# RaphaelHaddad/Real-Time-Brain-Inspired-Video-Memory

Hardware: NVIDIA B200
Metric: queries_per_sec_top10_384d (higher is better)
Workload: dtype tf32

## Files before the change

real-time-brain-inspired-video-memory_b200/csrc/api.cu:

```cuda
#include "common.cuh"

#include <dlfcn.h>
#include <stdarg.h>
#include <stdlib.h>
#include <string.h>
#include <time.h>
#include <new>
#include <vector>

namespace vm {

static thread_local char g_err[512] = "";
void set_error(const char *fmt, ...)
{
    va_list ap;
    va_start(ap, fmt);
    vsnprintf(g_err, sizeof(g_err), fmt, ap);
    va_end(ap);
}

int k_convert_rows(const void *src, int src_dtype, void *dst, int dst_dtype, int64_t n, int dim, int ld, cudaStream_t st);
int k_row_inv_norms(const void *rows, int dtype, float *inv_norms, int64_t row0, int64_t n, int ld, int *extreme, cudaStream_t st,
                    const double *exact = nullptr);
int k_invalidate_rows(float *inv_norms, const int64_t *rows_dev, int64_t n, int64_t size, cudaStream_t st);
int k_normalize_queries(const void *q, int q_dtype, int nq, int nq_pad, int dim, int ld, float *out_f32, void *out_bf16,
                        int32_t *zero_me, uint32_t *zero_tab, int zero_tab_n, int tf32_round, int split, bool pdl, cudaStream_t st);
int k_synth_fill(void *rows, int dtype, uint64_t seed, int64_t row0, int64_t n, int dim, int ld, uint64_t dup_period,
                 cudaStream_t st);
int k_merge_candidates(const uint64_t *cand, int lists, int nq, int kp, uint64_t *merged, cudaStream_t st);

int k_slab_top(const SelectArgs &sa, int nq, int kp, uint64_t *merged, int *incomplete, cudaStream_t st);
int k_rescore(const RescoreArgs &a, cudaStream_t st, const int *incomplete);
int k_select_rescore(const SelectArgs &sa, const RescoreArgs &a, cudaStream_t st, bool pdl);
bool select_rescore_fits(int lists, int list_len, int kp, int dtype, int dim, int ld);
int k_collect_rescore(const uint64_t *buf, const int *cnt, int cap, const RescoreArgs &a, cudaStream_t st);
int k_exact(const ExactArgs &a, cudaStream_t st, bool pdl);
int k_merge_topk_lists(const void *idx, const void *score, const void *count, size_t stride_bytes, int lists, int nq, int k,
                       int64_t *out_idx, double *out_score, int32_t *out_count, cudaStream_t st);
int k_p2p_publish(void *flag, unsigned long long gen, cudaStream_t st);
int k_merge_topk_p2p(void *const *peers, int nranks, size_t slot_off, size_t flag_off, unsigned long long gen, int nq, int k,
                     int64_t *out_idx, double *out_score, int32_t *out_count, cudaStream_t st);
int k_merge_max_by_id(const int64_t *idx, const double *score, const int32_t *count, int nq, int k, int k2,
                      int64_t *out_idx, double *out_score, int32_t *out_count, cudaStream_t st);
int k_cosine_pairs(const void *a, const void *b, int dtype, int64_t n, int dim, int zero_rule, int sum_mode, double *out,
                   cudaStream_t st);
int k_pairs_above(int device, const void *x, int dtype, int64_t n, int dim, int ld, float threshold, int64_t cap,
                  int64_t *out_i, int64_t *out_j, float *out_score, int64_t *out_count, int part, int nparts, int flags,
                  cudaStream_t st);
int k_pairs_concat(const void *gathered, size_t per_rank_bytes, int64_t slot, const int64_t *counts, int nranks, int64_t cap,
                   int64_t *out_i, int64_t *out_j, float *out_score, int64_t *out_count, cudaStream_t st);

struct Arena;
int arena_create(Arena **out, int device, size_t max_bytes);
int arena_grow(Arena *a, size_t bytes);
void arena_destroy(Arena *a);
void *arena_base(const Arena *a);
size_t arena_mapped(const Arena *a);

static constexpr int MAXQ = 64;
static constexpr int MAXK = 64;
static constexpr int XCTAS = 148;
static constexpr int MAX_DEVICES = 64;
static constexpr int COLLECT_CAP = 4096;
static constexpr int FLAG_INTERNAL_CAPTURE = 1 << 30;

struct ResultBlock {
    int64_t *idx;
    double *score;
    int32_t *count;
    static ResultBlock at(void *base, int nq, int k)
    {
        char *b = (char *)base;
        return {(int64_t *)b, (double *)(b + (size_t)nq * k * 8), (int32_t *)(b + (size_t)nq * k * 16)};
    }
    ResultBlock from(int q0, int k) const { return {idx + (size_t)q0 * k, score + (size_t)q0 * k, count + q0}; }
};
static constexpr size_t result_bytes(int nq, int k) { return (size_t)nq * k * 16 + (size_t)nq * 4; }
static constexpr size_t packed_bytes(int nq, int k) { return (result_bytes(nq, k) + 7) & ~(size_t)7; }

static void unpack_to_host(const void *pack, int nq, int k, const ResultBlock &out)
{
    const ResultBlock p = ResultBlock::at(const_cast<void *>(pack), nq, k);
    memcpy(out.idx, p.idx, (size_t)nq * k * 8);
    memcpy(out.score, p.score, (size_t)nq * k * 8);
    memcpy(out.count, p.count, (size_t)nq * 4);
}

struct DeviceGuard {
    int prev = -1;
    bool ok = true;
    explicit DeviceGuard(int dev)
    {
        if (cudaGetDevice(&prev) != cudaSuccess) { ok = false; return; }
        if (prev != dev && cudaSetDevice(dev) != cudaSuccess) ok = false;
    }
    ~DeviceGuard() { if (prev >= 0) cudaSetDevice(prev); }
};

struct Buf {
    void *p = nullptr;
    size_t bytes = 0;
    int ensure(size_t need)
    {
        if (need <= bytes) return VM_OK;
        if (p) cudaFree(p);
        p = nullptr; bytes = 0;
        cudaError_t e = cudaMalloc(&p, need);
        if (e != cudaSuccess) { set_error("cudaMalloc(%zu) failed: %s", need, cudaGetErrorString(e)); return VM_ERR_OOM; }
        bytes = need;
        return VM_OK;
    }
    void release() { if (p) cudaFree(p); p = nullptr; bytes = 0; }
};

struct Workspace {
    bool ready = false;
    int lists_max = 0;
    Buf q_raw, q_f32, q_bf16, seed, cand, merged, o_idx, flags, col_thr, col_cnt, col_buf, xs, xr, xc, taken, gather_send, gather_recv, misc, ubuf, done, scnt, sel_inc;
    int32_t *h_uncert = nullptr;
    unsigned char *h_pack = nullptr;
    unsigned char *h_q = nullptr;
    void release()
    {
        Buf *all[] = {&q_raw, &q_f32, &q_bf16, &seed, &cand, &merged, &o_idx, &flags, &col_thr, &col_cnt, &col_buf, &xs, &xr, &xc, &taken,
                      &gather_send, &gather_recv, &misc, &ubuf, &done, &scnt, &sel_inc};
        for (Buf *b : all) b->release();
        if (h_uncert) cudaFreeHost(h_uncert);
        if (h_pack) cudaFreeHost(h_pack);
        if (h_q) cudaFreeHost(h_q);
        h_uncert = nullptr; h_pack = nullptr; h_q = nullptr;
        ready = false;
    }
};

}

using namespace vm;

struct vm_store {
    int device = 0, dim = 0, ld = 0, dtype = VM_F32, sm_count = 148;
    int64_t capacity = 0, size = 0;
    void *rows = nullptr;
    float *inv_norms = nullptr;
    double *rows_exact = nullptr;
    bool owns = false;
    Arena *ar_rows = nullptr, *ar_inv = nullptr, *ar_exact = nullptr;
    int64_t max_capacity = 0;
    const void *exact_rows() const { return rows_exact ? (const void *)rows_exact : (const void *)rows; }
    int exact_dtype() const { return rows_exact ? (int)VM_F64 : dtype; }
    int *extreme = nullptr;
    unsigned long long *cum = nullptr;
    int64_t n_batches = 0, n_queries = 0;
    int last_band_ctas = 0, last_band_nq = 0;
    Buf stage, stage_idx;
    Workspace ws;
    static constexpr int EV_RING = 64;
    cudaEvent_t evr[EV_RING][2] = {};
    int ev_next = 0;
    int ev_pending = 0;
    int ev_cur = -1;
    bool timed = false;
    struct GraphEntry {
        cudaGraphExec_t exec = nullptr;
        uint64_t version = 0;
        int nq = 0, k = 0, flags = 0, score_mode = 0, sum_mode = 0, q_dtype = 0;
        double min_score = 0.0;
        int64_t row_offset = 0;
        vm_topk_stats stats{};
    };
    GraphEntry graphs[4];
    int graph_next = 0;
    uint64_t version = 1;
    uint64_t seen_version = 0;
    int stable_calls = 0;
    cudaStream_t gstream = nullptr;
};

static constexpr size_t XCHG_SLOT_BYTES = (result_bytes(MAXQ, MAXK) + 255) & ~(size_t)255;
static constexpr size_t XCHG_FLAG_OFF = 2 * XCHG_SLOT_BYTES;
static constexpr size_t XCHG_BYTES = XCHG_FLAG_OFF + 256;

struct vm_comm {
    void *nccl = nullptr;
    int nranks = 1, rank = 0, device = 0;
    void *peer[16] = {};
    bool p2p = false;
    unsigned long long gen = 0;
    Buf pl_i, pl_j, pl_s, pl_cnt, pg_cnt, pg_send, pg_recv;
    int64_t *h_counts = nullptr;
};

struct Id128 { char b[128]; };
namespace {
struct NcclApi {
    void *h = nullptr;
    int (*GetUniqueId)(void *) = nullptr;
    int (*CommInitRank)(void **, int,  Id128, int) = nullptr;
    int (*AllGather)(const void *, void *, size_t, int, void *, cudaStream_t) = nullptr;
    int (*Broadcast)(const void *, void *, size_t, int, int, void *, cudaStream_t) = nullptr;
    int (*CommDestroy)(void *) = nullptr;
    const char *(*GetErrorString)(int) = nullptr;
};
}
static NcclApi g_nccl;

static int nccl_load()
{
    if (g_nccl.h) return VM_OK;
    void *h = dlopen("libnccl.so.2", RTLD_NOW | RTLD_GLOBAL);
    if (!h) h = dlopen("libnccl.so", RTLD_NOW | RTLD_GLOBAL);
    VM_REQUIRE(h, VM_ERR_NCCL, "cannot load libnccl.so.2: %s", dlerror());
    g_nccl.GetUniqueId = (int (*)(void *))dlsym(h, "ncclGetUniqueId");
    g_nccl.CommInitRank = (int (*)(void **, int, Id128, int))dlsym(h, "ncclCommInitRank");
    g_nccl.AllGather = (int (*)(const void *, void *, size_t, int, void *, cudaStream_t))dlsym(h, "ncclAllGather");
    g_nccl.Broadcast = (int (*)(const void *, void *, size_t, int, int, void *, cudaStream_t))dlsym(h, "ncclBroadcast");
    g_nccl.CommDestroy = (int (*)(void *))dlsym(h, "ncclCommDestroy");
    g_nccl.GetErrorString = (const char *(*)(int))dlsym(h, "ncclGetErrorString");
    VM_REQUIRE(g_nccl.GetUniqueId && g_nccl.CommInitRank && g_nccl.AllGather && g_nccl.Broadcast && g_nccl.CommDestroy, VM_ERR_NCCL,
               "libnccl lacks a required symbol");
    g_nccl.h = h;
    return VM_OK;
}
#define VM_NCCL_CHECK(expr)                                                                            \
    do {                                                                                               \
        int _r = (expr);                                                                               \
        if (_r != 0) {                                                                                 \
            set_error("%s failed: %s", #expr, g_nccl.GetErrorString ? g_nccl.GetErrorString(_r) : "?"); \
            return VM_ERR_NCCL;                                                                        \
        }                                                                                              \
    } while (0)

static int check_arch(int device, int *sm_count)
{
    cudaDeviceProp p;
    VM_CUDA_CHECK(cudaGetDeviceProperties(&p, device));
    VM_REQUIRE(p.major == 10, VM_ERR_UNSUPPORTED, "device %d is sm_%d%d; libvidmem is built for sm_100a only", device,
               p.major, p.minor);
    if (sm_count) *sm_count = p.multiProcessorCount;
    return VM_OK;
}

static int ws_prepare(vm_store *s)
{
    Workspace &w = s->ws;
    if (w.ready) return VM_OK;
    int lists = 2 * s->sm_count;
    w.lists_max = lists;
    int rc;
#define ENS(b, bytes) if ((rc = (b).ensure(bytes)) != VM_OK) return rc
    ENS(w.q_raw, (size_t)MAXQ * s->dim * 8);
    ENS(w.q_f32, (size_t)MAXQ * s->ld * 4);
    ENS(w.q_bf16, (size_t)2 * MAXQ * s->ld * 2);
    ENS(w.cand, (size_t)lists * MAXQ * (MAXK > SCAN_SLAB ? MAXK : SCAN_SLAB) * 8);
    ENS(w.merged, (size_t)MAXQ * MAXK * 8);
    ENS(w.o_idx, result_bytes(MAXQ, MAXK) + 64);
    ENS(w.flags, (size_t)(MAXQ + 2) * 4);
    ENS(w.seed, (size_t)(SEED_TAB_WORDS + 3 * MAXQ) * 4);
    ENS(w.ubuf, (size_t)MAXQ * SCAN_UNION_CAP * 8);
    ENS(w.done, 64);
    ENS(w.scnt, (size_t)256 * MAXQ * 4);
    ENS(w.sel_inc, (size_t)MAXQ * 4);
    VM_CUDA_CHECK(cudaMemset(w.done.p, 0, 64));
    ENS(w.col_thr, (size_t)MAXQ * 4);
    ENS(w.col_cnt, (size_t)MAXQ * 4);
    ENS(w.col_buf, (size_t)MAXQ * COLLECT_CAP * 8);
    ENS(w.xs, (size_t)XCTAS * MAXQ * MAXK * 8);
    ENS(w.xr, (size_t)XCTAS * MAXQ * MAXK * 4);
    ENS(w.xc, (size_t)XCTAS * MAXQ * 4);
    ENS(w.taken, (size_t)MAXQ * XCTAS * MAXK);
#undef ENS
    VM_CUDA_CHECK(cudaMallocHost((void **)&w.h_uncert, 64));
    VM_CUDA_CHECK(cudaMallocHost((void **)&w.h_pack, result_bytes(MAXQ, MAXK) + 64));
    VM_CUDA_CHECK(cudaMallocHost((void **)&w.h_q, (size_t)MAXQ * s->dim * 8));
    w.ready = true;
    return VM_OK;
}

static double scan_eps_stored(int kernel, int store_dtype, int dim, int split);
static double scan_eps(int kernel, int store_dtype, int dim, int split, bool shadow = false)
{
    const double base = scan_eps_stored(kernel, store_dtype, dim, split);
    if (!shadow) return base;
    return base + (store_dtype == VM_F32 ? 1.1920928955078125e-07 : 1.953125e-3 * 1.01);
}
static double scan_eps_stored(int kernel, int store_dtype, int dim, int split)
{
    const double u = 1.1920928955078125e-07;
    const double fp32_acc = (double)(dim + 16) * u;
    if (kernel == 1) return fp32_acc;
    if (store_dtype == VM_F32)
        return 9.765625e-4 + 4.8828125e-4 + 1e-6 + fp32_acc;
    if (!split) return 3.90625e-3 + fp32_acc;
    return 1.52587890625e-5 * 1.01 + (double)(dim + dim / 8 + 32) * u;
}

extern "C" int vm_version(void) { return VM_ABI_VERSION; }
extern "C" const char *vm_last_error(void) { return g_err; }

extern "C" int vm_device_info(int device, int *sm_count, int *cc_major, int *cc_minor, size_t *total_mem)
{
    cudaDeviceProp p;
    VM_CUDA_CHECK(cudaGetDeviceProperties(&p, device));
    if (sm_count) *sm_count = p.multiProcessorCount;
    if (cc_major) *cc_major = p.major;
    if (cc_minor) *cc_minor = p.minor;
    if (total_mem) *total_mem = p.totalGlobalMem;
    return VM_OK;
}

extern "C" int vm_ld(int dim) { return ld_for_dim(dim); }

static int store_new(vm_store **out, int device, int dim, int dtype, int64_t capacity)
{
    VM_REQUIRE(out, VM_ERR_BADARG, "out is NULL");
    VM_REQUIRE(dim >= 1 && dim <= 4096, VM_ERR_BADARG, "dim %d outside [1, 4096]", dim);
    VM_REQUIRE(dtype == VM_F32 || dtype == VM_BF16, VM_ERR_BADARG, "store dtype must be VM_F32 or VM_BF16");
    VM_REQUIRE(capacity >= 1 && capacity < 0xFFFFFFFFLL, VM_ERR_BADARG, "capacity %lld outside [1, 2^32-2]", (long long)capacity);
    int sms = 0;
    int rc = check_arch(device, &sms);
    if (rc != VM_OK) return rc;
    vm_store *s = new (std::nothrow) vm_store();
    VM_REQUIRE(s, VM_ERR_OOM, "host allocation failed");
    s->device = device; s->dim = dim; s->ld = ld_for_dim(dim); s->dtype = dtype; s->capacity = capacity; s->sm_count = sms;
    {
        DeviceGuard g(device);
        if (cudaMalloc((void **)&s->extreme, 4) != cudaSuccess || cudaMemset(s->extreme, 0, 4) != cudaSuccess ||
            cudaMalloc((void **)&s->cum, 64) != cudaSuccess || cudaMemset(s->cum, 0, 64) != cudaSuccess) {
            set_error("store allocation failed");
            vm_store_destroy(s);
            return VM_ERR_OOM;
        }
    }
    *out = s;
    return VM_OK;
}

extern "C" int vm_store_create(vm_store **out, int device, int dim, int dtype, int64_t capacity)
{
    int rc = store_new(out, device, dim, dtype, capacity);
    if (rc != VM_OK) return rc;
    vm_store *s = *out;
    DeviceGuard g(device);
    s->owns = true;
    size_t bytes = (size_t)capacity * s->ld * dtype_size(dtype);
    cudaError_t e = cudaMalloc(&s->rows, bytes);
    if (e == cudaSuccess) e = cudaMalloc((void **)&s->inv_norms, (size_t)capacity * 4);
    if (e != cudaSuccess) {
        set_error("store allocation of %zu bytes failed: %s", bytes, cudaGetErrorString(e));
        vm_store_destroy(s);
        *out = nullptr;
        return VM_ERR_OOM;
    }
    return VM_OK;
}

extern "C" int vm_store_create_exact(vm_store **out, int device, int dim, int shadow_dtype, int64_t capacity)
{
    int rc = vm_store_create(out, device, dim, shadow_dtype, capacity);
    if (rc != VM_OK) return rc;
    vm_store *s = *out;
    DeviceGuard g(device);
    const size_t bytes = (size_t)capacity * s->ld * 8;
    cudaError_t e = cudaMalloc((void **)&s->rows_exact, bytes);
    if (e != cudaSuccess) {
        set_error("store allocation of %zu bytes (binary64 rows) failed: %s", bytes, cudaGetErrorString(e));
        vm_store_destroy(s);
        *out = nullptr;
        return VM_ERR_OOM;
    }
    return VM_OK;
}

static int store_back(vm_store *s, int64_t capacity)
{
    int rc = arena_grow(s->ar_rows, (size_t)capacity * s->ld * dtype_size(s->dtype));
    if (rc == VM_OK) rc = arena_grow(s->ar_inv, (size_t)capacity * 4);
    if (rc == VM_OK && s->ar_exact) rc = arena_grow(s->ar_exact, (size_t)capacity * s->ld * 8);
    return rc;
}

extern "C" int vm_store_create_growable(vm_store **out, int device, int dim, int dtype, int exact, int64_t initial_capacity,
                                        int64_t max_capacity)
{
    VM_REQUIRE(initial_capacity >= 1 && max_capacity >= initial_capacity, VM_ERR_BADARG, "need 1 <= initial_capacity <= max_capacity");
    int rc = store_new(out, device, dim, dtype, max_capacity);
    if (rc != VM_OK) return rc;
    vm_store *s = *out;
    DeviceGuard g(device);
    s->max_capacity = max_capacity;
    s->capacity = initial_capacity;
    rc = arena_create(&s->ar_rows, device, (size_t)max_capacity * s->ld * dtype_size(dtype));
    if (rc == VM_OK) rc = arena_create(&s->ar_inv, device, (size_t)max_capacity * 4);
    if (rc == VM_OK && exact) rc = arena_create(&s->ar_exact, device, (size_t)max_capacity * s->ld * 8);
    if (rc == VM_OK) rc = store_back(s, initial_capacity);
    if (rc != VM_OK) { vm_store_destroy(s); *out = nullptr; return rc; }
    s->rows = arena_base(s->ar_rows);
    s->inv_norms = (float *)arena_base(s->ar_inv);
    if (exact) s->rows_exact = (double *)arena_base(s->ar_exact);
    return VM_OK;
}

extern "C" int vm_store_reserve(vm_store *s, int64_t capacity)
{
    VM_REQUIRE(s, VM_ERR_BADARG, "store is NULL");
    if (capacity <= s->capacity) return VM_OK;
    VM_REQUIRE(s->ar_rows, VM_ERR_STATE, "store is not growable (created over fixed buffers of %lld rows)", (long long)s->capacity);
    VM_REQUIRE(capacity <= s->max_capacity, VM_ERR_OVERFLOW, "capacity %lld exceeds the reserved maximum %lld", (long long)capacity,
               (long long)s->max_capacity);
    DeviceGuard g(s->device);
    int rc = store_back(s, capacity);
    if (rc != VM_OK) return rc;
    s->capacity = capacity;
    return VM_OK;
}

extern "C" int64_t vm_store_max_capacity(const vm_store *s) { return s ? (s->ar_rows ? s->max_capacity : s->capacity) : -1; }
extern "C" void *vm_store_rows_ptr(const vm_store *s) { return s ? s->rows : nullptr; }
extern "C" float *vm_store_inv_norms_ptr(const vm_store *s) { return s ? s->inv_norms : nullptr; }
extern "C" double *vm_store_rows_exact_ptr(const vm_store *s) { return s ? s->rows_exact : nullptr; }
extern "C" size_t vm_store_resident_bytes(const vm_store *s)
{
    if (!s) return 0;
    if (s->ar_rows) return arena_mapped(s->ar_rows) + arena_mapped(s->ar_inv) + (s->ar_exact ? arena_mapped(s->ar_exact) : 0);
    return (size_t)s->capacity * ((size_t)s->ld * (dtype_size(s->dtype) + (s->rows_exact ? 8 : 0)) + 4);
}

extern "C" int vm_store_attach_exact(vm_store **out, int device, int dim, int shadow_dtype, int64_t capacity, void *rows_dev,
                                     float *inv_norms_dev, double *rows_exact_dev)
{
    VM_REQUIRE(rows_exact_dev && ((uintptr_t)rows_exact_dev & 15) == 0, VM_ERR_BADARG, "binary64 rows buffer must be 16-byte aligned");
    int rc = vm_store_attach(out, device, dim, shadow_dtype, capacity, rows_dev, inv_norms_dev);
    if (rc != VM_OK) return rc;
    (*out)->rows_exact = rows_exact_dev;
    return VM_OK;
}

extern "C" int vm_store_attach(vm_store **out, int device, int dim, int dtype, int64_t capacity, void *rows_dev,
                               float *inv_norms_dev)
{
    VM_REQUIRE(rows_dev && inv_norms_dev, VM_ERR_BADARG, "attach needs device buffers");
    VM_REQUIRE(((uintptr_t)rows_dev & 127) == 0, VM_ERR_BADARG, "rows buffer must be 128-byte aligned");
    int rc = store_new(out, device, dim, dtype, capacity);
    if (rc != VM_OK) return rc;
    (*out)->rows = rows_dev;
    (*out)->inv_norms = inv_norms_dev;
    (*out)->owns = false;
    return VM_OK;
}

extern "C" int vm_store_destroy(vm_store *s)
{
    if (!s) return VM_OK;
    DeviceGuard g(s->device);
    cudaDeviceSynchronize();
    if (s->owns) { cudaFree(s->rows); cudaFree(s->inv_norms); if (s->rows_exact) cudaFree(s->rows_exact); }
    arena_destroy(s->ar_rows); arena_destroy(s->ar_inv); arena_destroy(s->ar_exact);
    if (s->extreme) cudaFree(s->extreme);
    if (s->cum) cudaFree(s->cum);
    s->stage.release(); s->stage_idx.release();
    s->ws.release();
    for (auto &pr : s->evr) { if (pr[0]) cudaEventDestroy(pr[0]); if (pr[1]) cudaEventDestroy(pr[1]); }
    for (auto &ge : s->graphs) if (ge.exec) cudaGraphExecDestroy(ge.exec);
    if (s->gstream) cudaStreamDestroy(s->gstream);
    delete s;
    return VM_OK;
}

extern "C" int64_t vm_store_size(const vm_store *s) { return s ? s->size : -1; }
extern "C" int64_t vm_store_capacity(const vm_store *s) { return s ? s->capacity : -1; }
extern "C" int vm_store_dim(const vm_store *s) { return s ? s->dim : -1; }
extern "C" int vm_store_ld(const vm_store *s) { return s ? s->ld : -1; }

static int store_write(vm_store *s, int64_t row0, const void *rows, int src_dtype, int src_mem, int64_t n, cudaStream_t st)
{
    VM_REQUIRE(src_dtype == VM_F32 || src_dtype == VM_BF16 || src_dtype == VM_F64, VM_ERR_BADARG, "bad source dtype");
    if (n == 0) return VM_OK;
    VM_REQUIRE(rows, VM_ERR_BADARG, "rows is NULL");
    DeviceGuard g(s->device);
    const void *src = rows;
    if (src_mem == VM_MEM_HOST) {
        size_t bytes = (size_t)n * s->dim * dtype_size(src_dtype);
        int rc = s->stage.ensure(bytes);
        if (rc != VM_OK) return rc;
        VM_CUDA_CHECK(cudaMemcpyAsync(s->stage.p, rows, bytes, cudaMemcpyHostToDevice, st));
        src = s->stage.p;
    }
    char *dst = (char *)s->rows + (size_t)row0 * s->ld * dtype_size(s->dtype);
    int rc = k_convert_rows(src, src_dtype, dst, s->dtype, n, s->dim, s->ld, st);
    if (rc != VM_OK) return rc;
    if (s->rows_exact) {
        rc = k_convert_rows(src, src_dtype, s->rows_exact + (size_t)row0 * s->ld, VM_F64, n, s->dim, s->ld, st);
        if (rc != VM_OK) return rc;
    }
    return k_row_inv_norms(s->rows, s->dtype, s->inv_norms, row0, row0 + n, s->ld, s->extreme, st, s->rows_exact);
}

extern "C" int vm_store_append(vm_store *s, const void *rows, int src_dtype, int src_mem, int64_t n, int64_t *first_row,
                               void *stream)
{
    VM_REQUIRE(s, VM_ERR_BADARG, "store is NULL");
    VM_REQUIRE(n >= 0, VM_ERR_BADARG, "n < 0");
    if (s->ar_rows && s->size + n > s->capacity) {
        const int64_t row_bytes = (int64_t)s->ld * (int64_t)(dtype_size(s->dtype) + (s->rows_exact ? 8 : 0)) + 4;
        const int64_t slack_rows = ((int64_t)256 << 20) / row_bytes + 1;
        int64_t want = s->size + n + slack_rows;
        if (want > s->max_capacity) want = s->max_capacity;
        if (want >= s->size + n) {
            int rc = vm_store_reserve(s, want);
            if (rc != VM_OK && want > s->size + n) rc = vm_store_reserve(s, s->size + n);
            if (rc != VM_OK) return rc;
        }
    }
    VM_REQUIRE(s->size + n <= s->capacity, VM_ERR_OVERFLOW, "append of %lld rows exceeds capacity %lld (size %lld)",
               (long long)n, (long long)s->capacity, (long long)s->size);
    int rc = store_write(s, s->size, rows, src_dtype, src_mem, n, (cudaStream_t)stream);
    if (rc != VM_OK) return rc;
    if (first_row) *first_row = s->size;
    s->size += n;
    ++s->version;
    return VM_OK;
}

extern "C" int vm_store_update(vm_store *s, int64_t row0, const void *rows, int src_dtype, int src_mem, int64_t n, void *stream)
{
    VM_REQUIRE(s, VM_ERR_BADARG, "store is NULL");
    VM_REQUIRE(row0 >= 0 && n >= 0 && row0 + n <= s->size, VM_ERR_BADARG, "update range [%lld, %lld) outside [0, %lld)",
               (long long)row0, (long long)(row0 + n), (long long)s->size);
    ++s->version;
    return store_write(s, row0, rows, src_dtype, src_mem, n, (cudaStream_t)stream);
}

extern "C" int vm_store_invalidate(vm_store *s, const int64_t *rows_host, int64_t n, void *stream)
{
    VM_REQUIRE(s, VM_ERR_BADARG, "store is NULL");
    if (n <= 0) return VM_OK;
    VM_REQUIRE(rows_host, VM_ERR_BADARG, "rows is NULL");
    DeviceGuard g(s->device);
    int rc = s->stage_idx.ensure((size_t)n * 8);
    if (rc != VM_OK) return rc;
    VM_CUDA_CHECK(cudaMemcpyAsync(s->stage_idx.p, rows_host, (size_t)n * 8, cudaMemcpyHostToDevice, (cudaStream_t)stream));
    ++s->version;
    return k_invalidate_rows(s->inv_norms, (const int64_t *)s->stage_idx.p, n, s->size, (cudaStream_t)stream);
}

extern "C" int vm_store_set_size(vm_store *s, int64_t n, int64_t recompute_from_row, void *stream)
{
    VM_REQUIRE(s, VM_ERR_BADARG, "store is NULL");
    VM_REQUIRE(n >= 0 && n <= s->capacity, VM_ERR_BADARG, "size %lld outside [0, capacity]", (long long)n);
    DeviceGuard g(s->device);
    s->size = n;
    ++s->version;
    if (recompute_from_row >= 0 && recompute_from_row < n) {
        if (s->rows_exact) {
            const int64_t r0 = recompute_from_row;
            int rc = k_convert_rows((const char *)s->rows + (size_t)r0 * s->ld * dtype_size(s->dtype), s->dtype,
                                    s->rows_exact + (size_t)r0 * s->ld, VM_F64, n - r0, s->ld, s->ld, (cudaStream_t)stream);
            if (rc != VM_OK) return rc;
        }
        return k_row_inv_norms(s->rows, s->dtype, s->inv_norms, recompute_from_row, n, s->ld, s->extreme, (cudaStream_t)stream, s->rows_exact);
    }
    return VM_OK;
}

extern "C" int vm_store_last_scan_ms(vm_store *s, float *ms)
{
    VM_REQUIRE(s && ms, VM_ERR_BADARG, "NULL argument");
    VM_REQUIRE(s->timed, VM_ERR_STATE, "no vm_topk call with VM_FLAG_TIMING has run the scan kernel yet");
    DeviceGuard g(s->device);
    VM_CUDA_CHECK(cudaEventSynchronize(s->evr[s->ev_cur][1]));
    VM_CUDA_CHECK(cudaEventElapsedTime(ms, s->evr[s->ev_cur][0], s->evr[s->ev_cur][1]));
    return VM_OK;
}

extern "C" int vm_store_avg_scan_ms(vm_store *s, float *ms, int *calls)
{
    VM_REQUIRE(s && ms, VM_ERR_BADARG, "NULL argument");
    VM_REQUIRE(s->timed && s->ev_pending > 0, VM_ERR_STATE, "no vm_topk call with VM_FLAG_TIMING since the last read");
    DeviceGuard g(s->device);
    VM_CUDA_CHECK(cudaEventSynchronize(s->evr[s->ev_cur][1]));
    double sum = 0.0;
    const int n = s->ev_pending;
    for (int i = 0; i < n; ++i) {
        const int slot = (s->ev_cur - i + 2 * vm_store::EV_RING) % vm_store::EV_RING;
        float t = 0.0f;
        VM_CUDA_CHECK(cudaEventElapsedTime(&t, s->evr[slot][0], s->evr[slot][1]));
        sum += t;
    }
    *ms = (float)(sum / n);
    if (calls) *calls = n;
    s->ev_pending = 0;
    return VM_OK;
}

extern "C" int vm_store_band_keys(vm_store *s, int nq_cap, int64_t *kept_per_query, int64_t *spilled_per_query, int *nq_out)
{
    VM_REQUIRE(s && kept_per_query && spilled_per_query, VM_ERR_BADARG, "NULL argument");
    VM_REQUIRE(s->ws.ready && s->last_band_ctas > 0, VM_ERR_STATE, "the last top-k call of this store was not a band-keeping tcgen05 scan");
    const int ctas = s->last_band_ctas, nq = s->last_band_nq;
    VM_REQUIRE(nq_cap >= nq, VM_ERR_BADARG, "room for %d queries needed", nq);
    DeviceGuard g(s->device);
    VM_CUDA_CHECK(cudaDeviceSynchronize());
    std::vector<int> sc((size_t)ctas * nq), uc(nq);
    VM_CUDA_CHECK(cudaMemcpy(sc.data(), s->ws.scnt.p, sc.size() * 4, cudaMemcpyDeviceToHost));
    VM_CUDA_CHECK(cudaMemcpy(uc.data(), (int *)s->ws.seed.p + SEED_TAB_WORDS + 2 * MAXQ, (size_t)nq * 4, cudaMemcpyDeviceToHost));
    for (int q = 0; q < nq; ++q) {
        int64_t k = 0;
        for (int c = 0; c < ctas; ++c) k += sc[(size_t)c * nq + q];
        kept_per_query[q] = k;
        spilled_per_query[q] = uc[q];
    }
    if (nq_out) *nq_out = nq;
    return VM_OK;
}

extern "C" int vm_store_read_counters(vm_store *s, vm_store_counters *out, int reset)
{
    VM_REQUIRE(s && out, VM_ERR_BADARG, "NULL argument");
    DeviceGuard g(s->device);
    unsigned long long h[8] = {0, 0, 0, 0, 0, 0, 0, 0};
    VM_CUDA_CHECK(cudaMemcpy(h, s->cum, sizeof(h), cudaMemcpyDeviceToHost));
    out->batches = s->n_batches; out->queries = s->n_queries;
    out->uncertified = (int64_t)h[0]; out->band_settled = (int64_t)h[1]; out->collect_settled = (int64_t)h[2];
    out->full_rescans = (int64_t)h[3];
    out->bound_violations = (int64_t)h[4];
    if (reset) {
        VM_CUDA_CHECK(cudaMemset(s->cum, 0, sizeof(h)));
        s->n_batches = 0; s->n_queries = 0;
    }
    return VM_OK;
}

extern "C" int vm_store_clear(vm_store *s)
{
    VM_REQUIRE(s, VM_ERR_BADARG, "store is NULL");
    DeviceGuard g(s->device);
    VM_CUDA_CHECK(cudaMemset(s->extreme, 0, 4));
    s->size = 0;
    ++s->version;
    return VM_OK;
}

extern "C" size_t vm_topk_packed_bytes(int nq, int k) { return nq > 0 && k > 0 ? packed_bytes(nq, k) : 0; }

namespace {
struct TopkCall {
    vm_store *s;
    const void *queries;
    int q_dtype, q_mem, nq, k;
    double min_score;
    int score_mode, sum_mode, flags;
    int64_t row_offset;
    ResultBlock d;
    cudaStream_t st;
    vm_topk_stats *stats;
    ResultBlock h = {};
};
}

static cudaError_t wait_stream(cudaStream_t st, const vm_store *s = nullptr)
{
    static const bool block = [] { const char *e = getenv("VIDMEM_SYNC"); return e && !strcmp(e, "block"); }();
    if (block) return cudaStreamSynchronize(st);
    if (s) {
        const double est_us = (double)s->size * s->ld * (double)dtype_size(s->dtype) / 6.5e6;
        if (est_us > 400.0) {
            struct timespec ts;
            const long ns = (long)(est_us * 750.0);
            ts.tv_sec = ns / 1000000000L; ts.tv_nsec = ns % 1000000000L;
            nanosleep(&ts, nullptr);
        }
    }
    for (;;) {
        const cudaError_t e = cudaStreamQuery(st);
        if (e != cudaErrorNotReady) return e;
#if defined(__x86_64__) || defined(__i386__)
        __builtin_ia32_pause();
#endif
    }
}

static int pack_out_enqueue(const TopkCall &c)
{
    VM_CUDA_CHECK(cudaMemcpyAsync(c.s->ws.h_pack, c.d.idx, result_bytes(c.nq, c.k), cudaMemcpyDeviceToHost, c.st));
    return VM_OK;
}

static int tc_list_len(int k) { return k <= 16 ? 32 : (k <= 48 ? 64 : 0); }

static int queries_per_pass(const vm_store *s, int k, int flags)
{
    const int kp = tc_list_len(k);
    if (!(flags & (VM_FLAG_FORCE_EXACT | VM_FLAG_FORCE_SIMT)) && kp)
        for (int nq = 64; nq >= 16; nq -= 16)
            if (scan_tc_supported(s->dtype, s->dim, nq, kp)) return nq;
    return MAXQ;
}

static int topk_batch(const TopkCall &c)
{
    vm_store *s = c.s;
    Workspace &w = s->ws;
    cudaStream_t st = c.st;
    const void *q_dev = c.queries;
    if (c.q_mem == VM_MEM_HOST) {
        const size_t qbytes = (size_t)c.nq * s->dim * dtype_size(c.q_dtype);
        memcpy(w.h_q, c.queries, qbytes);
        VM_CUDA_CHECK(cudaMemcpyAsync(w.q_raw.p, w.h_q, qbytes, cudaMemcpyHostToDevice, st));
        q_dev = w.q_raw.p;
    }
    FinalizeArgs fin{c.k, c.min_score, c.score_mode, c.row_offset, c.d.idx, c.d.score, c.d.count};
    ExactArgs ex{s->exact_rows(), s->inv_norms, s->exact_dtype(), s->ld, s->dim, s->size, q_dev, c.q_dtype, c.nq, c.k, c.sum_mode,
                 nullptr, (double *)w.xs.p, (uint32_t *)w.xr.p, (int32_t *)w.xc.p, (uint8_t *)w.taken.p, XCTAS, fin, s->cum,
                 (int *)w.done.p};
    if (!(c.flags & FLAG_INTERNAL_CAPTURE)) { ++s->n_batches; s->n_queries += c.nq; }
    int launches = 0;
    if (c.stats) { c.stats->uncertified = 0; c.stats->candidates = 0; c.stats->scan_ctas = 0; }

    int kernel = 0, kp = 0;
    if (!(c.flags & VM_FLAG_FORCE_EXACT) && s->size > 0) {
        int kp_tc = tc_list_len(c.k);
        int kp_simt = c.k <= 24 ? (c.k + 8 > 16 ? ((c.k + 8 + 7) & ~7) : 16) : 0;
        bool tc_ok = kp_tc > 0 && scan_tc_supported(s->dtype, s->dim, c.nq, kp_tc);
        bool want_tc = !(c.flags & VM_FLAG_FORCE_SIMT);
        if (want_tc && tc_ok) { kernel = 2; kp = kp_tc; }
        else if (kp_simt > 0) { kernel = 1; kp = kp_simt; }
        else if (tc_ok) { kernel = 2; kp = kp_tc; }
    }
    if (kernel == 0) {
        int rc = k_exact(ex, st, false);
        if (rc != VM_OK) return rc;
        launches += 2;
        if (c.h.idx) {
            if ((rc = pack_out_enqueue(c)) != VM_OK) return rc;
            VM_CUDA_CHECK(wait_stream(st, s));
            unpack_to_host(w.h_pack, c.nq, c.k, c.h);
        }
        if (c.stats) { c.stats->scan_kernel = 0; c.stats->scan_launches += launches; }
        return VM_OK;
    }

    int nq_pad = kernel == 2 ? ((c.nq + 15) & ~15) : c.nq;
    const int split = (kernel == 2 && s->dtype == VM_BF16 && !(c.flags & VM_FLAG_NO_SPLIT) &&
                       (c.nq <= 48 || (c.flags & VM_FLAG_SPLIT)) && scan_tc_supported(s->dtype, s->dim, c.nq, kp, 1)) ? 1 : 0;
#ifdef VIDMEM_NO_GRAPH_PDL
    const bool pdl = !(c.flags & (VM_FLAG_TIMING | FLAG_INTERNAL_CAPTURE));
#else
    const bool pdl = !(c.flags & VM_FLAG_TIMING);
#endif
    int rc = k_normalize_queries(q_dev, c.q_dtype, c.nq, nq_pad, s->dim, s->ld, (float *)w.q_f32.p,
                                 (kernel == 2 && s->dtype == VM_BF16) ? w.q_bf16.p : nullptr,
                                 (int32_t *)w.flags.p + c.nq, kernel == 2 ? (uint32_t *)w.seed.p : nullptr,
                                 kernel == 2 ? (int)(w.seed.bytes / 4) : 0, kernel == 2 && s->dtype == VM_F32, split, pdl, st);
    if (rc != VM_OK) return rc;
    ++launches;
    const double eps = scan_eps(kernel, s->dtype, s->dim, split, s->rows_exact != nullptr);

    ScanArgs a;
    ScanInfo sinfo;
    a.rows = s->rows; a.inv_norms = s->inv_norms; a.dtype = s->dtype; a.n = s->size; a.dim = s->dim; a.ld = s->ld;
    a.queries = (const float *)w.q_f32.p; a.nq = c.nq; a.kp = kp; a.cand = (uint64_t *)w.cand.p; a.stream = st;
    a.slab = (uint64_t *)w.cand.p; a.scnt = (int *)w.scnt.p;
    a.ubuf = (uint64_t *)w.ubuf.p; a.ucnt = (int *)w.seed.p + SEED_TAB_WORDS + 2 * MAXQ; a.ucap = SCAN_UNION_CAP;
    a.band = nextafterf((float)(2.0 * eps), INFINITY); a.ksel = c.k; a.split = split; a.pdl = pdl;
    const bool timing = (c.flags & VM_FLAG_TIMING) != 0;
    if (timing) {
        s->ev_cur = s->ev_next;
        s->ev_next = (s->ev_next + 1) % vm_store::EV_RING;
        if (s->ev_pending < vm_store::EV_RING) ++s->ev_pending;
        if (!s->evr[s->ev_cur][0]) { VM_CUDA_CHECK(cudaEventCreate(&s->evr[s->ev_cur][0])); VM_CUDA_CHECK(cudaEventCreate(&s->evr[s->ev_cur][1])); }
        VM_CUDA_CHECK(cudaEventRecord(s->evr[s->ev_cur][0], st));
    }
    if (kernel == 1) {
        int64_t need = (s->size + 31) / 32;
        a.ctas = (int)imin64(need, 2 * s->sm_count);
        rc = launch_scan_simt(a);
        launches += (c.nq + 7) / 8;
    } else {
        int64_t tiles = (s->size + 127) / 128;
        a.ctas = (int)imin64(tiles, s->sm_count);

        a.dump = tiles <= s->sm_count && tiles * SCAN_DUMP_TILE <= SCAN_DUMP_MAX_KEYS &&
                 (size_t)tiles * c.nq * SCAN_DUMP_TILE * 8 <= w.cand.bytes &&
                 select_rescore_fits((int)tiles, SCAN_DUMP_TILE, kp, s->exact_dtype(), s->dim, s->ld);
        s->last_band_ctas = a.dump ? 0 : a.ctas; s->last_band_nq = c.nq;
        rc = launch_scan_tc(a, s->dtype == VM_BF16 ? w.q_bf16.p : w.q_f32.p, (uint32_t *)w.seed.p, (int *)w.flags.p + c.nq + 1, nullptr, &sinfo);
        launches += 1;
    }
    if (rc != VM_OK) return rc;
    if (timing) { VM_CUDA_CHECK(cudaEventRecord(s->evr[s->ev_cur][1], st)); s->timed = true; }

    int32_t *flags = (int32_t *)w.flags.p;
    int32_t *uncert = flags + c.nq;
    RescoreArgs rs{(const uint64_t *)w.merged.p, kp, s->exact_rows(), s->inv_norms, s->exact_dtype(), s->ld, s->dim, s->size, q_dev,
                   c.q_dtype, c.nq, eps, c.sum_mode, fin, flags, uncert, s->extreme,
                   kernel == 2 ? (float *)w.col_thr.p : nullptr, s->cum};
    SelectArgs sel;
    const bool union_src = kernel == 2 && !a.dump;
    if (union_src) {
        sel.slab = a.slab; sel.scnt = a.scnt; sel.ctas = a.ctas; sel.ubuf = a.ubuf; sel.ucnt = a.ucnt; sel.ucap = a.ucap;
        sel.seed_tab = a.ctas <= 256 ? (const uint32_t *)w.seed.p : nullptr; sel.nq_pad = nq_pad; sel.ksel = c.k; sel.band = a.band;
    } else { sel.cand = a.cand; sel.lists = a.ctas; sel.list_len = a.dump ? SCAN_DUMP_TILE : kp; sel.complete = a.dump ? 1 : 0; }
    rc = k_select_rescore(sel, rs, st, pdl);
    if (rc == VM_ERR_UNSUPPORTED && !a.dump) {
        if (union_src) rc = k_slab_top(sel, c.nq, kp, (uint64_t *)w.merged.p, (int *)w.sel_inc.p, st);
        else rc = k_merge_candidates(a.cand, a.ctas, c.nq, kp, (uint64_t *)w.merged.p, st);
        if (rc != VM_OK) return rc;
        rc = k_rescore(rs, st, union_src ? (const int *)w.sel_inc.p : nullptr);
        ++launches;
    }
    if (rc != VM_OK) return rc;
    launches += 1;

    ex.flags = flags;
    int n_uncert = 0, n_full = -1;
    auto run_collect = [&]() -> int {
        VM_CUDA_CHECK(cudaMemsetAsync(w.col_cnt.p, 0, (size_t)c.nq * 4, st));
        ScanCollect sc{(const float *)w.col_thr.p, (uint64_t *)w.col_buf.p, (int *)w.col_cnt.p, COLLECT_CAP, uncert};
        int r = launch_scan_tc(a, s->dtype == VM_BF16 ? w.q_bf16.p : w.q_f32.p, nullptr, nullptr, &sc);
        if (r != VM_OK) return r;
        return k_collect_rescore((const uint64_t *)w.col_buf.p, (const int *)w.col_cnt.p, COLLECT_CAP, rs, st);
    };
    if (c.flags & VM_FLAG_ASYNC) {
        if (c.flags & FLAG_INTERNAL_CAPTURE) {
            VM_CUDA_CHECK(cudaMemcpyAsync(w.h_uncert, uncert, 4, cudaMemcpyDeviceToHost, st));
        } else {
            rc = k_exact(ex, st, pdl);
            if (rc != VM_OK) return rc;
            launches += 1;
        }
        n_uncert = -1;
    } else {
        VM_CUDA_CHECK(cudaMemcpyAsync(w.h_uncert, uncert, 4, cudaMemcpyDeviceToHost, st));
        if (c.h.idx && (rc = pack_out_enqueue(c)) != VM_OK) return rc;
        VM_CUDA_CHECK(wait_stream(st, s));
        n_uncert = *w.h_uncert;
        n_full = 0;
        if (n_uncert > 0) {
            int left = n_uncert;
            if (kernel == 2) {
                if ((rc = run_collect()) != VM_OK) return rc;
                launches += 2;
                VM_CUDA_CHECK(cudaMemcpyAsync(w.h_uncert, uncert, 4, cudaMemcpyDeviceToHost, st));
                VM_CUDA_CHECK(wait_stream(st, s));
                left = *w.h_uncert;
            }
            n_full = left;
            if (left > 0) {
                rc = k_exact(ex, st, false);
                if (rc != VM_OK) return rc;
                launches += 1;
            }
            if (c.h.idx) {
                if ((rc = pack_out_enqueue(c)) != VM_OK) return rc;
                VM_CUDA_CHECK(wait_stream(st, s));
            }
        }
        if (c.h.idx) unpack_to_host(w.h_pack, c.nq, c.k, c.h);
    }
    if (c.stats) {
        c.stats->scan_kernel = kernel;
        c.stats->scan_launches += launches;
        c.stats->uncertified += n_uncert > 0 ? n_uncert : 0;
        c.stats->full_rescans = n_full;
        c.stats->candidates = kp;
        c.stats->scan_ctas = a.ctas;
        c.stats->scan_stages = kernel == 2 ? sinfo.stages : 0;
        c.stats->scan_variant = kernel == 2 ? sinfo.variant : 0;
    }
    return VM_OK;
}

static constexpr int GRAPH_SKIPPED = 1;

static int graph_capture(const TopkCall &c, vm_store::GraphEntry *ge)
{
    vm_store *s = c.s;
    Workspace &w = s->ws;
    vm_topk_stats cs{};
    TopkCall cc = c;
    cc.queries = w.q_raw.p; cc.q_mem = VM_MEM_DEVICE; cc.flags |= VM_FLAG_ASYNC | FLAG_INTERNAL_CAPTURE;
    cc.d = ResultBlock::at(w.o_idx.p, c.nq, c.k); cc.st = s->gstream; cc.stats = &cs;
    const size_t qbytes = (size_t)c.nq * s->dim * dtype_size(c.q_dtype);
    cudaGraph_t graph = nullptr;
    VM_CUDA_CHECK(cudaStreamBeginCapture(s->gstream, cudaStreamCaptureModeRelaxed));
    int rc = VM_OK;
    if (cudaMemcpyAsync(w.q_raw.p, w.h_q, qbytes, cudaMemcpyHostToDevice, s->gstream) != cudaSuccess) rc = VM_ERR_CUDA;
    if (rc == VM_OK) rc = topk_batch(cc);
    if (rc == VM_OK && cudaMemcpyAsync(w.h_pack, cc.d.idx, result_bytes(c.nq, c.k), cudaMemcpyDeviceToHost, s->gstream) != cudaSuccess)
        rc = VM_ERR_CUDA;
    cudaError_t ce = cudaStreamEndCapture(s->gstream, &graph);
    if (rc != VM_OK || ce != cudaSuccess || !graph) {
        if (graph) cudaGraphDestroy(graph);
        if (rc == VM_OK) { set_error("graph capture failed: %s", cudaGetErrorString(ce)); rc = VM_ERR_CUDA; }
        cudaGetLastError();
        return rc;
    }
    ce = cudaGraphInstantiate(&ge->exec, graph, 0);
    cudaGraphDestroy(graph);
    if (ce != cudaSuccess) { ge->exec = nullptr; set_error("cudaGraphInstantiate failed: %s", cudaGetErrorString(ce)); return VM_ERR_CUDA; }
    ge->version = s->version; ge->nq = c.nq; ge->k = c.k; ge->flags = c.flags; ge->score_mode = c.score_mode;
    ge->sum_mode = c.sum_mode; ge->q_dtype = c.q_dtype; ge->min_score = c.min_score; ge->row_offset = c.row_offset; ge->stats = cs;
    return VM_OK;
}

static int topk_graph(const TopkCall &c, int out_mem, bool sharded, const ResultBlock &out)
{
    vm_store *s = c.s;
    Workspace &w = s->ws;
    static const bool no_graph = getenv("VIDMEM_NO_GRAPH") != nullptr;
    if (s->seen_version == s->version) { if (s->stable_calls < 1 << 20) ++s->stable_calls; }
    else { s->seen_version = s->version; s->stable_calls = 0; }
    if (no_graph || s->stable_calls < 16 || sharded || c.st != nullptr || c.q_mem != VM_MEM_HOST || out_mem != VM_MEM_HOST ||
        (c.flags & (VM_FLAG_ASYNC | VM_FLAG_TIMING | VM_FLAG_FORCE_EXACT)) || s->size == 0 ||
        c.nq > queries_per_pass(s, c.k, c.flags))
        return GRAPH_SKIPPED;
    if (!s->gstream) VM_CUDA_CHECK(cudaStreamCreate(&s->gstream));
    vm_store::GraphEntry *ge = nullptr;
    for (auto &e : s->graphs)
        if (e.exec && e.version == s->version && e.nq == c.nq && e.k == c.k && e.flags == c.flags && e.score_mode == c.score_mode &&
            e.sum_mode == c.sum_mode && e.q_dtype == c.q_dtype && e.row_offset == c.row_offset &&
            memcmp(&e.min_score, &c.min_score, sizeof(double)) == 0) { ge = &e; break; }
    if (!ge) {
        ge = &s->graphs[s->graph_next];
        s->graph_next = (s->graph_next + 1) & 3;
        if (ge->exec) { cudaGraphExecDestroy(ge->exec); ge->exec = nullptr; }
        const int rc = graph_capture(c, ge);
        if (rc != VM_OK) return rc;
    }
    memcpy(w.h_q, c.queries, (size_t)c.nq * s->dim * dtype_size(c.q_dtype));
    ++s->n_batches; s->n_queries += c.nq;
    VM_CUDA_CHECK(cudaGraphLaunch(ge->exec, s->gstream));
    VM_CUDA_CHECK(wait_stream(s->gstream, s));
    const int uncertified = ge->stats.scan_kernel != 0 ? *w.h_uncert : 0;
    if (uncertified > 0) {
        TopkCall rerun = c;
        rerun.d = ResultBlock::at(w.o_idx.p, c.nq, c.k); rerun.st = s->gstream; rerun.h = out;
        return topk_batch(rerun);
    }
    unpack_to_host(w.h_pack, c.nq, c.k, out);
    if (c.stats) { *c.stats = ge->stats; c.stats->uncertified = uncertified; }
    return VM_OK;
}

static size_t xchg_slot_off(unsigned long long gen) { return (size_t)(gen & 1) * XCHG_SLOT_BYTES; }

static ResultBlock batch_dest(vm_store *s, const vm_comm *comm, bool sharded, int out_mem, const ResultBlock &out, int nb, int k)
{
    if (sharded && comm->p2p) return ResultBlock::at((char *)comm->peer[comm->rank] + xchg_slot_off(comm->gen), nb, k);
    if (sharded) return ResultBlock::at(s->ws.gather_send.p, nb, k);
    return out_mem == VM_MEM_DEVICE ? out : ResultBlock::at(s->ws.o_idx.p, nb, k);
}

static int exchange_merge(vm_store *s, vm_comm *comm, int nb, int k, const ResultBlock &m, cudaStream_t st)
{
    if (comm->p2p) {
        const int rc = k_p2p_publish((char *)comm->peer[comm->rank] + XCHG_FLAG_OFF, comm->gen, st);
        if (rc != VM_OK) return rc;
        return k_merge_topk_p2p(comm->peer, comm->nranks, xchg_slot_off(comm->gen), XCHG_FLAG_OFF, comm->gen, nb, k, m.idx, m.score,
                                m.count, st);
    }
    const Workspace &w = s->ws;
    VM_NCCL_CHECK(g_nccl.AllGather(w.gather_send.p, w.gather_recv.p, packed_bytes(nb, k),  0, comm->nccl, st));
    const ResultBlock r = ResultBlock::at(w.gather_recv.p, nb, k);
    return k_merge_topk_lists(r.idx, r.score, r.count, packed_bytes(nb, k), comm->nranks, nb, k, m.idx, m.score, m.count, st);
}

static int topk_common(vm_store *s, vm_comm *comm, int64_t row_offset, const void *queries, int q_dtype, int q_mem, int nq,
                       int k, double min_score, int score_mode, int sum_mode, int flags, int64_t *out_idx,
                       double *out_score, int32_t *out_count, int out_mem, vm_topk_stats *stats, void *stream)
{
    VM_REQUIRE(s, VM_ERR_BADARG, "store is NULL");
    VM_REQUIRE(nq >= 0, VM_ERR_BADARG, "nq < 0");
    VM_REQUIRE(k >= 1 && k <= MAXK, VM_ERR_BADARG, "k %d outside [1, %d]", k, MAXK);
    VM_REQUIRE(q_dtype == VM_F32 || q_dtype == VM_BF16 || q_dtype == VM_F64, VM_ERR_BADARG, "bad query dtype");
    VM_REQUIRE(score_mode == VM_SCORE_RAW || score_mode == VM_SCORE_NEO4J, VM_ERR_BADARG, "bad score_mode");
    VM_REQUIRE(sum_mode == VM_SUM_NAIVE || sum_mode == VM_SUM_NEUMAIER, VM_ERR_BADARG, "bad sum_mode");
    VM_REQUIRE(!(flags & VM_FLAG_ASYNC) || (out_mem == VM_MEM_DEVICE && q_mem == VM_MEM_DEVICE), VM_ERR_BADARG,
               "VM_FLAG_ASYNC needs device queries and device outputs");
    if (stats) memset(stats, 0, sizeof(*stats));
    if (nq == 0) return VM_OK;
    VM_REQUIRE(queries && out_idx && out_score && out_count, VM_ERR_BADARG, "NULL buffer");
    DeviceGuard g(s->device);
    VM_REQUIRE(g.ok, VM_ERR_CUDA, "cannot select device %d", s->device);
    int rc = ws_prepare(s);
    if (rc != VM_OK) return rc;
    const bool sharded = comm && comm->nranks > 1;
    const ResultBlock out{out_idx, out_score, out_count};
    const TopkCall call{s, queries, q_dtype, q_mem, nq, k, min_score, score_mode, sum_mode, flags, row_offset, {}, (cudaStream_t)stream,
                        stats};
    if ((rc = topk_graph(call, out_mem, sharded, out)) != GRAPH_SKIPPED) return rc;

    Workspace &w = s->ws;
    const int bq = queries_per_pass(s, k, flags);
    for (int q0 = 0; q0 < nq; q0 += bq) {
        const int nb = nq - q0 < bq ? nq - q0 : bq;
        const ResultBlock out_b = out.from(q0, k);
        if (sharded && comm->p2p) {
            ++comm->gen;
        } else if (sharded) {
            if ((rc = w.gather_send.ensure(packed_bytes(nb, k))) != VM_OK) return rc;
            if ((rc = w.gather_recv.ensure(packed_bytes(nb, k) * comm->nranks)) != VM_OK) return rc;
        }
        TopkCall c = call;
        c.queries = (const char *)queries + (size_t)q0 * s->dim * dtype_size(q_dtype);
        c.nq = nb;
        c.d = batch_dest(s, comm, sharded, out_mem, out_b, nb, k);
        if (out_mem == VM_MEM_HOST) {
            if (sharded) c.flags |= VM_FLAG_ASYNC;
            else c.h = out_b;
        }
        if ((rc = topk_batch(c)) != VM_OK) return rc;
        if (!sharded) continue;
        const ResultBlock ws = ResultBlock::at(w.o_idx.p, nb, k);
        if ((rc = exchange_merge(s, comm, nb, k, out_mem == VM_MEM_DEVICE ? out_b : ws, c.st)) != VM_OK) return rc;
        if (stats) stats->scan_launches += 2;
        if (out_mem == VM_MEM_HOST) {
            VM_CUDA_CHECK(cudaMemcpyAsync(w.h_pack, ws.idx, result_bytes(nb, k), cudaMemcpyDeviceToHost, c.st));
            VM_CUDA_CHECK(wait_stream(c.st, s));
            unpack_to_host(w.h_pack, nb, k, out_b);
        }
    }
    return VM_OK;
}

extern "C" int vm_topk(vm_store *s, const void *queries, int q_dtype, int q_mem, int nq, int k, double min_score,
                       int score_mode, int sum_mode, int flags, int64_t *out_idx, double *out_score, int32_t *out_count,
                       int out_mem, vm_topk_stats *stats, void *stream)
{
    return topk_common(s, nullptr, 0, queries, q_dtype, q_mem, nq, k, min_score, score_mode, sum_mode, flags, out_idx,
                       out_score, out_count, out_mem, stats, stream);
}

extern "C" int vm_topk_sharded(vm_store *s, vm_comm *comm, int64_t row_offset, const void *queries, int q_dtype, int q_mem,
                               int nq, int k, double min_score, int score_mode, int sum_mode, int flags, int64_t *out_idx,
                               double *out_score, int32_t *out_count, int out_mem, vm_topk_stats *stats, void *stream)
{
    VM_REQUIRE(comm, VM_ERR_BADARG, "comm is NULL");
    return topk_common(s, comm, row_offset, queries, q_dtype, q_mem, nq, k, min_score, score_mode, sum_mode, flags, out_idx,
                       out_score, out_count, out_mem, stats, stream);
}

extern "C" int vm_merge_topk_lists(int device, const int64_t *idx_dev, const double *score_dev, const int32_t *count_dev,
                                   int nlists, int nq, int k, int64_t *out_idx_dev, double *out_score_dev,
                                   int32_t *out_count_dev, void *stream)
{
    VM_REQUIRE(idx_dev && score_dev && count_dev && out_idx_dev && out_score_dev && out_count_dev, VM_ERR_BADARG, "NULL buffer");
    VM_REQUIRE(nlists >= 1 && nq >= 1 && k >= 1, VM_ERR_BADARG, "bad shape");
    DeviceGuard g(device);
    size_t stride = (size_t)nq * k * 8;
    VM_REQUIRE(device >= 0 && device < MAX_DEVICES, VM_ERR_BADARG, "device index %d outside [0, %d)", device, MAX_DEVICES);
    static thread_local Buf cnt_wide_dev[MAX_DEVICES];
    Buf &cnt_wide = cnt_wide_dev[device];
    int rc = cnt_wide.ensure(stride * nlists);
    if (rc != VM_OK) return rc;
    VM_CUDA_CHECK(cudaMemcpy2DAsync(cnt_wide.p, stride, count_dev, (size_t)nq * 4, (size_t)nq * 4, nlists,
                                    cudaMemcpyDeviceToDevice, (cudaStream_t)stream));
    return k_merge_topk_lists(idx_dev, score_dev, cnt_wide.p, stride, nlists, nq, k, out_idx_dev, out_score_dev,
                              out_count_dev, (cudaStream_t)stream);
}

extern "C" int vm_merge_topk_packed(int device, const void *packed_dev, int nlists, int nq, int k, int64_t *out_idx_dev,
                                    double *out_score_dev, int32_t *out_count_dev, void *stream)
{
    VM_REQUIRE(packed_dev && out_idx_dev && out_score_dev && out_count_dev, VM_ERR_BADARG, "NULL buffer");
    VM_REQUIRE(nlists >= 1 && nq >= 1 && k >= 1, VM_ERR_BADARG, "bad shape");
// ... 196 lines not shown
```

real-time-brain-inspired-video-memory_b200/csrc/common.cuh:

```cuda
#pragma once
#include <cuda_runtime.h>
#include <cuda_bf16.h>
#include <stdint.h>
#include <stdio.h>
#include <math.h>
#include <utility>
#include "../../include/vidmem.h"

namespace vm {

void set_error(const char *fmt, ...);
#define VM_CUDA_CHECK(expr)                                                                      \
    do {                                                                                         \
        cudaError_t _e = (expr);                                                                 \
        if (_e != cudaSuccess) {                                                                 \
            vm::set_error("%s failed: %s (%s:%d)", #expr, cudaGetErrorString(_e), __FILE__, __LINE__); \
            return VM_ERR_CUDA;                                                                  \
        }                                                                                        \
    } while (0)
#define VM_REQUIRE(cond, code, ...)          \
    do {                                     \
        if (!(cond)) {                       \
            vm::set_error(__VA_ARGS__);      \
            return (code);                   \
        }                                    \
    } while (0)

__device__ __forceinline__ void pdl_wait() { asm volatile("griddepcontrol.wait;" ::: "memory"); }
__device__ __forceinline__ void pdl_launch_dependents() { asm volatile("griddepcontrol.launch_dependents;" ::: "memory"); }

template <typename... KArgs, typename... Args>
static inline cudaError_t launch_pdl(void (*kernel)(KArgs...), dim3 grid, dim3 block, size_t smem, cudaStream_t st, bool pdl,
                                     Args &&...args)
{
    cudaLaunchConfig_t cfg = {};
    cfg.gridDim = grid; cfg.blockDim = block; cfg.dynamicSmemBytes = smem; cfg.stream = st;
    cudaLaunchAttribute at[1];
    at[0].id = cudaLaunchAttributeProgrammaticStreamSerialization;
    at[0].val.programmaticStreamSerializationAllowed = 1;
    cfg.attrs = at;
    cfg.numAttrs = pdl ? 1 : 0;
    return cudaLaunchKernelEx(&cfg, kernel, std::forward<Args>(args)...);
}

template <auto Kernel>
static inline cudaError_t max_smem_once(int bytes)
{
    static bool set[64] = {};
    int dev = 0;
    cudaError_t e = cudaGetDevice(&dev);
    if (e != cudaSuccess || set[dev & 63]) return e;
    e = cudaFuncSetAttribute(Kernel, cudaFuncAttributeMaxDynamicSharedMemorySize, bytes);
    if (e == cudaSuccess) set[dev & 63] = true;
    return e;
}

__host__ __device__ __forceinline__ uint32_t f32_ordered(float f)
{
#ifdef __CUDA_ARCH__
    uint32_t b = __float_as_uint(f);
#else
    uint32_t b;
    memcpy(&b, &f, 4);
#endif
    return (b & 0x80000000u) ? ~b : (b | 0x80000000u);
}
__host__ __device__ __forceinline__ float f32_from_ordered(uint32_t o)
{
    uint32_t b = (o & 0x80000000u) ? (o & 0x7FFFFFFFu) : ~o;
#ifdef __CUDA_ARCH__
    return __uint_as_float(b);
#else
    float f;
    memcpy(&f, &b, 4);
    return f;
#endif
}
__host__ __device__ __forceinline__ uint64_t make_key(float score, uint32_t row)
{
    return ((uint64_t)f32_ordered(score) << 32) | (uint64_t)(0xFFFFFFFFu - row);
}
__host__ __device__ __forceinline__ uint32_t key_row(uint64_t k) { return 0xFFFFFFFFu - (uint32_t)(k & 0xFFFFFFFFu); }
__host__ __device__ __forceinline__ float key_score(uint64_t k) { return f32_from_ordered((uint32_t)(k >> 32)); }

static constexpr int SEED_TAB_WORDS = 256 * 64;
#ifdef __CUDACC__
__device__ __forceinline__ float seed_select(const uint32_t *seed_tab, int G, int nq_pad, int q, int k, int lane)
{
    uint32_t vals[8];
#pragma unroll
    for (int t = 0; t < 8; ++t) {
        const int i = lane + 32 * t;
        vals[t] = i < G ? __ldcg(seed_tab + (size_t)i * nq_pad + q) : 0u;
    }
    uint32_t prefix = 0;
    int need = k;
    for (int bit = 31; bit >= 16; --bit) {
        const uint32_t hi = bit == 31 ? 0u : (0xFFFFFFFFu << (bit + 1));
        int cnt = 0;
#pragma unroll
        for (int t = 0; t < 8; ++t) cnt += ((vals[t] & hi) == prefix && ((vals[t] >> bit) & 1u)) ? 1 : 0;
        const int tot = __reduce_add_sync(0xffffffffu, cnt);
        if (tot >= need) prefix |= 1u << bit;
        else need -= tot;
    }
    float sd = f32_from_ordered(prefix);
    if (!(sd > -INFINITY) || G < k) sd = -INFINITY;
    return sd;
}

__device__ __forceinline__ float band_floor(float L, float band)
{
    if (!(L > -INFINITY)) return -INFINITY;
    const float t = __fsub_rd(L, band);
    return nextafterf(t, -INFINITY);
}

#endif

struct RefSum {
    double s, c;
    __device__ __forceinline__ void init() { s = 0.0; c = 0.0; }
    template <bool NEUMAIER>
    __device__ __forceinline__ void add(double x)
    {
        double t = __dadd_rn(s, x);
        if (NEUMAIER) {
            const bool big = fabs(s) >= fabs(x);
            const double hi = big ? s : x, lo = big ? x : s;
            c = __dadd_rn(c, __dadd_rn(__dadd_rn(hi, -t), lo));
        }
        s = t;
    }
    template <bool NEUMAIER>
    __device__ __forceinline__ void add_block(const double (&x)[8])
    {
        double t[8];
        t[0] = __dadd_rn(s, x[0]);
#pragma unroll
        for (int u = 1; u < 8; ++u) t[u] = __dadd_rn(t[u - 1], x[u]);
        if (NEUMAIER) {
#pragma unroll
            for (int u = 0; u < 8; ++u) {
                const double prev = u ? t[u - 1] : s;
                const bool big = fabs(prev) >= fabs(x[u]);
                const double hi = big ? prev : x[u], lo = big ? x[u] : prev;
                c = __dadd_rn(c, __dadd_rn(__dadd_rn(hi, -t[u]), lo));
            }
        }
        s = t[7];
    }
    template <bool NEUMAIER>
    __device__ __forceinline__ double result() const
    {
        double r = s;
        if (NEUMAIER && c != 0.0 && isfinite(c)) r = __dadd_rn(r, c);
        return r;
    }
};

template <bool NEUMAIER, typename F>
__device__ __forceinline__ void ref_sum_range(RefSum &acc, int lo, int hi, F prod)
{
    int i = lo;
    for (; i + 8 <= hi; i += 8) {
        double x[8];
#pragma unroll
        for (int u = 0; u < 8; ++u) x[u] = prod(i + u);
        acc.add_block<NEUMAIER>(x);
    }
    for (; i < hi; ++i) acc.add<NEUMAIER>(prod(i));
}

__device__ __forceinline__ float load_as_float(const float *p, int64_t i) { return p[i]; }
__device__ __forceinline__ float load_as_float(const __nv_bfloat16 *p, int64_t i) { return __bfloat162float(p[i]); }
__device__ __forceinline__ double load_elem(const float *p, int64_t i) { return (double)p[i]; }
__device__ __forceinline__ double load_elem(const __nv_bfloat16 *p, int64_t i) { return (double)__bfloat162float(p[i]); }
__device__ __forceinline__ double load_elem(const double *p, int64_t i) { return p[i]; }
__device__ __forceinline__ double load_as_double(const void *p, int dtype, int64_t i)
{
    if (dtype == VM_F32) return (double)((const float *)p)[i];
    if (dtype == VM_BF16) return (double)__bfloat162float(((const __nv_bfloat16 *)p)[i]);
    return ((const double *)p)[i];
}

static inline int64_t imin64(int64_t a, int64_t b) { return a < b ? a : b; }
static inline int ld_for_dim(int dim) { return (dim + 7) & ~7; }
static inline size_t dtype_size(int dt) { return dt == VM_F32 ? 4 : dt == VM_BF16 ? 2 : 8; }

struct ScanArgs {
    const void *rows;
    const float *inv_norms;
    int dtype;
    int64_t n;
    int dim, ld;
    const float *queries;
    int nq;
    int kp;
    uint64_t *cand;
    int ctas;
    cudaStream_t stream;
    int dump = 0;
    uint64_t *slab = nullptr;
    int *scnt = nullptr;
    uint64_t *ubuf = nullptr;
    int *ucnt = nullptr;
    int ucap = 0;
    float band = 0.0f;
    int ksel = 0;
    int split = 0;
    bool pdl = false;
};
static constexpr int SCAN_UNION_CAP = 16384;
static constexpr int SCAN_SLAB = 128;
static constexpr int SELECT_KEY_CAP = 4096;
static constexpr int SCAN_DUMP_TILE = 128;
static constexpr int SCAN_DUMP_MAX_KEYS = 9472;
int launch_scan_simt(const ScanArgs &a);
int scan_simt_max_queries();
struct ScanCollect {
    const float *thr;
    uint64_t *buf;
    int *cnt;
    int cap;
    const int *pending;
};
struct ScanInfo { int stages = 0, variant = 0; };
int launch_scan_tc(const ScanArgs &a, const void *queries_store_dtype, uint32_t *seed_tab, int *seed_ctr,
                   const ScanCollect *sc = nullptr, ScanInfo *info = nullptr);
bool scan_tc_supported(int dtype, int dim, int nq, int kp, int split = 0);


struct FinalizeArgs {
    int k;
    double min_score;
    int score_mode;
    int64_t row_offset;
    int64_t *out_idx;
    double *out_score;
    int32_t *out_count;
};
struct RescoreArgs {
    const uint64_t *merged;
    int kp;
    const void *rows;
    const float *inv_norms;
    int dtype, ld, dim;
    int64_t n_rows;
    const void *queries;
    int q_dtype, nq;
    double eps;
    int sum_mode;
    FinalizeArgs fin;
    int32_t *flags, *uncertified_count;
    const int *extreme;
    float *collect_thr;
    unsigned long long *cum = nullptr;
};
struct SelectArgs {
    const uint64_t *cand = nullptr;
    int lists = 0, list_len = 0;
    int complete = 0;
    const uint64_t *slab = nullptr;
    const int *scnt = nullptr;
    int ctas = 0;
    const uint64_t *ubuf = nullptr;
    const int *ucnt = nullptr;
    int ucap = 0;
    const uint32_t *seed_tab = nullptr;
    int nq_pad = 0, ksel = 0;
    float band = 0.0f;
};
struct ExactArgs {
    const void *rows;
    const float *inv_norms;
    int dtype, ld, dim;
    int64_t n;
    const void *queries;
    int q_dtype, nq, k, sum_mode;
    int32_t *flags;
    double *xlist_score;
    uint32_t *xlist_row;
    int32_t *xlist_cnt;
    uint8_t *taken;
    int ctas;
    FinalizeArgs fin;
    unsigned long long *cum = nullptr;
    int *done_ctr = nullptr;
};

}
```

real-time-brain-inspired-video-memory_b200/csrc/scan_tc.cu:

```cuda
#include "tc_common.cuh"

namespace vm {
using namespace tc;

static constexpr int TC_BLOCK_M = 128;
static constexpr int TC_STAGE_BYTES = TC_BLOCK_M * 128;
static constexpr int TC_ACC = 8;
static constexpr int TC_THREADS_SVC = 288;
static constexpr int TC_THREADS = 192;
static constexpr int TC_TMEM_COLS = 512;
static constexpr int TC_MAX_STAGES = 8;

struct CollectArgs {
    const float *thr;
    uint64_t *buf;
    int *cnt;
    int cap;
    const int *pending;
};

struct BandArgs {
    uint64_t *slab;
    int *scnt;
    uint64_t *ubuf;
    int *ucnt;
    int ucap;
    float band;
    int ksel;
    int use_seed;
};

struct TcLayout {
    int nq_pad, KB, stages, split;
    uint32_t off_b, off_a, off_tauf, off_lcnt, off_cmax, off_wmax, off_flags, off_bars, off_tmem, total;
};

static TcLayout make_layout(int dtype, int ld, int nq, int split = 0)
{
    TcLayout L{};
    const int es = dtype == VM_F32 ? 4 : 2;
    L.nq_pad = (nq + 15) & ~15;
    L.KB = (ld * es + 127) / 128;
    L.split = (split && dtype == VM_BF16) ? 1 : 0;
    uint32_t o = 0;
    L.off_b = o; o += (uint32_t)L.KB * L.nq_pad * 128 * (L.split ? 2 : 1);
    const uint32_t epi = (uint32_t)L.nq_pad * (4 + 4 + 4 + 16) + 64 + 8 * (2 * TC_MAX_STAGES + 1 + 2 * TC_ACC) + 16;
    int64_t room = 227 * 1024 - 2048 - (int64_t)o - epi;
    L.stages = (int)(room / TC_STAGE_BYTES);
    if (L.stages > TC_MAX_STAGES) L.stages = TC_MAX_STAGES;
    if (L.stages < 0) L.stages = 0;
    L.off_a = o; o += (uint32_t)L.stages * TC_STAGE_BYTES;
    L.off_tauf = o; o += (uint32_t)L.nq_pad * 4;
    L.off_lcnt = o; o += (uint32_t)L.nq_pad * 4;
    L.off_cmax = o; o += (uint32_t)L.nq_pad * 4;
    L.off_wmax = o; o += (uint32_t)L.nq_pad * 16;
    L.off_flags = o; o += 64;
    L.off_bars = o; o += 8 * (2 * TC_MAX_STAGES + 1 + 2 * TC_ACC);
    L.off_tmem = o; o += 16;
    L.total = o + 1024;
#ifdef VIDMEM_AB_SMEMPAD
    if (L.total < 220 * 1024) L.total = 220 * 1024;
#endif
    return L;
}

__device__ __forceinline__ uint32_t own_kth_score(const uint64_t *slab, int n, int k, int lane)
{
    constexpr int PER = SCAN_SLAB / 32;
    uint32_t vals[PER];
#pragma unroll
    for (int t = 0; t < PER; ++t) {
        const int i = lane + 32 * t;
        vals[t] = i < n ? (uint32_t)(__ldcg(slab + i) >> 32) : 0u;
    }
    uint32_t prefix = 0;
    int need = k;
    for (int bit = 31; bit >= 12; --bit) {
        const uint32_t hi = bit == 31 ? 0u : (0xFFFFFFFFu << (bit + 1));
        int cnt = 0;
#pragma unroll
        for (int t = 0; t < PER; ++t) cnt += ((vals[t] & hi) == prefix && ((vals[t] >> bit) & 1u)) ? 1 : 0;
        const int tot = __reduce_add_sync(0xffffffffu, cnt);
        if (tot >= need) prefix |= 1u << bit;
        else need -= tot;
    }
    int ge = 0;
#pragma unroll
    for (int t = 0; t < PER; ++t) ge += (vals[t] != 0u && vals[t] >= prefix) ? 1 : 0;
    ge = __reduce_add_sync(0xffffffffu, ge);
    return (ge >= k && prefix != 0u) ? prefix : 0u;
}

template <bool TF32, bool DUMP, bool SPLIT>
__global__ void __launch_bounds__(DUMP ? TC_THREADS : TC_THREADS_SVC, 1)
scan_tc_kernel(const __grid_constant__ CUtensorMap tmA, const __grid_constant__ CUtensorMap tmB,
               const float *__restrict__ inv_norms, int64_t n, int num_tiles, int nq, TcLayout L, uint64_t *__restrict__ dump_keys,
               uint32_t *__restrict__ seed_tab, int *__restrict__ seed_ctr, CollectArgs col, BandArgs ub, int svc_sleep)
{
    const bool collect = !DUMP && col.thr != nullptr;
#ifndef VIDMEM_AB_NOPDL
    pdl_launch_dependents();
#endif
    if (collect) {
        pdl_wait();
        if (*col.pending == 0) return;
    }

    extern __shared__ __align__(16) uint8_t smem_raw[];
    uint8_t *base = smem_raw + ((1024u - (smem_u32(smem_raw) & 1023u)) & 1023u);
    uint8_t *sB = base + L.off_b;
    uint8_t *sA = base + L.off_a;
    float *tauf = (float *)(base + L.off_tauf);
    int *lcnt = (int *)(base + L.off_lcnt);
    uint32_t *cmax = (uint32_t *)(base + L.off_cmax);
    uint32_t *wmax = (uint32_t *)(base + L.off_wmax);
    volatile int *s_done = (volatile int *)(base + L.off_flags);
    uint64_t *bars = (uint64_t *)(base + L.off_bars);
    uint64_t *full = bars, *empty = bars + TC_MAX_STAGES, *qfull = bars + 2 * TC_MAX_STAGES;
    uint64_t *tfull = qfull + 1, *tempty = tfull + TC_ACC;
    uint32_t *tmem_slot = (uint32_t *)(base + L.off_tmem);

    const int warp = __shfl_sync(0xffffffffu, threadIdx.x >> 5, 0);
    const int lane = threadIdx.x & 31;
    const int nq_pad = L.nq_pad, KB = L.KB, stages = L.stages;
    constexpr int ELEMS = TF32 ? 32 : 64;

    if (warp == 0 && lane == 0) {
        tma_prefetch_desc(&tmA);
        tma_prefetch_desc(&tmB);
        for (int s = 0; s < stages; ++s) { mbar_init(&full[s], 1); mbar_init(&empty[s], 1); }
        mbar_init(qfull, 1);
        for (int a = 0; a < TC_ACC; ++a) { mbar_init(&tfull[a], 1); mbar_init(&tempty[a], 4); }
        fence_barrier_init();
    }
    if (warp == 1) tmem_alloc(tmem_slot, TC_TMEM_COLS);
#ifndef VIDMEM_AB_NOPDL
    if (!collect) pdl_wait();
#endif
    if (warp >= 2 && warp < 6) {
        const int e = threadIdx.x - 64;
        if (e < nq_pad) {
            lcnt[e] = 0;
            cmax[e] = 0u;
            tauf[e] = collect ? (e < nq ? col.thr[e] : INFINITY) : (e < nq ? -INFINITY : INFINITY);
        }
        if (e < 2) s_done[e] = 0;
    }
    tc_fence_before();
    __syncthreads();
    tc_fence_after();
    const uint32_t tmem_base = *tmem_slot;
    uint32_t *gbound = seed_tab ? seed_tab + SEED_TAB_WORDS : nullptr;

    if (warp == 0) {
        if (elect_one()) {
            constexpr int QPARTS = SPLIT ? 2 : 1;
            mbar_arrive_expect_tx(qfull, (uint32_t)(KB * QPARTS) * nq_pad * 128);
            for (int part = 0; part < QPARTS; ++part)
                for (int kb = 0; kb < KB; ++kb)
                    tma_load_2d(&tmB, qfull, sB + (size_t)(part * KB + kb) * nq_pad * 128, kb * ELEMS, part * nq_pad, L2_EVICT_LAST);
        }
        __syncwarp();
        int stage = 0;
        uint32_t phase = 0;
        for (int tile = blockIdx.x; tile < num_tiles; tile += gridDim.x) {
            for (int kb = 0; kb < KB; ++kb) {
                mbar_wait(&empty[stage], phase ^ 1);
                if (elect_one()) {
                    mbar_arrive_expect_tx(&full[stage], TC_STAGE_BYTES);
                    tma_load_2d(&tmA, &full[stage], sA + (size_t)stage * TC_STAGE_BYTES, kb * ELEMS, tile * TC_BLOCK_M, L2_EVICT_FIRST);
                }
                __syncwarp();
                if (++stage == stages) { stage = 0; phase ^= 1; }
            }
        }
    } else if (warp == 1) {
        const uint32_t idesc = make_idesc(TF32 ? 2u : 1u, TC_BLOCK_M, (uint32_t)nq_pad);
        mbar_wait(qfull, 0);
        tc_fence_after();
        int stage = 0, acc = 0;
        uint32_t phase = 0, acc_phase = 0;
        const uint64_t da0 = make_smem_desc_sw128(smem_u32(sA)), db0 = make_smem_desc_sw128(smem_u32(sB));
        const uint32_t kb_step = (uint32_t)(nq_pad * 128) >> 4, lo_step = (uint32_t)(KB * nq_pad * 128) >> 4;
        for (int tile = blockIdx.x; tile < num_tiles; tile += gridDim.x) {
            mbar_wait(&tempty[acc], acc_phase ^ 1);
            tc_fence_after();
            const uint32_t d_tmem = tmem_base + (uint32_t)(acc * nq_pad);
            for (int kb = 0; kb < KB; ++kb) {
                mbar_wait(&full[stage], phase);
                tc_fence_after();
                if (elect_one()) {
                    const uint64_t da = da0 + (uint64_t)((uint32_t)stage * (TC_STAGE_BYTES >> 4));
                    const uint64_t db = db0 + (uint64_t)((uint32_t)kb * kb_step);
#pragma unroll
                    for (int j = 0; j < 4; ++j) {
                        umma<TF32>(d_tmem, da + 2 * j, db + 2 * j, idesc, (uint32_t)((kb | j) != 0));
                        if constexpr (SPLIT) umma<TF32>(d_tmem, da + 2 * j, db + lo_step + 2 * j, idesc, 1u);
                    }
                    umma_commit(&empty[stage]);
                    if (kb == KB - 1) umma_commit(&tfull[acc]);
                }
                __syncwarp();
                if (++stage == stages) { stage = 0; phase ^= 1; }
            }
            if (++acc == TC_ACC) { acc = 0; acc_phase ^= 1; }
        }
    } else if (warp < 6) {
        const int e = threadIdx.x - 64;
        const int quad = warp & 3;
        const int row_in_tile = quad * 32 + lane;
        int acc = 0;
        uint32_t acc_phase = 0;
        if constexpr (DUMP) {
            for (int tile = blockIdx.x; tile < num_tiles; tile += gridDim.x) {
                const int64_t r = (int64_t)tile * TC_BLOCK_M + row_in_tile;
                const float iv = r < n ? __ldg(inv_norms + r) : -1.0f;
                mbar_wait(&tfull[acc], acc_phase);
                tc_fence_after();
                const uint32_t taddr = tmem_base + ((uint32_t)(quad * 32) << 16) + (uint32_t)(acc * nq_pad);
                uint64_t *out = dump_keys + (int64_t)tile * nq * TC_BLOCK_M + row_in_tile;
                for (int c = 0; c < nq_pad; c += 16) {
                    uint32_t v[16];
                    tmem_ld16(taddr + c, v);
                    tmem_ld_wait();
#pragma unroll
                    for (int j = 0; j < 16; ++j)
                        if (c + j < nq)
                            out[(int64_t)(c + j) * TC_BLOCK_M] = iv >= 0.0f ? make_key(__uint_as_float(v[j]) * iv, (uint32_t)r) : 0ull;
                }
                tc_fence_before();
                __syncwarp();
                if (lane == 0) mbar_arrive(&tempty[acc]);
                if (++acc == TC_ACC) { acc = 0; acc_phase ^= 1; }
            }
        } else {
        if (ub.use_seed && !collect) {
            const int64_t row0 = (int64_t)blockIdx.x * TC_BLOCK_M + row_in_tile;
            const float inv0 = row0 < n ? __ldg(inv_norms + row0) : -1.0f;
            mbar_wait(&tfull[0], 0);
            tc_fence_after();
            const uint32_t taddr0 = tmem_base + ((uint32_t)(quad * 32) << 16);
            for (int c = 0; c < nq_pad; c += 16) {
                uint32_t v[16];
                tmem_ld16(taddr0 + c, v);
                tmem_ld_wait();
#pragma unroll
                for (int j = 0; j < 16; ++j) {
                    const float sc = inv0 >= 0.0f ? __uint_as_float(v[j]) * inv0 : -INFINITY;
                    const uint32_t mx = __reduce_max_sync(0xffffffffu, f32_ordered(sc));
                    if (lane == 0) wmax[(warp - 2) * nq_pad + c + j] = mx;
                }
            }
            named_bar_sync(1, 128);
            if (e < nq_pad) {
                uint32_t m = wmax[e];
#pragma unroll
                for (int w = 1; w < 4; ++w) m = max(m, wmax[w * nq_pad + e]);
                seed_tab[(size_t)blockIdx.x * nq_pad + e] = m;
                cmax[e] = m;
            }
            __threadfence();
            named_bar_sync(1, 128);
            if (e == 0) {
                atomicAdd(seed_ctr, 1);
                const long long t0 = clock64();
                while (*(volatile int *)seed_ctr < (int)gridDim.x)
                    if (clock64() - t0 > 400000) break;
                __threadfence();
            }
            named_bar_sync(1, 128);
            const int G = (int)gridDim.x;
            int *pub_ctr = reinterpret_cast<int *>(gbound + 64);
            if (warp == 2) {
                for (int q = blockIdx.x; q < nq; q += G) {
                    const float sd = seed_select(seed_tab, G, nq_pad, q, ub.ksel, lane);
                    if (lane == 0) {
                        if (sd > -INFINITY) atomicMax(gbound + q, f32_ordered(sd));
                        __threadfence();
                        atomicAdd(pub_ctr, 1);
                    }
                }
                if (lane == 0) {
                    const long long t0 = clock64();
                    while (*(volatile int *)pub_ctr < nq)
                        if (clock64() - t0 > 200000) break;
                    __threadfence();
                }
            }
            named_bar_sync(1, 128);
            if (e < nq) {
                const uint32_t o = __ldcg(gbound + e);
                if (o != 0u) tauf[e] = band_floor(f32_from_ordered(o), ub.band);
            }
            named_bar_sync(1, 128);
        }
        if (!collect && e == 0) s_done[1] = 1;
        uint64_t *my_slab = collect ? nullptr : ub.slab + (size_t)blockIdx.x * nq * SCAN_SLAB;
        int64_t row = (int64_t)blockIdx.x * TC_BLOCK_M + row_in_tile;
        float inv = row < n ? __ldg(inv_norms + row) : -1.0f;
        for (int tile = blockIdx.x; tile < num_tiles; tile += gridDim.x) {
            const int64_t row_next = row + (int64_t)gridDim.x * TC_BLOCK_M;
            const float inv_next = (tile + (int)gridDim.x < num_tiles && row_next < n) ? __ldg(inv_norms + row_next) : -1.0f;
            const bool valid = inv >= 0.0f;
            mbar_wait(&tfull[acc], acc_phase);
            tc_fence_after();
            const uint32_t taddr = tmem_base + ((uint32_t)(quad * 32) << 16) + (uint32_t)(acc * nq_pad);
            auto process = [&](const uint32_t (&v)[16], int c) {
                float tf[16];
#pragma unroll
                for (int j4 = 0; j4 < 4; ++j4) {
                    const float4 t4 = *reinterpret_cast<const float4 *>(tauf + c + 4 * j4);
                    tf[4 * j4] = t4.x; tf[4 * j4 + 1] = t4.y; tf[4 * j4 + 2] = t4.z; tf[4 * j4 + 3] = t4.w;
                }
                if (valid) {
                    uint32_t hits = 0;
#pragma unroll
                    for (int j = 0; j < 16; ++j) hits |= (__uint_as_float(v[j]) * inv >= tf[j]) ? (1u << j) : 0u;
                    hits &= nq - c >= 16 ? 0xFFFFu : ((1u << (nq - c > 0 ? nq - c : 0)) - 1u);
                    while (hits) {
                        const int j = __ffs(hits) - 1;
                        hits &= hits - 1;
                        const int q = c + j;
                        float s = 0.0f;
#pragma unroll
                        for (int jj = 0; jj < 16; ++jj) s = (jj == j) ? __uint_as_float(v[jj]) * inv : s;
                        const uint64_t key = make_key(s, (uint32_t)row);
                        if (collect) {
                            const int pos = atomicAdd(col.cnt + q, 1);
                            if (pos < col.cap) col.buf[(size_t)q * col.cap + pos] = key;
                        } else {
#ifdef VIDMEM_AB_NORARE
                            if (key == 1) tauf[q] = 0.0f;
                            continue;
#endif
                            const int pos = atomicAdd(&lcnt[q], 1);
                            atomicMax(&cmax[q], (uint32_t)(key >> 32));
                            if (pos < SCAN_SLAB) __stcg(my_slab + (size_t)q * SCAN_SLAB + pos, key);
                            else {
                                const int p = atomicAdd(ub.ucnt + q, 1);
                                if (p < ub.ucap) __stcg(ub.ubuf + (size_t)q * ub.ucap + p, key);
                                else tauf[q] = INFINITY;
                            }
                        }
                    }
                }
            };
            uint32_t va[16], vb[16];
#ifdef VIDMEM_AB_NOEPI
            if (tile < 0)
#endif
            tmem_ld16(taddr, va);
#ifdef VIDMEM_AB_NOEPI
            if (tile < 0)
#endif
            for (int c = 0; c < nq_pad; c += 32) {
                tmem_ld_wait();
                if (c + 16 < nq_pad) tmem_ld16(taddr + c + 16, vb);
                process(va, c);
                if (c + 16 < nq_pad) {
                    tmem_ld_wait();
                    if (c + 32 < nq_pad) tmem_ld16(taddr + c + 32, va);
                    process(vb, c + 16);
                }
            }
#ifdef VIDMEM_AB_TILEBAR
            named_bar_sync(1, 128);
#endif
            tc_fence_before();
            __syncwarp();
            if (lane == 0) mbar_arrive(&tempty[acc]);
            if (++acc == TC_ACC) { acc = 0; acc_phase ^= 1; }
            row = row_next;
            inv = inv_next;
        }
        if (!collect) {
            named_bar_sync(1, 128);
            if (e < nq) {
                ub.scnt[(size_t)blockIdx.x * nq + e] = lcnt[e];
                if (seed_tab != nullptr) __stcg(seed_tab + (size_t)blockIdx.x * nq_pad + e, cmax[e]);
            }
        }
        }
        __syncwarp();
        if (lane == 0) atomicAdd((int *)s_done, 1);
    } else {
#ifdef VIDMEM_AB_NOSVC
        if (false) {
#else
        if (!DUMP && warp == 8 && seed_tab != nullptr && !collect) {
#endif
            const int G = (int)gridDim.x;
            while (s_done[1] == 0 && s_done[0] < 4) __nanosleep(100);
            uint32_t pub0 = 0xFFFFFFFFu, pub1 = 0xFFFFFFFFu;
            uint32_t kth_done = 0;
            const uint64_t *my_slab = ub.slab + (size_t)blockIdx.x * nq * SCAN_SLAB;
            while (!__any_sync(0xffffffffu, s_done[0] >= 4)) {
#pragma unroll
                for (int h = 0; h < 2; ++h) {
                    const int q = lane + 32 * h;
                    if (q < nq) {
                        const uint32_t c = *(volatile uint32_t *)(cmax + q);
                        uint32_t &pub = h ? pub1 : pub0;
                        if (c != pub && c != 0u) { __stcg(seed_tab + (size_t)blockIdx.x * nq_pad + q, c); pub = c; }
                    }
                }
                __syncwarp();
                if (G >= ub.ksel)
                    for (int q = blockIdx.x; q < nq; q += G) {
                        const float sd = seed_select(seed_tab, G, nq_pad, q, ub.ksel, lane);
                        if (lane == 0 && sd > -INFINITY) atomicMax(gbound + q, f32_ordered(sd));
                    }
                __syncwarp();
#ifndef VIDMEM_AB_KTH_LEVELS
#define VIDMEM_AB_KTH_LEVELS 2
#endif
#ifndef VIDMEM_AB_KTH_PER_ROUND
#define VIDMEM_AB_KTH_PER_ROUND 1
#endif
                {
                    constexpr int LV = VIDMEM_AB_KTH_LEVELS;
                    int served = 0;
#pragma unroll
                    for (int h = 0; h < 2; ++h) {
                        const int q = lane + 32 * h;
                        int level = 0;
                        if (q < nq) {
                            const int have = *(volatile int *)(lcnt + q);
#pragma unroll
                            for (int l = 1; l <= LV; ++l) level = have >= (SCAN_SLAB >> (LV - l)) ? l : level;
                        }
                        const int done = (int)((kth_done >> (4 * h)) & 15u);
                        unsigned todo = __ballot_sync(0xffffffffu, level > done && (SCAN_SLAB >> (LV - level)) >= ub.ksel);
                        while (todo && (VIDMEM_AB_KTH_PER_ROUND == 0 || served < VIDMEM_AB_KTH_PER_ROUND)) {
                            const int src = __ffs(todo) - 1;
                            todo &= todo - 1;
                            ++served;
                            const int lv = __shfl_sync(0xffffffffu, level, src);
                            const int qq = src + 32 * h;
                            const uint32_t ok = own_kth_score(my_slab + (size_t)qq * SCAN_SLAB, SCAN_SLAB >> (LV - lv), ub.ksel, lane);
                            if (lane == src && ok != 0u) {
                                atomicMax(gbound + qq, ok);
                                kth_done = (kth_done & ~(15u << (4 * h))) | ((uint32_t)lv << (4 * h));
                            }
                        }
                    }
                }
                __syncwarp();
#pragma unroll
                for (int h = 0; h < 2; ++h) {
                    const int q = lane + 32 * h;
                    if (q < nq) {
                        const uint32_t o = __ldcg(gbound + q);
                        if (o != 0u) {
                            const float f = band_floor(f32_from_ordered(o), ub.band);
                            if (f > tauf[q]) *(volatile float *)(tauf + q) = f;
                        }
                    }
                }
                __nanosleep(svc_sleep);
            }
        }
    }

    tc_fence_before();
    __syncthreads();
    if (warp == 1) {
        tc_fence_after();
        tmem_dealloc(tmem_base, TC_TMEM_COLS);
    }
}

bool scan_tc_supported(int dtype, int dim, int nq, int kp, int split)
{
    (void)kp;
    if (dtype != VM_F32 && dtype != VM_BF16) return false;
    if (nq < 1 || nq > 64) return false;
    TcLayout L = make_layout(dtype, ld_for_dim(dim), nq, split);
    return L.stages >= 3;
}

int launch_scan_tc(const ScanArgs &a, const void *queries_store_dtype, uint32_t *seed_tab, int *seed_ctr, const ScanCollect *sc,
                   ScanInfo *info)
{
    VM_REQUIRE(a.n >= 1 && a.n < 0x7FFFFF00LL, VM_ERR_UNSUPPORTED, "tcgen05 scan: shard rows %lld outside [1, 2^31)", (long long)a.n);
    TcLayout L = make_layout(a.dtype, a.ld, a.nq, a.split);
    VM_REQUIRE(L.stages >= 3, VM_ERR_UNSUPPORTED, "tcgen05 scan: dim %d x %d queries does not fit shared memory", a.dim, a.nq);
    CUtensorMap tmA, tmB;
    int rc = make_tmap_2d_cached(&tmA, a.rows, a.dtype, (uint64_t)a.n, (uint64_t)a.ld, (uint64_t)a.ld, TC_BLOCK_M);
    if (rc != VM_OK) return rc;
    rc = make_tmap_2d_cached(&tmB, queries_store_dtype, a.dtype, (uint64_t)L.nq_pad * (L.split ? 2 : 1), (uint64_t)a.ld, (uint64_t)a.ld,
                             (uint32_t)L.nq_pad);
    if (rc != VM_OK) return rc;
    const int num_tiles = (int)((a.n + TC_BLOCK_M - 1) / TC_BLOCK_M);
    const bool dump = a.dump && !sc;
    if (sc || dump || a.ctas > 256) { seed_tab = nullptr; seed_ctr = nullptr; }
    CollectArgs col{};
    if (sc) { col.thr = sc->thr; col.buf = sc->buf; col.cnt = sc->cnt; col.cap = sc->cap; col.pending = sc->pending; }
    BandArgs ub{a.slab, a.scnt, a.ubuf, a.ucnt, a.ucap, a.band, a.ksel, 0};
    ub.use_seed = (seed_tab && seed_ctr && a.ksel >= 1 && a.ctas >= a.ksel) ? 1 : 0;
    if (!sc && !dump)
        VM_REQUIRE(ub.slab && ub.scnt && ub.ubuf && ub.ucnt && ub.ucap > 0 && ub.ksel >= 1, VM_ERR_BADARG, "tcgen05 scan: slab / spill buffers missing");
    if (dump) VM_REQUIRE(TC_BLOCK_M == SCAN_DUMP_TILE && (int64_t)num_tiles * TC_BLOCK_M <= SCAN_DUMP_MAX_KEYS && a.ctas == num_tiles,
                         VM_ERR_UNSUPPORTED, "tcgen05 scan: dump mode needs one CTA per tile and at most %d rows", SCAN_DUMP_MAX_KEYS);
#ifdef VIDMEM_AB_SVCSLEEP
    const int svc_sleep = VIDMEM_AB_SVCSLEEP;
#else
    const int svc_sleep = a.dtype == VM_F32 ? 500 : 200;
#endif
    if (info && !sc) { info->stages = L.stages; info->variant = dump ? 1 : 2; }
    const bool pdl = a.pdl && !sc;
#ifdef VIDMEM_AB_CLASSIC_LAUNCH
#define LAUNCH_IMPL(TF, DU, SP) scan_tc_kernel<TF, DU, SP><<<a.ctas, DU ? TC_THREADS : TC_THREADS_SVC, L.total, a.stream>>>(tmA, tmB, a.inv_norms, a.n, num_tiles, a.nq, L, a.cand, seed_tab, seed_ctr, col, ub, svc_sleep)
#else
#define LAUNCH_IMPL(TF, DU, SP) VM_CUDA_CHECK(launch_pdl(scan_tc_kernel<TF, DU, SP>, dim3(a.ctas), dim3(DU ? TC_THREADS : TC_THREADS_SVC), L.total, a.stream, pdl, \
                                 tmA, tmB, a.inv_norms, a.n, num_tiles, a.nq, L, a.cand, seed_tab, seed_ctr, col, ub, svc_sleep))
#endif
#define LAUNCH_TC(TF, DU, SP)                                                                                                \
    do {                                                                                                                   \
        VM_CUDA_CHECK((max_smem_once<scan_tc_kernel<TF, DU, SP>>(227 * 1024)));                                              \
        LAUNCH_IMPL(TF, DU, SP);                                                                                           \
    } while (0)
    if (a.dtype == VM_F32) { if (dump) LAUNCH_TC(true, true, false); else LAUNCH_TC(true, false, false); }
    else if (L.split) { if (dump) LAUNCH_TC(false, true, true); else LAUNCH_TC(false, false, true); }
    else { if (dump) LAUNCH_TC(false, true, false); else LAUNCH_TC(false, false, false); }
#undef LAUNCH_TC
#undef LAUNCH_IMPL
    VM_CUDA_CHECK(cudaGetLastError());
    return VM_OK;
}

}
```

real-time-brain-inspired-video-memory_b200/csrc/select.cu:

```cuda
#include "common.cuh"

#include <type_traits>

namespace vm {

static constexpr int MERGE_THREADS = 512;
static constexpr int MERGE_SURV = 1024;

__device__ uint64_t radix_select_kth(const uint64_t *skeys, int total, int kp, int *hist, int *s_bin, int *s_need)
{
    const int tid = threadIdx.x, lane = tid & 31;
    uint64_t prefix = 0;
    int need = kp;
    for (int pass = 0; pass < 8; ++pass) {
        const int shift = 56 - 8 * pass;
        const uint64_t hmask = pass == 0 ? 0ull : (~0ull << (shift + 8));
        if (tid < 256) hist[tid] = 0;
        __syncthreads();
        for (int e = tid; e < total; e += MERGE_THREADS) {
            const uint64_t k = skeys[e];
            const bool act = k != 0 && (k & hmask) == prefix;
            const int bin = act ? (int)((k >> shift) & 0xFF) : -1;
            const unsigned peers = __match_any_sync(__activemask(), bin);
            if (act && (__ffs(peers) - 1) == lane) atomicAdd(&hist[bin], __popc(peers));
// ... 155 lines not shown
}

__device__ __forceinline__ bool better(double sa, uint32_t ra, double sb, uint32_t rb)
{
    return sa > sb || (sa == sb && ra < rb);
}

static constexpr int RS_THREADS = 256;
static constexpr int RS_SMEM_ROW_BYTES = 96 * 1024;

__device__ __forceinline__ void load_vec16(const float *p, float *o)
{
    const float4 t = *reinterpret_cast<const float4 *>(p);
    o[0] = t.x; o[1] = t.y; o[2] = t.z; o[3] = t.w;
}
__device__ __forceinline__ void load_vec16(const __nv_bfloat16 *p, float *o)
{
    const uint4 u = *reinterpret_cast<const uint4 *>(p);
    o[0] = __uint_as_float(u.x << 16); o[1] = __uint_as_float(u.x & 0xffff0000u);
    o[2] = __uint_as_float(u.y << 16); o[3] = __uint_as_float(u.y & 0xffff0000u);
    o[4] = __uint_as_float(u.z << 16); o[5] = __uint_as_float(u.z & 0xffff0000u);
    o[6] = __uint_as_float(u.w << 16); o[7] = __uint_as_float(u.w & 0xffff0000u);
}

__device__ __forceinline__ void load_vec16(const double *p, double *o)
{
    const double2 t = *reinterpret_cast<const double2 *>(p);
    o[0] = t.x; o[1] = t.y;
}
template <typename T> struct StageOf { using type = float; };
template <> struct StageOf<double> { using type = double; };

template <bool NEUMAIER, typename T>
__global__ void __launch_bounds__(RS_THREADS, 1) rescore_kernel(const uint64_t *__restrict__ merged, int kp, const T *__restrict__ rows,
                                                            const float *__restrict__ inv_norms, int ld, int dim, int64_t n_rows,
                                                            const void *__restrict__ queries, int q_dtype, double eps,
                                                            FinalizeArgs f, int32_t *__restrict__ flags,
                                                            int32_t *__restrict__ uncertified_count, int chunk,
                                                            const int *__restrict__ extreme, float *__restrict__ collect_thr,
                                                            unsigned long long *__restrict__ cum, const int *__restrict__ incomplete)
{
    constexpr int VEC = 16 / (int)sizeof(T);
    extern __shared__ double rs_smem[];
    double *sq = rs_smem;
    using S = typename StageOf<T>::type;
    S *srow = reinterpret_cast<S *>(rs_smem + chunk);
    const int pitch = chunk + 1;
    __shared__ double s_dot[64], s_rr[64], s_qq;
    __shared__ double s_score[64];
    __shared__ uint32_t s_row[64];
    __shared__ int s_valid[64];
    __shared__ int s_cnt;
    const int q = blockIdx.x, j = threadIdx.x;
    if (j == 0) s_cnt = 0;
    if (j < 64) {
        uint64_t key = j < kp ? merged[(int64_t)q * kp + j] : 0;
        s_valid[j] = key != 0;
        s_row[j] = key != 0 ? key_row(key) : 0;
    }
    __syncthreads();
    const int kind = j < kp ? 0 : (j < 2 * kp ? 1 : (j == 2 * kp ? 2 : 3));
    const int cand = kind == 0 ? j : (kind == 1 ? j - kp : 0);
    const bool active = kind == 2 || (kind < 2 && s_valid[cand]);
    RefSum acc;
    acc.init();
    for (int c0 = 0; c0 < dim; c0 += chunk) {
        const int len = min(chunk, dim - c0);
        const int vlen = (min(chunk, ld - c0) + VEC - 1) / VEC;
        for (int i = j; i < len; i += RS_THREADS) sq[i] = load_as_double(queries, q_dtype, (int64_t)q * dim + c0 + i);
        const int groups = kp * vlen;
        for (int g0 = j; g0 < groups; g0 += 4 * RS_THREADS) {
            S buf[4][VEC];
            int rr_[4], cc_[4];
#pragma unroll
            for (int u = 0; u < 4; ++u) {
                const int g = g0 + u * RS_THREADS;
                rr_[u] = g < groups ? g / vlen : -1;
                cc_[u] = g < groups ? (g - rr_[u] * vlen) * VEC : 0;
                if (rr_[u] >= 0 && s_valid[rr_[u]]) load_vec16(rows + (int64_t)s_row[rr_[u]] * ld + c0 + cc_[u], buf[u]);
                else
#pragma unroll
                    for (int x = 0; x < VEC; ++x) buf[u][x] = (S)0;
            }
#pragma unroll
            for (int u = 0; u < 4; ++u)
                if (rr_[u] >= 0)
#pragma unroll
                    for (int x = 0; x < VEC; ++x)
                        if (cc_[u] + x < chunk) srow[rr_[u] * pitch + cc_[u] + x] = buf[u][x];
        }
        __syncthreads();
        if (active) {
            const S *mine = srow + cand * pitch;
            if (kind == 0)
                ref_sum_range<NEUMAIER>(acc, 0, len, [&](int i) { return __dmul_rn(sq[i], (double)mine[i]); });
            else if (kind == 1)
                ref_sum_range<NEUMAIER>(acc, 0, len, [&](int i) { const double y = (double)mine[i]; return __dmul_rn(y, y); });
            else
                ref_sum_range<NEUMAIER>(acc, 0, len, [&](int i) { const double x = sq[i]; return __dmul_rn(x, x); });
        }
        __syncthreads();
    }
    if (active) {
        const double r = acc.result<NEUMAIER>();
        if (kind == 0) s_dot[cand] = r;
        else if (kind == 1) s_rr[cand] = r;
        else s_qq = r;
    }
    __syncthreads();
    const bool valid = j < 64 && s_valid[j];
    double sc = 0.0;
    const uint32_t row = j < 64 ? s_row[j] : 0;
    if (valid) {
        const double n1 = __dsqrt_rn(s_qq);
        const double n2 = __dsqrt_rn(s_rr[j]);
        sc = (n1 == 0.0 || n2 == 0.0) ? 0.0 : __ddiv_rn(s_dot[j], __dmul_rn(n1, n2));
    }
    if (j < 64) s_score[j] = sc;
    __syncthreads();
    int ncand = 0;
    for (int i = 0; i < 64; ++i) ncand += s_valid[i];
    int rank = 0;
    if (valid)
        for (int i = 0; i < 64; ++i)
            if (s_valid[i] && i != j && better(s_score[i], s_row[i], sc, row)) ++rank;
    double outv = convert_score(sc, f.score_mode);
    bool emit = valid && rank < f.k && outv > f.min_score;
    if (emit) {
        f.out_idx[(int64_t)q * f.k + rank] = (int64_t)row + f.row_offset;
        f.out_score[(int64_t)q * f.k + rank] = outv;
        atomicAdd(&s_cnt, 1);
    }
    __syncthreads();
    if (valid && rank == min(f.k, ncand) - 1) {
        bool cert = true;
        if (ncand >= kp && (int64_t)ncand < n_rows) {
            float worst = key_score(merged[(int64_t)q * kp + kp - 1]);
            cert = ((double)worst + eps) < sc;
        }
        if (incomplete && incomplete[q]) cert = false;
        const bool bound_ok = !(extreme && *extreme != 0);
        if (!bound_ok && (int64_t)ncand < n_rows) cert = false;
        flags[q] = cert ? 0 : (bound_ok ? 1 : 2);
        if (collect_thr) {
            float t = (float)(sc - 2.0 * eps);
            t = nextafterf(nextafterf(t, -INFINITY), -INFINITY);
            collect_thr[q] = (!cert && bound_ok) ? t : INFINITY;
        }
        if (!cert) { atomicAdd(uncertified_count, 1); if (cum) atomicAdd(cum, 1ull); }
    }
    if (ncand == 0 && j == 0) { flags[q] = 0; if (collect_thr) collect_thr[q] = INFINITY; }
    if (j == 0) f.out_count[q] = s_cnt;
    int cnt = s_cnt;
    for (int t = cnt + j; t < f.k; t += RS_THREADS) {
        f.out_idx[(int64_t)q * f.k + t] = -1;
        f.out_score[(int64_t)q * f.k + t] = 0.0;
    }
}

__device__ __forceinline__ void cp_async16(void *smem_dst, const void *gsrc)
{
    asm volatile("cp.async.cg.shared.global [%0], [%1], 16;" ::"r"((uint32_t)__cvta_generic_to_shared(smem_dst)), "l"(gsrc) : "memory");
}
__device__ __forceinline__ void cp_async_commit() { asm volatile("cp.async.commit_group;" ::: "memory"); }
template <int N> __device__ __forceinline__ void cp_async_wait() { asm volatile("cp.async.wait_group %0;" ::"n"(N) : "memory"); }

static constexpr int SR_THREADS = 512;
static constexpr int BAND_CAP_MIN = 1024, BAND_CAP_MAX = 2048;

template <bool NEUMAIER, typename T, int THREADS>
__device__ void band_score_global(const T *__restrict__ rows, int ld, int dim, const double *sq, double n1, int m, double *s_sc, double *s_rr,
                                  const uint32_t *s_row)
{
    const int tid = threadIdx.x;
    const int lines = (ld * (int)sizeof(T) + 127) / 128;
    for (int e = tid; e < m * lines; e += THREADS) {
        const int r = e / lines, l = e - r * lines;
        asm volatile("prefetch.global.L2 [%0];" ::"l"(reinterpret_cast<const char *>(rows + (int64_t)s_row[r] * ld) + (size_t)l * 128));
    }
    for (int t = tid; t < 2 * m; t += THREADS) {
        const int e = t >> 1;
        const T *row = rows + (int64_t)s_row[e] * ld;
        RefSum acc;
        acc.init();
        if (t & 1) {
            ref_sum_range<NEUMAIER>(acc, 0, dim, [&](int i) { const double y = load_elem(row, i); return __dmul_rn(y, y); });
            s_rr[e] = acc.result<NEUMAIER>();
        } else {
            ref_sum_range<NEUMAIER>(acc, 0, dim, [&](int i) { return __dmul_rn(sq[i], load_elem(row, i)); });
            s_sc[e] = acc.result<NEUMAIER>();
        }
    }
    __syncthreads();
    for (int e = tid; e < m; e += THREADS) {
        const double n2 = __dsqrt_rn(s_rr[e]);
        s_sc[e] = (n1 == 0.0 || n2 == 0.0) ? 0.0 : __ddiv_rn(s_sc[e], __dmul_rn(n1, n2));
    }
    __syncthreads();
}

template <int THREADS>
__device__ int band_emit(int m, const double *s_sc, const uint32_t *s_row, int *s_out, const FinalizeArgs &f, int q)
{
    const int tid = threadIdx.x;
    if (tid == 0) *s_out = 0;
    __syncthreads();
    for (int e = tid; e < m; e += THREADS) {
        const double sc = s_sc[e];
        const uint32_t row = s_row[e];
        int rank = 0;
        for (int i = 0; i < m && rank < f.k; ++i) rank += better(s_sc[i], s_row[i], sc, row) ? 1 : 0;
        if (rank < f.k) {
            const double outv = convert_score(sc, f.score_mode);
            if (outv > f.min_score) {
                f.out_idx[(int64_t)q * f.k + rank] = (int64_t)row + f.row_offset;
                f.out_score[(int64_t)q * f.k + rank] = outv;
                atomicMax(s_out, rank + 1);
            }
        }
    }
    __syncthreads();
    const int cntv = *s_out;
    if (tid == 0) f.out_count[q] = cntv;
    for (int t = cntv + tid; t < f.k; t += THREADS) {
        f.out_idx[(int64_t)q * f.k + t] = -1;
        f.out_score[(int64_t)q * f.k + t] = 0.0;
    }
    return cntv;
}

static constexpr uint32_t NO_ROW = 0xFFFFFFFFu;

template <bool NEUMAIER, typename T, int THREADS>
__device__ __forceinline__ void stage_and_chain(const T *__restrict__ rows, int ld, int dim, int kp, const uint32_t *s_rid,
                                                unsigned char *srow, int pitch, const double *sq, double *s_dot, double *s_rr, double *s_qq)
{
    const int tid = threadIdx.x, j = tid;
    const int gpr = ld * (int)sizeof(T) / 16;
    const int c1 = gpr / 3, c2 = 2 * gpr / 3;
#pragma unroll
    for (int c = 0; c < 3; ++c) {
        const int g_lo = c == 0 ? 0 : (c == 1 ? c1 : c2), g_hi = c == 0 ? c1 : (c == 1 ? c2 : gpr);
        const int w = g_hi - g_lo;
        for (int e = tid; e < kp * w; e += THREADS) {
            const int r = e / w, g = g_lo + (e - r * w);
            const uint32_t rid = s_rid[r];
            if (rid != NO_ROW)
                cp_async16(srow + (size_t)r * pitch + (size_t)g * 16,
                           reinterpret_cast<const unsigned char *>(rows + (int64_t)rid * ld) + (size_t)g * 16);
        }
        cp_async_commit();
    }
    const int kind = j < kp ? 0 : (j < 2 * kp ? 1 : ((j == 2 * kp && s_qq != nullptr) ? 2 : 3));
    const int cidx = kind == 0 ? j : (kind == 1 ? j - kp : 0);
    const bool active = kind == 2 || (kind < 2 && s_rid[cidx] != NO_ROW);
    const T *mine = reinterpret_cast<const T *>(srow + (size_t)cidx * pitch);
    constexpr int EPG = 16 / (int)sizeof(T);
    RefSum acc;
    acc.init();
#pragma unroll
    for (int c = 0; c < 3; ++c) {
        if (c == 0) cp_async_wait<2>();
        else if (c == 1) cp_async_wait<1>();
        else cp_async_wait<0>();
        __syncthreads();
        const int g_lo = c == 0 ? 0 : (c == 1 ? c1 : c2), g_hi = c == 0 ? c1 : (c == 1 ? c2 : gpr);
        const int i_lo = g_lo * EPG, i_hi = min(g_hi * EPG, dim);
        if (active) {
            if (kind == 0)
                ref_sum_range<NEUMAIER>(acc, i_lo, i_hi, [&](int i) { return __dmul_rn(sq[i], load_elem(mine, i)); });
            else if (kind == 1)
                ref_sum_range<NEUMAIER>(acc, i_lo, i_hi, [&](int i) { const double y = load_elem(mine, i); return __dmul_rn(y, y); });
            else
                ref_sum_range<NEUMAIER>(acc, i_lo, i_hi, [&](int i) { const double x = sq[i]; return __dmul_rn(x, x); });
        }
    }
    if (active) {
        const double r = acc.result<NEUMAIER>();
        if (kind == 0) s_dot[cidx] = r;
        else if (kind == 1) s_rr[cidx] = r;
        else *s_qq = r;
    }
    __syncthreads();
}

struct SelectSrc {
    const uint64_t *cand;
    int lists, list_len;
    int complete;
    const uint64_t *slab;
    const int *scnt;
    int ctas;
    const uint64_t *ubuf;
    const int *ucnt;
    int ucap;
    const uint32_t *seed_tab;
    int nq_pad, ksel;
    float band;
    int key_cap;
    int band_cap;
};

template <int THREADS>
__device__ int load_slab_keys(const SelectSrc &src, int q, int nq, uint64_t *skeys, int *s_cnts, int *s_total, float *s_bf, bool *incomplete)
{
    const int tid = threadIdx.x, lane = tid & 31, warp = tid >> 5;
    if (warp == 0) {
        float Lb = -INFINITY;
        if (src.seed_tab != nullptr) {
            if (src.ctas >= src.ksel) Lb = seed_select(src.seed_tab, src.ctas, src.nq_pad, q, src.ksel, lane);
            const uint32_t o = __ldcg(src.seed_tab + SEED_TAB_WORDS + q);
            if (o != 0u) Lb = fmaxf(Lb, f32_from_ordered(o));
        }
        if (lane == 0) { *s_bf = band_floor(Lb, src.band); *s_total = 0; }
    }
    for (int c = tid; c < src.ctas; c += THREADS) s_cnts[c] = min(src.scnt[(size_t)c * nq + q], SCAN_SLAB);
    __syncthreads();
    const float bf = *s_bf;
    constexpr int WARPS = THREADS / 32, PER = SCAN_SLAB / 32, BATCH = 4;
    for (int c0 = warp; c0 < src.ctas; c0 += WARPS * BATCH) {
        uint64_t kk[BATCH][PER];
#pragma unroll
        for (int b = 0; b < BATCH; ++b) {
            const int c = c0 + b * WARPS;
            const int cnt = c < src.ctas ? s_cnts[c] : 0;
#pragma unroll
            for (int t = 0; t < PER; ++t)
                kk[b][t] = (lane + 32 * t < cnt) ? __ldcg(src.slab + ((size_t)c * nq + q) * SCAN_SLAB + lane + 32 * t) : 0ull;
        }
#pragma unroll
        for (int b = 0; b < BATCH; ++b)
#pragma unroll
            for (int t = 0; t < PER; ++t) {
                const uint64_t k = kk[b][t];
                if (k != 0 && key_score(k) >= bf) {
                    const int p = atomicAdd(s_total, 1);
                    if (p < src.key_cap) skeys[p] = k;
                }
            }
    }
    const int spilled = src.ucnt[q];
    const int ns = min(spilled, src.ucap);
    for (int e = tid; e < ns; e += THREADS) {
        const uint64_t k = __ldcg(src.ubuf + (size_t)q * src.ucap + e);
        if (k != 0 && key_score(k) >= bf) {
            const int p = atomicAdd(s_total, 1);
            if (p < src.key_cap) skeys[p] = k;
        }
    }
    __syncthreads();
    const int got = *s_total;
    *incomplete = spilled > src.ucap || got > src.key_cap;
    return min(got, src.key_cap);
}

__global__ void __launch_bounds__(SR_THREADS) slab_top_kernel(SelectSrc src, int nq, int kp, uint64_t *__restrict__ merged,
                                                             int *__restrict__ incomplete)
{
    extern __shared__ __align__(16) unsigned char st_smem[];
    uint64_t *skeys = reinterpret_cast<uint64_t *>(st_smem);
    __shared__ int s_cnts[256];
    __shared__ int s_total, s_bin, s_need, s_m;
    __shared__ int hist[256];
    __shared__ float s_bf;
    const int q = blockIdx.x, tid = threadIdx.x;
    bool inc = false;
    const int total = load_slab_keys<SR_THREADS>(src, q, nq, skeys, s_cnts, &s_total, &s_bf, &inc);
    for (int e = tid; e < kp; e += SR_THREADS) merged[(int64_t)q * kp + e] = 0;
    if (tid == 0) { incomplete[q] = inc ? 1 : 0; s_m = 0; }
    __syncthreads();
    if (total <= MERGE_SURV) {
        for (int e = tid; e < total; e += SR_THREADS) {
            const uint64_t k = skeys[e];
            int rank = 0;
            for (int i = 0; i < total; ++i) rank += skeys[i] > k ? 1 : 0;
            if (rank < kp) merged[(int64_t)q * kp + rank] = k;
        }
        return;
    }
    const uint64_t Tk = radix_select_kth(skeys, total, kp, hist, &s_bin, &s_need);
    for (int e = tid; e < total; e += SR_THREADS) {
        const uint64_t k = skeys[e];
        if (k > Tk) merged[(int64_t)q * kp + atomicAdd(&s_m, 1)] = k;
        else if (k == Tk) merged[(int64_t)q * kp + kp - 1] = k;
    }
}

template <bool NEUMAIER, typename T>
__global__ void __launch_bounds__(SR_THREADS, 1) select_rescore_kernel(SelectSrc src, int nq, int kp,
                                                                   const T *__restrict__ rows, int ld, int dim, int64_t n_rows,
                                                                   const void *__restrict__ queries, int q_dtype, double eps,
                                                                   FinalizeArgs f, int32_t *__restrict__ flags,
                                                                   int32_t *__restrict__ uncertified_count,
                                                                   const int *__restrict__ extreme, float *__restrict__ collect_thr,
                                                                   unsigned long long *__restrict__ cum, const float *__restrict__ inv_norms)
{
    extern __shared__ __align__(16) unsigned char sr_smem[];
    uint64_t *skeys = reinterpret_cast<uint64_t *>(sr_smem);
    uint32_t *lmax = reinterpret_cast<uint32_t *>(skeys + src.key_cap);
    double *sq = reinterpret_cast<double *>(lmax + ((src.lists + 3) & ~3));
    const int pitch = ld * (int)sizeof(T) + 16;
    unsigned char *srow = reinterpret_cast<unsigned char *>(sq + ((dim + 1) & ~1));
    double *b_sc = reinterpret_cast<double *>(srow + (((size_t)kp * pitch + 15) & ~(size_t)15));
    uint32_t *b_row = reinterpret_cast<uint32_t *>(b_sc + src.band_cap);
    __shared__ uint64_t s_top[64];
    __shared__ uint32_t s_rid[64];
    __shared__ uint64_t surv[MERGE_SURV];
    __shared__ int hist[256];
    __shared__ int s_bin, s_need, s_m, s_nz, s_cnt, s_band, s_viol, s_out, s_total;
    __shared__ int s_cnts[256];
    __shared__ uint32_t s_L;
    __shared__ float s_thr, s_bf;
    __shared__ double s_dot[64], s_rr[64], s_qq, s_score[64];
    const int q = blockIdx.x, tid = threadIdx.x, lane = tid & 31, warp = tid >> 5;

    pdl_launch_dependents();
    if (tid == 0) { s_m = 0; s_nz = 0; s_cnt = 0; s_band = 0; s_viol = 0; s_thr = -INFINITY; }
    if (tid < 64) s_top[tid] = 0;
    pdl_wait();
    __syncthreads();

    const bool union_mode = src.slab != nullptr;
    int total, lists = src.lists, list_len = src.list_len;
    bool overflow = false;
    int nz = 0;
    if (union_mode) {
        total = load_slab_keys<SR_THREADS>(src, q, nq, skeys, s_cnts, &s_total, &s_bf, &overflow);
        lists = 0;
        if (tid == 0) nz = total;
    } else {
        total = lists * list_len;
#pragma unroll 10
        for (int e = tid; e < total; e += SR_THREADS) {
            const int l = e / list_len, j = e - l * list_len;
            const uint64_t k = src.cand[((int64_t)l * nq + q) * list_len + j];
            skeys[e] = k;
            nz += k != 0;
        }
    }
    for (int i = tid; i < dim; i += SR_THREADS) sq[i] = load_as_double(queries, q_dtype, (int64_t)q * dim + i);
    if (nz) atomicAdd(&s_nz, nz);
    __syncthreads();
    const int nonzero = s_nz;
    bool done = false;
    if (total <= MERGE_SURV) {
        for (int e = tid; e < total; e += SR_THREADS) {
            const uint64_t k = skeys[e];
            if (k == 0) continue;
            int rank = 0;
            for (int i = 0; i < total; ++i) rank += skeys[i] > k ? 1 : 0;
            if (rank < kp) s_top[rank] = k;
        }
        done = true;
    } else if (nonzero >= kp && lists >= kp && lists <= 256) {
        for (int l = warp; l < lists; l += SR_THREADS / 32) {
            uint32_t m = 0;
            for (int j = lane; j < list_len; j += 32) m = max(m, (uint32_t)(skeys[l * list_len + j] >> 32));
            m = __reduce_max_sync(0xffffffffu, m);
            if (lane == 0) lmax[l] = m;
        }
        __syncthreads();
        if (warp == 0) {
            uint32_t vals[8];
#pragma unroll
            for (int t = 0; t < 8; ++t) vals[t] = (lane + 32 * t) < lists ? lmax[lane + 32 * t] : 0u;
            uint32_t prefix = 0;
            int need = kp;
            for (int bit = 31; bit >= 12; --bit) {
                const uint32_t hi = bit == 31 ? 0u : (0xFFFFFFFFu << (bit + 1));
                int cnt = 0;
#pragma unroll
                for (int t = 0; t < 8; ++t) cnt += ((vals[t] & hi) == prefix && ((vals[t] >> bit) & 1u)) ? 1 : 0;
                const int tot = __reduce_add_sync(0xffffffffu, cnt);
                if (tot >= need) prefix |= 1u << bit;
                else need -= tot;
            }
            if (lane == 0) s_L = prefix;
        }
        __syncthreads();
        const uint32_t Lb = s_L;
        if (Lb != 0) {
            for (int e = tid; e < total; e += SR_THREADS) {
                const uint64_t k = skeys[e];
                if ((uint32_t)(k >> 32) >= Lb && k != 0) {
                    const int p = atomicAdd(&s_m, 1);
                    if (p < MERGE_SURV) surv[p] = k;
                }
            }
            __syncthreads();
            const int m = s_m;
            if (m >= kp && m <= MERGE_SURV) {
                for (int e = tid; e < m; e += SR_THREADS) {
                    const uint64_t k = surv[e];
                    int rank = 0;
                    for (int i = 0; i < m; ++i) rank += surv[i] > k ? 1 : 0;
                    if (rank < kp) s_top[rank] = k;
                }
                done = true;
            }
        }
    }
    if (!done) {
        __syncthreads();
        uint64_t Tk = 1;
        if (nonzero >= kp) Tk = radix_select_kth(skeys, total, kp, hist, &s_bin, &s_need);
        if (tid == 0) s_m = 0;
        __syncthreads();
        for (int e = tid; e < total; e += SR_THREADS) {
            const uint64_t k = skeys[e];
            if (k >= Tk && k != 0) {
                if (nonzero >= kp && k == Tk) s_top[kp - 1] = k;
                else s_top[atomicAdd(&s_m, 1)] = k;
            }
        }
    }
    __syncthreads();

    const int j = tid;
    const uint64_t mykey = j < 64 ? s_top[j] : 0;
    const bool cand_valid = j < kp && mykey != 0;
    if (j < 64) s_rid[j] = cand_valid ? key_row(mykey) : NO_ROW;
    __syncthreads();
    stage_and_chain<NEUMAIER, T, SR_THREADS>(rows, ld, dim, kp, s_rid, srow, pitch, sq, s_dot, s_rr, &s_qq);

    double sc = 0.0;
    const uint32_t row = cand_valid ? key_row(mykey) : 0;
    const double n1 = __dsqrt_rn(s_qq);
    if (n1 == 0.0) {
        if (tid == 0) {
            int c = 0;
            const double outv = convert_score(0.0, f.score_mode);
            if (outv > f.min_score)
                for (int64_t r = 0; r < n_rows && c < f.k; ++r)
                    if (__ldg(inv_norms + r) >= 0.0f) {
                        f.out_idx[(int64_t)q * f.k + c] = r + f.row_offset;
                        f.out_score[(int64_t)q * f.k + c] = outv;
                        ++c;
                    }
            for (int t = c; t < f.k; ++t) { f.out_idx[(int64_t)q * f.k + t] = -1; f.out_score[(int64_t)q * f.k + t] = 0.0; }
            f.out_count[q] = c;
            flags[q] = 0;
            if (collect_thr) collect_thr[q] = INFINITY;
        }
        return;
    }
    if (cand_valid) {
        const double n2 = __dsqrt_rn(s_rr[j]);
        sc = (n1 == 0.0 || n2 == 0.0) ? 0.0 : __ddiv_rn(s_dot[j], __dmul_rn(n1, n2));
        if (fabs((double)key_score(mykey) - sc) > eps) atomicAdd(&s_viol, 1);
    }
    if (j < 64) s_score[j] = sc;
    __syncthreads();
    int ncand = 0;
    for (int i = 0; i < kp; ++i) ncand += s_top[i] != 0;
    int rank = 0;
    if (cand_valid)
        for (int i = 0; i < kp; ++i)
            if (s_top[i] != 0 && i != j && better(s_score[i], key_row(s_top[i]), sc, row)) ++rank;
    const double outv = convert_score(sc, f.score_mode);
    const bool emit = cand_valid && rank < f.k && outv > f.min_score;
    if (emit) {
        f.out_idx[(int64_t)q * f.k + rank] = (int64_t)row + f.row_offset;
        f.out_score[(int64_t)q * f.k + rank] = outv;
        atomicAdd(&s_cnt, 1);
    }
    if (cand_valid && ncand >= f.k && rank == f.k - 1) {
        float t = (float)(sc - eps);
        t = nextafterf(nextafterf(t, -INFINITY), -INFINITY);
        s_thr = t;
    }
    __syncthreads();
    const float thr = s_thr;
    {
        int inb = 0;
        for (int e = tid; e < total; e += SR_THREADS) {
            const uint64_t k = skeys[e];
            inb += (k != 0 && key_score(k) >= thr) ? 1 : 0;
        }
        if (inb) atomicAdd(&s_band, inb);
    }
    __syncthreads();
    const int band = s_band;
    const bool bound_ok = !(extreme && *extreme != 0) && s_viol == 0;
    const bool src_complete = union_mode ? !overflow : (src.complete != 0);
    bool cert;
    if (src_complete) cert = band <= ncand;
    else if (union_mode) cert = false;
    else cert = ncand < kp || band < kp;
    if (!bound_ok && (int64_t)ncand < n_rows) cert = false;
    if (ncand == 0) cert = true;
    if (cert) {
        if (tid == 0) {
            flags[q] = 0;
            if (collect_thr) collect_thr[q] = INFINITY;
            f.out_count[q] = s_cnt;
        }
        const int cnt = s_cnt;
        for (int t = cnt + tid; t < f.k; t += SR_THREADS) {
            f.out_idx[(int64_t)q * f.k + t] = -1;
            f.out_score[(int64_t)q * f.k + t] = 0.0;
        }
        return;
    }
    if (tid == 0 && cum) { atomicAdd(cum, 1ull); if (s_viol) atomicAdd(cum + 4, 1ull); }
    if (bound_ok && src_complete && band <= src.band_cap) {
        if (tid == 0) s_m = 0;
        __syncthreads();
        for (int e = tid; e < total; e += SR_THREADS) {
            const uint64_t k = skeys[e];
            if (k != 0 && key_score(k) >= thr) b_row[atomicAdd(&s_m, 1)] = key_row(k);
        }
        __syncthreads();
        for (int b0 = 0; b0 < band; b0 += kp) {
            const int cnt = min(kp, band - b0);
            if (tid < 64) s_rid[tid] = tid < cnt ? b_row[b0 + tid] : NO_ROW;
            __syncthreads();
            stage_and_chain<NEUMAIER, T, SR_THREADS>(rows, ld, dim, kp, s_rid, srow, pitch, sq, s_dot, s_rr, nullptr);
            if (tid < cnt) {
                const double n2 = __dsqrt_rn(s_rr[tid]);
                b_sc[b0 + tid] = (n1 == 0.0 || n2 == 0.0) ? 0.0 : __ddiv_rn(s_dot[tid], __dmul_rn(n1, n2));
            }
            __syncthreads();
        }
        band_emit<SR_THREADS>(band, b_sc, b_row, &s_out, f, q);
        if (tid == 0) {
            flags[q] = 0;
            if (collect_thr) collect_thr[q] = INFINITY;
            if (cum) atomicAdd(cum + 1, 1ull);
        }
        return;
    }
    if (tid == 0) {
        flags[q] = bound_ok ? 1 : 2;
        if (collect_thr) {
            float t = thr > -INFINITY ? (float)((double)thr - eps) : -INFINITY;
            t = nextafterf(t, -INFINITY);
            collect_thr[q] = bound_ok ? t : INFINITY;
        }
        atomicAdd(uncertified_count, 1);
        f.out_count[q] = s_cnt;
    }
    const int cnt = s_cnt;
    for (int t = cnt + tid; t < f.k; t += SR_THREADS) {
        f.out_idx[(int64_t)q * f.k + t] = -1;
        f.out_score[(int64_t)q * f.k + t] = 0.0;
    }
}

static constexpr int CR_THREADS = 512;
template <bool NEUMAIER, typename T>
__global__ void __launch_bounds__(CR_THREADS, 1) collect_rescore_kernel(const uint64_t *__restrict__ buf, const int *__restrict__ cnt, int cap,
                                                                       const T *__restrict__ rows, int ld, int dim,
                                                                       const void *__restrict__ queries, int q_dtype, FinalizeArgs f,
                                                                       int32_t *__restrict__ flags, int32_t *__restrict__ uncertified_count,
                                                                       int nq, unsigned long long *__restrict__ cum, int stage_rows)
{
    extern __shared__ __align__(16) unsigned char cr_smem[];
    double *sq = reinterpret_cast<double *>(cr_smem);
    double *s_sc = sq + ((dim + 1) & ~1);
    double *s_rr = s_sc + cap;
    uint32_t *s_row = reinterpret_cast<uint32_t *>(s_sc + (stage_rows > 0 ? cap : 2 * cap));
    const int pitch = ld * (int)sizeof(T) + 16;
    unsigned char *srow = reinterpret_cast<unsigned char *>(s_row + ((cap + 3) & ~3));
    __shared__ double s_n1;
    __shared__ int s_out;
    __shared__ uint32_t s_rid[64];
    __shared__ double s_dot[64], s_r2[64];
    const int q = blockIdx.x, tid = threadIdx.x;
    if (flags[nq] == 0 || flags[q] != 1) return;
    const int m = cnt[q];
    if (m > cap) {
        if (tid == 0) flags[q] = 2;
        return;
    }
    for (int i = tid; i < dim; i += CR_THREADS) sq[i] = load_as_double(queries, q_dtype, (int64_t)q * dim + i);
    for (int e = tid; e < m; e += CR_THREADS) s_row[e] = key_row(buf[(size_t)q * cap + e]);
    __syncthreads();
    if (tid == 0) {
        RefSum qq; qq.init();
        ref_sum_range<NEUMAIER>(qq, 0, dim, [&](int i) { return __dmul_rn(sq[i], sq[i]); });
        s_n1 = __dsqrt_rn(qq.result<NEUMAIER>());
    }
    __syncthreads();
    if (stage_rows > 0) {
        const double n1 = s_n1;
        for (int b0 = 0; b0 < m; b0 += stage_rows) {
            const int c = min(stage_rows, m - b0);
            if (tid < 64) s_rid[tid] = tid < c ? s_row[b0 + tid] : NO_ROW;
            __syncthreads();
            stage_and_chain<NEUMAIER, T, CR_THREADS>(rows, ld, dim, stage_rows, s_rid, srow, pitch, sq, s_dot, s_r2, nullptr);
            if (tid < c) {
                const double n2 = __dsqrt_rn(s_r2[tid]);
                s_sc[b0 + tid] = (n1 == 0.0 || n2 == 0.0) ? 0.0 : __ddiv_rn(s_dot[tid], __dmul_rn(n1, n2));
            }
            __syncthreads();
        }
    } else {
        band_score_global<NEUMAIER, T, CR_THREADS>(rows, ld, dim, sq, s_n1, m, s_sc, s_rr, s_row);
    }
    band_emit<CR_THREADS>(m, s_sc, s_row, &s_out, f, q);
    if (tid == 0) {
        flags[q] = 0;
        atomicSub(uncertified_count, 1);
        if (cum) atomicAdd(cum + 2, 1ull);
    }
}

#define XK 64

template <int THREADS>
__device__ void exact_merge_query(const double *__restrict__ xlist_score, const uint32_t *__restrict__ xlist_row,
                                  const int32_t *__restrict__ xlist_cnt, int lists, int nq, int k, int q, const FinalizeArgs &f,
                                  uint8_t *__restrict__ taken, double *w_s, uint32_t *w_r, int *w_p, int *s_out)
{
    const int tid = threadIdx.x, lane = tid & 31, warp = tid >> 5;
    const int total = lists * k;
    uint8_t *tk = taken + (int64_t)q * total;
    for (int e = tid; e < total; e += THREADS) tk[e] = 0;
    if (tid == 0) *s_out = 0;
    __syncthreads();
    auto scan_local = [&](double &bs, uint32_t &br, int &bp) {
        bp = -1; bs = 0.0; br = 0;
        for (int e = tid; e < total; e += THREADS) {
            int l = e / k, j = e - l * k;
            if (tk[e] || j >= xlist_cnt[(int64_t)l * nq + q]) continue;
            int64_t g = ((int64_t)l * nq + q) * k + j;
            double s = xlist_score[g];
            uint32_t r = xlist_row[g];
            if (bp < 0 || better(s, r, bs, br)) { bs = s; br = r; bp = e; }
        }
    };
    double bs; uint32_t br; int bp;
    scan_local(bs, br, bp);
    for (int r = 0; r < f.k; ++r) {
        double ms = bs; uint32_t mr = br; int mp = bp;
        for (int o = 16; o > 0; o >>= 1) {
            double ts = __shfl_xor_sync(0xffffffffu, ms, o);
            uint32_t tr = __shfl_xor_sync(0xffffffffu, mr, o);
            int tp = __shfl_xor_sync(0xffffffffu, mp, o);
            if (tp >= 0 && (mp < 0 || better(ts, tr, ms, mr))) { ms = ts; mr = tr; mp = tp; }
        }
        if (lane == 0) { w_s[warp] = ms; w_r[warp] = mr; w_p[warp] = mp; }
        __syncthreads();
        ms = w_s[0]; mr = w_r[0]; mp = w_p[0];
        for (int w = 1; w < THREADS / 32; ++w)
            if (w_p[w] >= 0 && (mp < 0 || better(w_s[w], w_r[w], ms, mr))) { ms = w_s[w]; mr = w_r[w]; mp = w_p[w]; }
        if (mp < 0) break;
        double outv = convert_score(ms, f.score_mode);
        if (tid == 0 && outv > f.min_score) {
            f.out_idx[(int64_t)q * f.k + r] = (int64_t)mr + f.row_offset;
            f.out_score[(int64_t)q * f.k + r] = outv;
            *s_out = r + 1;
        }
        if (mp == bp) {
            tk[bp] = 1;
            scan_local(bs, br, bp);
        }
        __syncthreads();
    }
    __syncthreads();
    int cnt = *s_out;
    if (tid == 0) f.out_count[q] = cnt;
    for (int t = cnt + tid; t < f.k; t += THREADS) {
        f.out_idx[(int64_t)q * f.k + t] = -1;
        f.out_score[(int64_t)q * f.k + t] = 0.0;
    }
    __syncthreads();
}

static constexpr int XS_THREADS = 256;
static constexpr int XS_CG = 24;
static constexpr int XS_PITCH = XS_CG * 16 + 16;

template <bool NEUMAIER, typename T>
__global__ void __launch_bounds__(XS_THREADS) exact_scan_kernel(const T *__restrict__ rows, const float *__restrict__ inv_norms,
                                                               int64_t n, int ld, int dim, const void *__restrict__ queries,
                                                               int q_dtype, int nq, int32_t *__restrict__ flags, int k,
                                                               double *__restrict__ xlist_score, uint32_t *__restrict__ xlist_row,
                                                               int32_t *__restrict__ xlist_cnt, unsigned long long *__restrict__ cum,
                                                               int *__restrict__ done_ctr, FinalizeArgs f, uint8_t *__restrict__ taken)
{
    pdl_launch_dependents();
    pdl_wait();
    if (flags && flags[nq] == 0) return;
    if (flags && cum && blockIdx.x == 0 && threadIdx.x == 0) atomicAdd(cum + 3, (unsigned long long)flags[nq]);
    extern __shared__ __align__(16) unsigned char xs_smem[];
    double *sq = reinterpret_cast<double *>(xs_smem);
    unsigned char *buf0 = reinterpret_cast<unsigned char *>(sq + ((dim + 1) & ~1));
    __shared__ double l_score[XK], n_score[XK];
    __shared__ uint32_t l_row[XK], n_row[XK];
    __shared__ double c_score[128];
    __shared__ uint32_t c_row[128];
    __shared__ double s_dotv[128], s_rrv[128];
    __shared__ int l_cnt, c_cnt;
    __shared__ double s_n1;
    const int tid = threadIdx.x, rt = tid & 127;
    const bool is_rr = tid >= 128;
    const int gpr = ld * (int)sizeof(T) / 16;
    const int nchunks = (gpr + XS_CG - 1) / XS_CG;
    constexpr int EPG = 16 / (int)sizeof(T);
    for (int q = 0; q < nq; ++q) {
        if (flags && flags[q] == 0) continue;
        __syncthreads();
        for (int i = tid; i < dim; i += XS_THREADS) sq[i] = load_as_double(queries, q_dtype, (int64_t)q * dim + i);
        if (tid == 0) { l_cnt = 0; c_cnt = 0; }
        __syncthreads();
        if (tid == 0) {
            RefSum qq; qq.init();
            ref_sum_range<NEUMAIER>(qq, 0, dim, [&](int i) { return __dmul_rn(sq[i], sq[i]); });
            s_n1 = __dsqrt_rn(qq.result<NEUMAIER>());
        }
        __syncthreads();
        const double n1 = s_n1;
        const int64_t ntiles = (n + 127) / 128;
        const int my_tiles = (int)((ntiles - blockIdx.x + gridDim.x - 1) / gridDim.x);
        const int total_steps = my_tiles > 0 ? my_tiles * nchunks : 0;
        auto issue = [&](int st) {
            if (st < total_steps) {
                const int64_t tile = blockIdx.x + (int64_t)(st / nchunks) * gridDim.x;
                const int c = st % nchunks;
                unsigned char *buf = buf0 + (size_t)(st % 3) * 128 * XS_PITCH;
                const int g0 = c * XS_CG, gw = min(XS_CG, gpr - g0);
                for (int e = tid; e < 128 * gw; e += XS_THREADS) {
                    const int rr_ = e / gw, g = e - rr_ * gw;
                    const int64_t row = tile * 128 + rr_;
                    if (row < n)
                        cp_async16(buf + (size_t)rr_ * XS_PITCH + (size_t)g * 16,
                                   reinterpret_cast<const unsigned char *>(rows + row * (int64_t)ld) + (size_t)(g0 + g) * 16);
                }
            }
            cp_async_commit();
        };
        issue(0);
        issue(1);
        RefSum acc;
        acc.init();
        for (int st = 0; st < total_steps; ++st) {
            const int64_t tile = blockIdx.x + (int64_t)(st / nchunks) * gridDim.x;
            const int c = st % nchunks;
            const int64_t r = tile * 128 + rt;
            const bool live = r < n && inv_norms[r] >= 0.0f;
            issue(st + 2);
            cp_async_wait<2>();
            __syncthreads();
            const unsigned char *cur = buf0 + (size_t)(st % 3) * 128 * XS_PITCH;
            const int i_lo = c * XS_CG * EPG, i_hi = min((c + 1) * XS_CG * EPG, dim);
            if (live && i_lo < i_hi) {
                const T *mine = reinterpret_cast<const T *>(cur + (size_t)rt * XS_PITCH);
                if (!is_rr)
                    ref_sum_range<NEUMAIER>(acc, i_lo, i_hi, [&](int i) { return __dmul_rn(sq[i], load_elem(mine, i - i_lo)); });
                else
                    ref_sum_range<NEUMAIER>(acc, i_lo, i_hi, [&](int i) { const double y = load_elem(mine, i - i_lo); return __dmul_rn(y, y); });
            }
            if (c + 1 < nchunks) {
                __syncthreads();
                continue;
            }
            if (live) { if (is_rr) s_rrv[rt] = acc.result<NEUMAIER>(); else s_dotv[rt] = acc.result<NEUMAIER>(); }
            acc.init();
            __syncthreads();
            double sc = 0.0;
            bool hit = false;
            if (live && !is_rr) {
                const double n2 = __dsqrt_rn(s_rrv[rt]);
                sc = (n1 == 0.0 || n2 == 0.0) ? 0.0 : __ddiv_rn(s_dotv[rt], __dmul_rn(n1, n2));
                const int lc = l_cnt;
                hit = lc < k || better(sc, (uint32_t)r, l_score[lc - 1], l_row[lc - 1]);
            }
            if (hit) {
                const int p = atomicAdd(&c_cnt, 1);
                c_score[p] = sc;
                c_row[p] = (uint32_t)r;
            }
            const int cc = __syncthreads_count(hit ? 1 : 0);
            const int lc = l_cnt;
            if (cc > 0) {
                for (int e = tid; e < lc + cc; e += XS_THREADS) {
                    const double se = e < lc ? l_score[e] : c_score[e - lc];
                    const uint32_t re = e < lc ? l_row[e] : c_row[e - lc];
                    int rank = 0;
                    for (int i = 0; i < lc; ++i) rank += better(l_score[i], l_row[i], se, re) ? 1 : 0;
                    for (int i = 0; i < cc; ++i) rank += better(c_score[i], c_row[i], se, re) ? 1 : 0;
                    if (rank < k) { n_score[rank] = se; n_row[rank] = re; }
                }
                __syncthreads();
                const int nl = min(k, lc + cc);
                for (int e = tid; e < nl; e += XS_THREADS) { l_score[e] = n_score[e]; l_row[e] = n_row[e]; }
                if (tid == 0) { l_cnt = nl; c_cnt = 0; }
                __syncthreads();
            }
        }
        cp_async_wait<0>();
        __syncthreads();
        const int lc = l_cnt;
        const int64_t base = ((int64_t)blockIdx.x * nq + q) * k;
        for (int e = tid; e < lc; e += XS_THREADS) { xlist_score[base + e] = l_score[e]; xlist_row[base + e] = l_row[e]; }
        if (tid == 0) xlist_cnt[(int64_t)blockIdx.x * nq + q] = lc;
    }
    if (done_ctr == nullptr) return;
    __shared__ int s_last, s_out;
    __shared__ double w_s[XS_THREADS / 32];
    __shared__ uint32_t w_r[XS_THREADS / 32];
    __shared__ int w_p[XS_THREADS / 32];
    __threadfence();
    __syncthreads();
    if (tid == 0) s_last = atomicAdd(done_ctr, 1) == (int)gridDim.x - 1;
    __syncthreads();
    if (!s_last) return;
    __threadfence();
    for (int q = 0; q < nq; ++q) {
        if (flags[q] == 0) continue;
        exact_merge_query<XS_THREADS>(xlist_score, xlist_row, xlist_cnt, (int)gridDim.x, nq, k, q, f, taken, w_s, w_r, w_p, &s_out);
        if (tid == 0) flags[q] = 0;
    }
    if (tid == 0) { *done_ctr = 0; flags[nq] = 0; }
}

__global__ void __launch_bounds__(256) exact_merge_kernel(const double *__restrict__ xlist_score, const uint32_t *__restrict__ xlist_row,
                                                         const int32_t *__restrict__ xlist_cnt, int lists, int nq, int k,
                                                         const int32_t *__restrict__ flags, FinalizeArgs f, uint8_t *__restrict__ taken)
{
    __shared__ double w_s[8];
    __shared__ uint32_t w_r[8];
    __shared__ int w_p[8];
    __shared__ int s_out;
    const int q = blockIdx.x;
    if (flags && (flags[nq] == 0 || flags[q] == 0)) return;
    exact_merge_query<256>(xlist_score, xlist_row, xlist_cnt, lists, nq, k, q, f, taken, w_s, w_r, w_p, &s_out);
}

__global__ void __launch_bounds__(256) merge_topk_lists_kernel(const char *__restrict__ idx_b, const char *__restrict__ score_b,
                                                              const char *__restrict__ count_b, size_t stride, int lists, int nq, int k,
                                                              int64_t *__restrict__ out_idx, double *__restrict__ out_score,
                                                              int32_t *__restrict__ out_count)
{
    extern __shared__ unsigned char smem_raw[];
    const int q = blockIdx.x, tid = threadIdx.x;
    const int total = lists * k;
    double *s_s = (double *)smem_raw;
    int64_t *s_i = (int64_t *)(s_s + total);
    int *s_v = (int *)(s_i + total);
    for (int e = tid; e < total; e += 256) {
        int l = e / k, j = e - l * k;
        const int64_t *idx = (const int64_t *)(idx_b + (size_t)l * stride);
        const double *score = (const double *)(score_b + (size_t)l * stride);
        const int32_t *count = (const int32_t *)(count_b + (size_t)l * stride);
        int64_t g = (int64_t)q * k + j;
        bool v = j < count[q];
        s_s[e] = v ? score[g] : 0.0;
        s_i[e] = v ? idx[g] : -1;
        s_v[e] = v ? 1 : 0;
    }
    __syncthreads();
    int nvalid = 0;
    for (int e = 0; e < total; ++e) nvalid += s_v[e];
    for (int e = tid; e < total; e += 256) {
        if (!s_v[e]) continue;
        int rank = 0;
        for (int i = 0; i < total; ++i)
            if (s_v[i] && (s_s[i] > s_s[e] || (s_s[i] == s_s[e] && s_i[i] < s_i[e]))) ++rank;
        if (rank < k) { out_idx[(int64_t)q * k + rank] = s_i[e]; out_score[(int64_t)q * k + rank] = s_s[e]; }
    }
    int cnt = min(nvalid, k);
    if (tid == 0) out_count[q] = cnt;
    for (int t = cnt + tid; t < k; t += 256) { out_idx[(int64_t)q * k + t] = -1; out_score[(int64_t)q * k + t] = 0.0; }
}

struct PeerPtrs { const unsigned char *p[16]; };

__global__ void p2p_publish_kernel(unsigned long long *flag, unsigned long long gen)
{
    __threadfence_system();
    asm volatile("st.release.sys.global.u64 [%0], %1;" ::"l"(flag), "l"(gen) : "memory");
}

__global__ void __launch_bounds__(256) merge_topk_p2p_kernel(PeerPtrs peers, int nranks, size_t slot_off, size_t flag_off,
                                                            unsigned long long gen, int nq, int k,
                                                            int64_t *__restrict__ out_idx, double *__restrict__ out_score,
                                                            int32_t *__restrict__ out_count)
{
    extern __shared__ unsigned char smem_raw[];
    const int q = blockIdx.x, tid = threadIdx.x;
    const int total = nranks * k;
    double *s_s = (double *)smem_raw;
    int64_t *s_i = (int64_t *)(s_s + total);
    int *s_v = (int *)(s_i + total);
    if (tid < nranks) {
        const unsigned long long *f = reinterpret_cast<const unsigned long long *>(peers.p[tid] + flag_off);
        unsigned long long v;
        const long long t0 = clock64();
        for (;;) {
            asm volatile("ld.acquire.sys.global.u64 %0, [%1];" : "=l"(v) : "l"(f) : "memory");
            if (v >= gen) break;
            if (clock64() - t0 > 4000000000LL) { printf("vidmem: peer %d never published batch %llu\n", tid, gen); __trap(); }
        }
    }
    __syncthreads();
    for (int e = tid; e < total; e += 256) {
        const int l = e / k, j = e - l * k;
        const unsigned char *b = peers.p[l] + slot_off;
        const int64_t *idx = reinterpret_cast<const int64_t *>(b);
        const double *score = reinterpret_cast<const double *>(b + (size_t)nq * k * 8);
        const int32_t *count = reinterpret_cast<const int32_t *>(b + (size_t)nq * k * 16);
        const bool v = j < __ldcv(count + q);
        s_s[e] = v ? __ldcv(score + (size_t)q * k + j) : 0.0;
        s_i[e] = v ? __ldcv(idx + (size_t)q * k + j) : -1;
        s_v[e] = v ? 1 : 0;
    }
    __syncthreads();
    int nvalid = 0;
    for (int e = 0; e < total; ++e) nvalid += s_v[e];
    for (int e = tid; e < total; e += 256) {
        if (!s_v[e]) continue;
        int rank = 0;
        for (int i = 0; i < total; ++i)
            if (s_v[i] && (s_s[i] > s_s[e] || (s_s[i] == s_s[e] && s_i[i] < s_i[e]))) ++rank;
        if (rank < k) { out_idx[(int64_t)q * k + rank] = s_i[e]; out_score[(int64_t)q * k + rank] = s_s[e]; }
    }
    const int cnt = min(nvalid, k);
    if (tid == 0) out_count[q] = cnt;
    for (int t = cnt + tid; t < k; t += 256) { out_idx[(int64_t)q * k + t] = -1; out_score[(int64_t)q * k + t] = 0.0; }
}

__global__ void __launch_bounds__(256) merge_max_by_id_kernel(const int64_t *__restrict__ idx, const double *__restrict__ score,
                                                             const int32_t *__restrict__ count, int nq, int k, int k2,
                                                             int64_t *__restrict__ out_idx, double *__restrict__ out_score,
                                                             int32_t *__restrict__ out_count)
{
    extern __shared__ unsigned char smem_raw[];
    const int tid = threadIdx.x, total = nq * k;
    double *s_s = (double *)smem_raw;
    int64_t *s_i = (int64_t *)(s_s + total);
    int *s_rep = (int *)(s_i + total);
    __shared__ int s_n;
    if (tid == 0) s_n = 0;
    for (int e = tid; e < total; e += 256) {
        int qi = e / k, j = e - qi * k;
        bool v = j < count[qi];
        s_i[e] = v ? idx[e] : -1;
        s_s[e] = v ? score[e] : 0.0;
        s_rep[e] = 0;
    }
    __syncthreads();
    for (int e = tid; e < total; e += 256) {
        if (s_i[e] < 0) continue;
        bool first = true;
        for (int i = 0; i < e; ++i)
            if (s_i[i] == s_i[e]) { first = false; break; }
        if (!first) continue;
        double m = s_s[e];
        for (int i = e + 1; i < total; ++i)
            if (s_i[i] == s_i[e] && score[i] > m) m = score[i];
        s_rep[e] = 1;
        s_s[e] = m;
        atomicAdd(&s_n, 1);
    }
    __syncthreads();
    for (int e = tid; e < total; e += 256) {
        if (!s_rep[e]) continue;
        int rank = 0;
        for (int i = 0; i < total; ++i)
            if (s_rep[i] && (s_s[i] > s_s[e] || (s_s[i] == s_s[e] && i < e))) ++rank;
        if (rank < k2) { out_idx[rank] = s_i[e]; out_score[rank] = s_s[e]; }
    }
    if (tid == 0) *out_count = min(s_n, k2);
}

template <bool NEUMAIER>
__global__ void cosine_pairs_kernel(const void *__restrict__ a, const void *__restrict__ b, int dtype, int64_t n, int dim,
                                    int zero_rule, double *__restrict__ out)
{
    int64_t i = blockIdx.x * (int64_t)blockDim.x + threadIdx.x;
    if (i >= n) return;
    RefSum dot, aa, bb;
    dot.init(); aa.init(); bb.init();
    for (int c = 0; c < dim; ++c) {
        double x = load_as_double(a, dtype, i * dim + c), y = load_as_double(b, dtype, i * dim + c);
        dot.add<NEUMAIER>(__dmul_rn(x, y));
        aa.add<NEUMAIER>(__dmul_rn(x, x));
        bb.add<NEUMAIER>(__dmul_rn(y, y));
    }
    double n1, n2;
    if (zero_rule == 2) { n1 = pow(aa.result<NEUMAIER>(), 0.5); n2 = pow(bb.result<NEUMAIER>(), 0.5); }
    else { n1 = __dsqrt_rn(aa.result<NEUMAIER>()); n2 = __dsqrt_rn(bb.result<NEUMAIER>()); }
    double den = __dmul_rn(n1, n2);
    bool zero = zero_rule == 1 ? (den == 0.0) : (n1 == 0.0 || n2 == 0.0);
    out[i] = zero ? 0.0 : __ddiv_rn(dot.result<NEUMAIER>(), den);
}

int k_merge_candidates(const uint64_t *cand, int lists, int nq, int kp, uint64_t *merged, cudaStream_t st)
{
    size_t smem = (size_t)lists * kp * sizeof(uint64_t) + (size_t)lists * sizeof(uint32_t) + 16;
    VM_CUDA_CHECK((max_smem_once<merge_candidates_kernel>(200 * 1024)));
    VM_REQUIRE(smem <= 200 * 1024, VM_ERR_UNSUPPORTED, "candidate merge: %d lists x %d exceeds shared memory", lists, kp);
    merge_candidates_kernel<<<nq, MERGE_THREADS, smem, st>>>(cand, lists, nq, kp, merged);
    VM_CUDA_CHECK(cudaGetLastError());
    return VM_OK;
}


template <typename F>
static int with_sum_mode(int sum_mode, F &&f)
{
    return sum_mode == VM_SUM_NEUMAIER ? f(std::true_type{}) : f(std::false_type{});
}

template <typename F>
static int with_row_type(int dtype, int sum_mode, F &&f)
{
    auto by_sum = [&](auto *tag) { return with_sum_mode(sum_mode, [&](auto neu) { return f(neu, tag); }); };
    if (dtype == VM_F32) return by_sum((float *)nullptr);
    if (dtype == VM_F64) return by_sum((double *)nullptr);
    return by_sum((__nv_bfloat16 *)nullptr);
}

int k_rescore(const RescoreArgs &a, cudaStream_t st, const int *incomplete)
{
    const int ssz = a.dtype == VM_F64 ? 8 : 4;
    int chunk = RS_SMEM_ROW_BYTES / (ssz * a.kp) - 1;
    chunk &= ~7;
    if (chunk > a.ld) chunk = a.ld;
    const size_t smem = (size_t)chunk * sizeof(double) + (size_t)a.kp * (chunk + 1) * ssz + 16;
    return with_row_type(a.dtype, a.sum_mode, [&](auto neu, auto *tag) -> int {
        using T = std::remove_pointer_t<decltype(tag)>;
        constexpr bool NEU = decltype(neu)::value;
        VM_CUDA_CHECK((max_smem_once<rescore_kernel<NEU, T>>(160 * 1024)));
        rescore_kernel<NEU, T><<<a.nq, RS_THREADS, smem, st>>>(a.merged, a.kp, (const T *)a.rows, a.inv_norms, a.ld, a.dim,
                                                               a.n_rows, a.queries, a.q_dtype, a.eps, a.fin, a.flags,
                                                               a.uncertified_count, chunk, a.extreme, a.collect_thr, a.cum, incomplete);
        VM_CUDA_CHECK(cudaGetLastError());
        return VM_OK;
    });
}


static constexpr size_t SR_SMEM_LIMIT = 180 * 1024;
static size_t select_rescore_base_smem(int key_cap, int lists, int kp, int dtype, int dim, int ld)
{
    const int es = (int)dtype_size(dtype);
    const size_t rows_area = (((size_t)kp * ((size_t)ld * es + 16) + 15) & ~(size_t)15) + 16;
    return (size_t)key_cap * 8 + (size_t)((lists + 3) & ~3) * 4 + (size_t)((dim + 1) & ~1) * 8 + rows_area + 32;
}
static int select_band_cap(int key_cap, int lists, int kp, int dtype, int dim, int ld)
{
    const size_t base = select_rescore_base_smem(key_cap, lists, kp, dtype, dim, ld);
    if (base + (size_t)BAND_CAP_MIN * 12 > SR_SMEM_LIMIT) return 0;
    size_t cap = (SR_SMEM_LIMIT - base) / 12;
    cap &= ~(size_t)63;
    if (cap > (size_t)BAND_CAP_MAX) cap = BAND_CAP_MAX;
    return (int)cap;
}
bool select_rescore_fits(int lists, int list_len, int kp, int dtype, int dim, int ld)
{
    const int key_cap = lists > 0 ? lists * list_len : SELECT_KEY_CAP;
    return select_band_cap(key_cap, lists, kp, dtype, dim, ld) >= BAND_CAP_MIN && kp <= 64 && 2 * kp + 1 <= SR_THREADS;
}

static SelectSrc make_src(const SelectArgs &sa)
{
    const bool slab_mode = sa.slab != nullptr;
    const int lists = slab_mode ? 0 : sa.lists;
    return SelectSrc{sa.cand, lists, sa.list_len, sa.complete, sa.slab, sa.scnt, sa.ctas, sa.ubuf, sa.ucnt, sa.ucap, sa.seed_tab,
                     sa.nq_pad, sa.ksel, sa.band, slab_mode ? SELECT_KEY_CAP : lists * sa.list_len, 0};
}

int k_select_rescore(const SelectArgs &sa, const RescoreArgs &a, cudaStream_t st, bool pdl)
{
    SelectSrc src = make_src(sa);
    VM_REQUIRE(src.slab == nullptr || src.ctas <= 256, VM_ERR_UNSUPPORTED, "select: %d scan CTAs exceed 256", src.ctas);
    if (!select_rescore_fits(src.lists, src.list_len, a.kp, a.dtype, a.dim, a.ld)) return VM_ERR_UNSUPPORTED;
    src.band_cap = select_band_cap(src.key_cap, src.lists, a.kp, a.dtype, a.dim, a.ld);
    const size_t smem = select_rescore_base_smem(src.key_cap, src.lists, a.kp, a.dtype, a.dim, a.ld) + (size_t)src.band_cap * 12;
    return with_row_type(a.dtype, a.sum_mode, [&](auto neu, auto *tag) -> int {
        using T = std::remove_pointer_t<decltype(tag)>;
        constexpr bool NEU = decltype(neu)::value;
        VM_CUDA_CHECK((max_smem_once<select_rescore_kernel<NEU, T>>(180 * 1024)));
        VM_CUDA_CHECK(launch_pdl(select_rescore_kernel<NEU, T>, dim3(a.nq), dim3(SR_THREADS), smem, st, pdl, src, a.nq, a.kp,
                                 (const T *)a.rows, a.ld, a.dim, a.n_rows, a.queries, a.q_dtype, a.eps, a.fin, a.flags,
                                 a.uncertified_count, a.extreme, a.collect_thr, a.cum, a.inv_norms));
        VM_CUDA_CHECK(cudaGetLastError());
        return VM_OK;
    });
}

int k_slab_top(const SelectArgs &sa, int nq, int kp, uint64_t *merged, int *incomplete, cudaStream_t st)
{
    const SelectSrc src = make_src(sa);
    VM_REQUIRE(src.slab != nullptr && src.ctas <= 256, VM_ERR_UNSUPPORTED, "slab selection: bad source");
    slab_top_kernel<<<nq, SR_THREADS, (size_t)src.key_cap * 8, st>>>(src, nq, kp, merged, incomplete);
    VM_CUDA_CHECK(cudaGetLastError());
    return VM_OK;
}

int k_collect_rescore(const uint64_t *buf, const int *cnt, int cap, const RescoreArgs &a, cudaStream_t st)
{
    const size_t head = (size_t)((a.dim + 1) & ~1) * 8;
    const size_t staged = head + (size_t)cap * 8 + (size_t)((cap + 3) & ~3) * 4 + (size_t)32 * ((size_t)a.ld * dtype_size(a.dtype) + 16) + 64;
    const int stage_rows = staged <= 200 * 1024 ? 32 : 0;
    const size_t smem = stage_rows ? staged : head + (size_t)cap * (8 + 8 + 4) + 32;
    VM_REQUIRE(smem <= 200 * 1024, VM_ERR_UNSUPPORTED, "collect pass: buffer of %d rows exceeds shared memory", cap);
    return with_row_type(a.dtype, a.sum_mode, [&](auto neu, auto *tag) -> int {
        using T = std::remove_pointer_t<decltype(tag)>;
        constexpr bool NEU = decltype(neu)::value;
        VM_CUDA_CHECK((max_smem_once<collect_rescore_kernel<NEU, T>>(200 * 1024)));
        collect_rescore_kernel<NEU, T><<<a.nq, CR_THREADS, smem, st>>>(buf, cnt, cap, (const T *)a.rows, a.ld, a.dim, a.queries,
                                                                       a.q_dtype, a.fin, a.flags, a.uncertified_count, a.nq, a.cum, stage_rows);
        VM_CUDA_CHECK(cudaGetLastError());
        return VM_OK;
    });
}

int k_exact(const ExactArgs &a, cudaStream_t st, bool pdl)
{
    VM_REQUIRE((size_t)a.dim * sizeof(double) <= 40 * 1024, VM_ERR_UNSUPPORTED, "exact scan: dim %d too large", a.dim);
    const size_t smem = (size_t)((a.dim + 1) & ~1) * sizeof(double) + (size_t)3 * 128 * XS_PITCH + 16;
    const bool conditional = a.flags != nullptr && a.done_ctr != nullptr;
    const int rc = with_row_type(a.dtype, a.sum_mode, [&](auto neu, auto *tag) -> int {
        using T = std::remove_pointer_t<decltype(tag)>;
        constexpr bool NEU = decltype(neu)::value;
        VM_CUDA_CHECK((max_smem_once<exact_scan_kernel<NEU, T>>(200 * 1024)));
        VM_CUDA_CHECK(launch_pdl(exact_scan_kernel<NEU, T>, dim3(a.ctas), dim3(XS_THREADS), smem, st, pdl && conditional, (const T *)a.rows,
                                 a.inv_norms, a.n, a.ld, a.dim, a.queries, a.q_dtype, a.nq, a.flags, a.k, a.xlist_score, a.xlist_row,
                                 a.xlist_cnt, a.cum, conditional ? a.done_ctr : (int *)nullptr, a.fin, a.taken));
        VM_CUDA_CHECK(cudaGetLastError());
        return VM_OK;
    });
    if (rc != VM_OK || conditional) return rc;
    exact_merge_kernel<<<a.nq, 256, 0, st>>>(a.xlist_score, a.xlist_row, a.xlist_cnt, a.ctas, a.nq, a.k, a.flags, a.fin, a.taken);
    VM_CUDA_CHECK(cudaGetLastError());
    return VM_OK;
}

int k_merge_topk_lists(const void *idx, const void *score, const void *count, size_t stride_bytes, int lists, int nq, int k,
                       int64_t *out_idx, double *out_score, int32_t *out_count, cudaStream_t st)
{
    int total = lists * k;
    VM_REQUIRE(total <= 4096, VM_ERR_UNSUPPORTED, "merge_topk_lists: lists*k = %d > 4096", total);
    size_t smem = (size_t)total * (8 + 8 + 4);
    VM_CUDA_CHECK((max_smem_once<merge_topk_lists_kernel>(100 * 1024)));
    merge_topk_lists_kernel<<<nq, 256, smem, st>>>((const char *)idx, (const char *)score, (const char *)count, stride_bytes, lists, nq, k,
                                                  out_idx, out_score, out_count);
    VM_CUDA_CHECK(cudaGetLastError());
    return VM_OK;
}

int k_p2p_publish(void *flag, unsigned long long gen, cudaStream_t st)
{
    p2p_publish_kernel<<<1, 1, 0, st>>>((unsigned long long *)flag, gen);
    VM_CUDA_CHECK(cudaGetLastError());
    return VM_OK;
}

int k_merge_topk_p2p(void *const *peers, int nranks, size_t slot_off, size_t flag_off, unsigned long long gen, int nq, int k,
                     int64_t *out_idx, double *out_score, int32_t *out_count, cudaStream_t st)
{
    VM_REQUIRE(nranks >= 1 && nranks <= 16, VM_ERR_UNSUPPORTED, "peer exchange supports up to 16 ranks");
    const int total = nranks * k;
    VM_REQUIRE(total <= 4096, VM_ERR_UNSUPPORTED, "merge: nranks*k = %d > 4096", total);
    PeerPtrs pp{};
    for (int r = 0; r < nranks; ++r) pp.p[r] = (const unsigned char *)peers[r];
    const size_t smem = (size_t)total * (8 + 8 + 4);
    VM_CUDA_CHECK((max_smem_once<merge_topk_p2p_kernel>(100 * 1024)));
    merge_topk_p2p_kernel<<<nq, 256, smem, st>>>(pp, nranks, slot_off, flag_off, gen, nq, k, out_idx, out_score, out_count);
    VM_CUDA_CHECK(cudaGetLastError());
    return VM_OK;
}

int k_merge_max_by_id(const int64_t *idx, const double *score, const int32_t *count, int nq, int k, int k2,
                      int64_t *out_idx, double *out_score, int32_t *out_count, cudaStream_t st)
{
    int total = nq * k;
    VM_REQUIRE(total <= 4096, VM_ERR_UNSUPPORTED, "merge_max_by_id: nq*k = %d > 4096", total);
    size_t smem = (size_t)total * (8 + 8 + 4);
    VM_CUDA_CHECK((max_smem_once<merge_max_by_id_kernel>(100 * 1024)));
    merge_max_by_id_kernel<<<1, 256, smem, st>>>(idx, score, count, nq, k, k2, out_idx, out_score, out_count);
    VM_CUDA_CHECK(cudaGetLastError());
    return VM_OK;
}

int k_cosine_pairs(const void *a, const void *b, int dtype, int64_t n, int dim, int zero_rule, int sum_mode, double *out,
                   cudaStream_t st)
{
    if (n <= 0) return VM_OK;
    int grid = (int)((n + 127) / 128);
    return with_sum_mode(sum_mode, [&](auto neu) -> int {
        cosine_pairs_kernel<decltype(neu)::value><<<grid, 128, 0, st>>>(a, b, dtype, n, dim, zero_rule, out);
        VM_CUDA_CHECK(cudaGetLastError());
        return VM_OK;
    });
}

}
```

real-time-brain-inspired-video-memory_b200/csrc/store.cu:

```cuda
#include "common.cuh"
#include "synth.cuh"

namespace vm {

template <typename DST>
__global__ void convert_rows_kernel(const void *__restrict__ src, int src_dtype, DST *__restrict__ dst, int64_t n,
                                    int dim, int ld)
{
    int64_t total = n * (int64_t)ld;
    for (int64_t e = blockIdx.x * (int64_t)blockDim.x + threadIdx.x; e < total; e += (int64_t)gridDim.x * blockDim.x) {
        int64_t r = e / ld;
        int c = (int)(e - r * ld);
        double dv = 0.0;
        if (c < dim) dv = load_as_double(src, src_dtype, r * dim + c);
        if constexpr (sizeof(DST) == 8) dst[e] = dv;
        else {
            const float v = (float)dv;
            if constexpr (sizeof(DST) == 4) dst[e] = v;
            else dst[e] = __float2bfloat16_rn(v);
        }
    }
}

template <typename T>
__global__ void row_inv_norms_kernel(const T *__restrict__ rows, float *__restrict__ inv_norms, int64_t row0,
                                     int64_t n, int ld, int *__restrict__ extreme, const double *__restrict__ exact)
{
    int lane = threadIdx.x & 31;
    int64_t warp = (blockIdx.x * (int64_t)blockDim.x + threadIdx.x) >> 5;
    int64_t nwarps = ((int64_t)gridDim.x * blockDim.x) >> 5;
    for (int64_t r = row0 + warp; r < n; r += nwarps) {
        const T *p = rows + r * (int64_t)ld;
        double ss = 0.0;
        for (int c = lane; c < ld; c += 32) {
            double v = (double)load_as_float(p, c);
            ss += v * v;
        }
        for (int o = 16; o > 0; o >>= 1) ss += __shfl_xor_sync(0xffffffffu, ss, o);
        double se = 0.0;
        if (exact != nullptr) {
            for (int c = lane; c < ld; c += 32) {
                const double v = exact[r * (int64_t)ld + c] * 0x1p-600;
                se += v * v;
            }
            for (int o = 16; o > 0; o >>= 1) se += __shfl_xor_sync(0xffffffffu, se, o);
        }
        if (lane == 0) {
            float inv = 0.0f;
            if (!isfinite(ss)) {
                inv = -1.0f;
                if (exact != nullptr && isfinite(se)) { inv = 0.0f; if (extreme) atomicAdd(extreme, 1); }
            } else if (ss > 0.0) {
                inv = (float)(1.0 / sqrt(ss));
                if (extreme && (ss < 7.52316384526264e-37 || ss > 1.329227995784916e+36)) atomicAdd(extreme, 1);
            } else if (exact != nullptr && se != 0.0) {
                if (extreme) atomicAdd(extreme, 1);
            }
            inv_norms[r] = inv;
        }
    }
}

__global__ void invalidate_rows_kernel(float *inv_norms, const int64_t *rows, int64_t n, int64_t size)
{
    int64_t i = blockIdx.x * (int64_t)blockDim.x + threadIdx.x;
    if (i < n && rows[i] >= 0 && rows[i] < size) inv_norms[rows[i]] = -1.0f;
}

__global__ void normalize_queries_kernel(const void *__restrict__ q, int q_dtype, int nq, int nq_pad, int dim, int ld,
                                         float *__restrict__ out_f32, __nv_bfloat16 *__restrict__ out_bf16,
                                         int32_t *__restrict__ zero_me, uint32_t *__restrict__ zero_tab, int zero_tab_n,
                                         int tf32_round, int split)
{
    pdl_launch_dependents();
    pdl_wait();
    if (zero_me && blockIdx.x == 0 && threadIdx.x < 2) zero_me[threadIdx.x] = 0;
    for (int i = blockIdx.x * blockDim.x + threadIdx.x; i < zero_tab_n; i += gridDim.x * blockDim.x) zero_tab[i] = 0u;
    int lane = threadIdx.x & 31;
    int w = (blockIdx.x * blockDim.x + threadIdx.x) >> 5;
    if (w >= nq_pad) return;
    double ss = 0.0;
    if (w < nq)
        for (int c = lane; c < dim; c += 32) {
            double v = load_as_double(q, q_dtype, (int64_t)w * dim + c);
            ss += v * v;
        }
    for (int o = 16; o > 0; o >>= 1) ss += __shfl_xor_sync(0xffffffffu, ss, o);
    double inv = (ss > 0.0 && isfinite(ss)) ? 1.0 / sqrt(ss) : 0.0;
    for (int c = lane; c < ld; c += 32) {
        float v = 0.0f;
        if (w < nq && c < dim) v = (float)(load_as_double(q, q_dtype, (int64_t)w * dim + c) * inv);
        float vf = v;
        if (tf32_round) vf = __uint_as_float((__float_as_uint(v) + 0x1000u) & 0xFFFFE000u);
        out_f32[(int64_t)w * ld + c] = vf;
        if (out_bf16) {
            const __nv_bfloat16 hi = __float2bfloat16_rn(v);
            out_bf16[(int64_t)w * ld + c] = hi;
            if (split) out_bf16[((int64_t)nq_pad + w) * ld + c] = __float2bfloat16_rn(v - __bfloat162float(hi));
        }
    }
}

template <typename T>
__global__ void synth_fill_kernel(T *__restrict__ rows, uint64_t seed, int64_t row0, int64_t n, int dim, int ld,
                                  uint64_t dup_period)
{
    int groups = ld >> 3;
    int64_t total = n * (int64_t)groups;
    uint64_t hk = splitmix64(seed ^ 0xD6E8FEB86659FD93ULL);
    for (int64_t e = blockIdx.x * (int64_t)blockDim.x + threadIdx.x; e < total; e += (int64_t)gridDim.x * blockDim.x) {
        int64_t i = e / groups;
        int g = (int)(e - i * groups);
        uint64_t row = (uint64_t)(row0 + i);
        uint64_t own = splitmix64(splitmix64(seed * 0x9E3779B97F4A7C15ULL + row) + (uint64_t)g);
        uint64_t par = 0, sel = 0;
        bool planted = false;
        if (dup_period > 0 && row > 0) {
            uint64_t hr = splitmix64(hk + row);
            if (hr % dup_period == 0) {
                planted = true;
                uint64_t parent = splitmix64(hr) % row;
                par = splitmix64(splitmix64(seed * 0x9E3779B97F4A7C15ULL + parent) + (uint64_t)g);
                sel = splitmix64(hr + 0x632BE59BD9B4E019ULL + (uint64_t)g);
            }
        }
        T *dst = rows + i * (int64_t)ld + g * 8;
#pragma unroll
        for (int b = 0; b < 8; ++b) {
            int col = g * 8 + b;
            int v = synth_int(own, b);
            if (planted && (((sel >> (8 * b)) & 15ULL) != 0ULL)) v = synth_int(par, b);
            float f = col < dim ? (float)v * (1.0f / 128.0f) : 0.0f;
            if constexpr (sizeof(T) == 4) dst[b] = f;
            else dst[b] = __float2bfloat16_rn(f);
        }
    }
}

int k_convert_rows(const void *src, int src_dtype, void *dst, int dst_dtype, int64_t n, int dim, int ld, cudaStream_t st)
{
    if (n <= 0) return VM_OK;
    int64_t total = n * (int64_t)ld;
    int grid = (int)vm::imin64((total + 255) / 256, 148 * 16);
    if (dst_dtype == VM_F32) convert_rows_kernel<float><<<grid, 256, 0, st>>>(src, src_dtype, (float *)dst, n, dim, ld);
    else if (dst_dtype == VM_F64) convert_rows_kernel<double><<<grid, 256, 0, st>>>(src, src_dtype, (double *)dst, n, dim, ld);
    else convert_rows_kernel<__nv_bfloat16><<<grid, 256, 0, st>>>(src, src_dtype, (__nv_bfloat16 *)dst, n, dim, ld);
    VM_CUDA_CHECK(cudaGetLastError());
    return VM_OK;
}

int k_row_inv_norms(const void *rows, int dtype, float *inv_norms, int64_t row0, int64_t n, int ld, int *extreme, cudaStream_t st,
                    const double *exact)
{
    if (n <= row0) return VM_OK;
    int64_t warps = n - row0;
    int grid = (int)vm::imin64((warps * 32 + 255) / 256, 148 * 16);
    if (dtype == VM_F32) row_inv_norms_kernel<float><<<grid, 256, 0, st>>>((const float *)rows, inv_norms, row0, n, ld, extreme, exact);
    else row_inv_norms_kernel<__nv_bfloat16><<<grid, 256, 0, st>>>((const __nv_bfloat16 *)rows, inv_norms, row0, n, ld, extreme, exact);
    VM_CUDA_CHECK(cudaGetLastError());
    return VM_OK;
}

int k_invalidate_rows(float *inv_norms, const int64_t *rows_dev, int64_t n, int64_t size, cudaStream_t st)
{
    if (n <= 0) return VM_OK;
    invalidate_rows_kernel<<<(int)((n + 255) / 256), 256, 0, st>>>(inv_norms, rows_dev, n, size);
    VM_CUDA_CHECK(cudaGetLastError());
    return VM_OK;
}

int k_normalize_queries(const void *q, int q_dtype, int nq, int nq_pad, int dim, int ld, float *out_f32,
                        void *out_bf16, int32_t *zero_me, uint32_t *zero_tab, int zero_tab_n, int tf32_round, int split, bool pdl,
                        cudaStream_t st)
{
    int threads = 128;
    int grid = (nq_pad * 32 + threads - 1) / threads;
    VM_CUDA_CHECK(launch_pdl(normalize_queries_kernel, dim3(grid), dim3(threads), 0, st, pdl, q, q_dtype, nq, nq_pad, dim, ld, out_f32,
                             (__nv_bfloat16 *)out_bf16, zero_me, zero_tab, zero_tab_n, tf32_round, split));
    VM_CUDA_CHECK(cudaGetLastError());
    return VM_OK;
}

int k_synth_fill(void *rows, int dtype, uint64_t seed, int64_t row0, int64_t n, int dim, int ld, uint64_t dup_period,
                 cudaStream_t st)
{
    if (n <= 0) return VM_OK;
    int64_t total = n * (int64_t)(ld >> 3);
    int grid = (int)vm::imin64((total + 255) / 256, 148 * 32);
    if (dtype == VM_F32) synth_fill_kernel<float><<<grid, 256, 0, st>>>((float *)rows, seed, row0, n, dim, ld, dup_period);
    else synth_fill_kernel<__nv_bfloat16><<<grid, 256, 0, st>>>((__nv_bfloat16 *)rows, seed, row0, n, dim, ld, dup_period);
    VM_CUDA_CHECK(cudaGetLastError());
    return VM_OK;
}

}
```

Baseline: 263,300.

## Add dynamic tile scheduling, early service-warp exit, warp-parallel slab loading, and step stamps

The tensor-core scan kernel now claims tiles from a global atomic counter and hands them to the MMA and epilogue warps through an smem ring of mbarriers, replacing static strided tile assignment. This is meant to balance load across CTAs. The service warp now breaks out of its loop and sleeps in short slices once the epilogue finishes, which shortens the kernel tail. Slab key loading in select is spread across several warps instead of one warp gathering counts first. Optional compile-time timestamp instrumentation is also added, and the seed-block offsets are renamed. The changes add atomic and mbarrier traffic per tile, and the tile counter's reset logic is not visible here.

```diff
diff --git a/real-time-brain-inspired-video-memory_b200/csrc/api.cu b/real-time-brain-inspired-video-memory_b200/csrc/api.cu
--- a/real-time-brain-inspired-video-memory_b200/csrc/api.cu
+++ b/real-time-brain-inspired-video-memory_b200/csrc/api.cu
@@ -117,6 +117,9 @@
     bool ready = false;
     int lists_max = 0;
     Buf q_raw, q_f32, q_bf16, seed, cand, merged, o_idx, flags, col_thr, col_cnt, col_buf, xs, xr, xc, taken, gather_send, gather_recv, misc, ubuf, done, scnt, sel_inc;
+#ifdef VIDMEM_STEP_STAMPS
+    Buf stamps;
+#endif
     int32_t *h_uncert = nullptr;
     unsigned char *h_pack = nullptr;
     unsigned char *h_q = nullptr;
@@ -125,6 +128,9 @@
         Buf *all[] = {&q_raw, &q_f32, &q_bf16, &seed, &cand, &merged, &o_idx, &flags, &col_thr, &col_cnt, &col_buf, &xs, &xr, &xc, &taken,
                       &gather_send, &gather_recv, &misc, &ubuf, &done, &scnt, &sel_inc};
         for (Buf *b : all) b->release();
+#ifdef VIDMEM_STEP_STAMPS
+        stamps.release();
+#endif
         if (h_uncert) cudaFreeHost(h_uncert);
         if (h_pack) cudaFreeHost(h_pack);
         if (h_q) cudaFreeHost(h_q);
@@ -255,7 +261,8 @@
     ENS(w.merged, (size_t)MAXQ * MAXK * 8);
     ENS(w.o_idx, result_bytes(MAXQ, MAXK) + 64);
     ENS(w.flags, (size_t)(MAXQ + 2) * 4);
-    ENS(w.seed, (size_t)(SEED_TAB_WORDS + 3 * MAXQ) * 4);
+    static_assert(MAXQ <= 64, "the seed block holds 64 bounds / spill counters");
+    ENS(w.seed, (size_t)SEED_WORDS * 4);
     ENS(w.ubuf, (size_t)MAXQ * SCAN_UNION_CAP * 8);
     ENS(w.done, 64);
     ENS(w.scnt, (size_t)256 * MAXQ * 4);
@@ -268,6 +275,14 @@
     ENS(w.xr, (size_t)XCTAS * MAXQ * MAXK * 4);
     ENS(w.xc, (size_t)XCTAS * MAXQ * 4);
     ENS(w.taken, (size_t)MAXQ * XCTAS * MAXK);
+#ifdef VIDMEM_STEP_STAMPS
+    ENS(w.stamps, (size_t)STAMP_SLOTS * 16);
+    VM_CUDA_CHECK(cudaMemset(w.stamps.p, 0, w.stamps.bytes));
+    {
+        unsigned long long *sp = (unsigned long long *)w.stamps.p;
+        if ((rc = stamps_bind_store(sp)) != VM_OK || (rc = stamps_bind_scan(sp)) != VM_OK || (rc = stamps_bind_select(sp)) != VM_OK) return rc;
+    }
+#endif
 #undef ENS
     VM_CUDA_CHECK(cudaMallocHost((void **)&w.h_uncert, 64));
     VM_CUDA_CHECK(cudaMallocHost((void **)&w.h_pack, result_bytes(MAXQ, MAXK) + 64));
@@ -602,7 +617,7 @@
     VM_CUDA_CHECK(cudaDeviceSynchronize());
     std::vector<int> sc((size_t)ctas * nq), uc(nq);
     VM_CUDA_CHECK(cudaMemcpy(sc.data(), s->ws.scnt.p, sc.size() * 4, cudaMemcpyDeviceToHost));
-    VM_CUDA_CHECK(cudaMemcpy(uc.data(), (int *)s->ws.seed.p + SEED_TAB_WORDS + 2 * MAXQ, (size_t)nq * 4, cudaMemcpyDeviceToHost));
+    VM_CUDA_CHECK(cudaMemcpy(uc.data(), (int *)s->ws.seed.p + SEED_SPILL_CNT, (size_t)nq * 4, cudaMemcpyDeviceToHost));
     for (int q = 0; q < nq; ++q) {
         int64_t k = 0;
         for (int c = 0; c < ctas; ++c) k += sc[(size_t)c * nq + q];
@@ -612,6 +627,18 @@
     if (nq_out) *nq_out = nq;
     return VM_OK;
 }
+
+#ifdef VIDMEM_STEP_STAMPS
+extern "C" int vm_step_stamps(vm_store *s, unsigned long long *out, int slots)
+{
+    VM_REQUIRE(s && out && slots >= STAMP_SLOTS && s->ws.ready, VM_ERR_BADARG, "vm_step_stamps: no stamps or buffer too small");
+    VM_CUDA_CHECK(cudaSetDevice(s->device));
+    VM_CUDA_CHECK(cudaDeviceSynchronize());
+    VM_CUDA_CHECK(cudaMemcpy(out, s->ws.stamps.p, (size_t)STAMP_SLOTS * 16, cudaMemcpyDeviceToHost));
+    VM_CUDA_CHECK(cudaMemset(s->ws.stamps.p, 0, (size_t)STAMP_SLOTS * 16));
+    return STAMP_SLOTS;
+}
+#endif
 
 extern "C" int vm_store_read_counters(vm_store *s, vm_store_counters *out, int reset)
 {
@@ -760,7 +787,7 @@
     a.rows = s->rows; a.inv_norms = s->inv_norms; a.dtype = s->dtype; a.n = s->size; a.dim = s->dim; a.ld = s->ld;
     a.queries = (const float *)w.q_f32.p; a.nq = c.nq; a.kp = kp; a.cand = (uint64_t *)w.cand.p; a.stream = st;
     a.slab = (uint64_t *)w.cand.p; a.scnt = (int *)w.scnt.p;
-    a.ubuf = (uint64_t *)w.ubuf.p; a.ucnt = (int *)w.seed.p + SEED_TAB_WORDS + 2 * MAXQ; a.ucap = SCAN_UNION_CAP;
+    a.ubuf = (uint64_t *)w.ubuf.p; a.ucnt = (int *)w.seed.p + SEED_SPILL_CNT; a.ucap = SCAN_UNION_CAP;
     a.band = nextafterf((float)(2.0 * eps), INFINITY); a.ksel = c.k; a.split = split; a.pdl = pdl;
     const bool timing = (c.flags & VM_FLAG_TIMING) != 0;
     if (timing) {
diff --git a/real-time-brain-inspired-video-memory_b200/csrc/common.cuh b/real-time-brain-inspired-video-memory_b200/csrc/common.cuh
--- a/real-time-brain-inspired-video-memory_b200/csrc/common.cuh
+++ b/real-time-brain-inspired-video-memory_b200/csrc/common.cuh
@@ -29,6 +29,32 @@
 __device__ __forceinline__ void pdl_wait() { asm volatile("griddepcontrol.wait;" ::: "memory"); }
 __device__ __forceinline__ void pdl_launch_dependents() { asm volatile("griddepcontrol.launch_dependents;" ::: "memory"); }
 
+static constexpr int STAMP_NORM = 0, STAMP_FIX = 4, STAMP_PER = 8, STAMP_SCAN = 8, STAMP_SEL = STAMP_SCAN + 256 * STAMP_PER,
+                     STAMP_SLOTS = STAMP_SEL + 64 * STAMP_PER;
+enum { STAMP_SCAN_ENTRY, STAMP_SCAN_WAITED, STAMP_SCAN_QFULL, STAMP_SCAN_FIRST_MMA, STAMP_SCAN_EPI_DONE, STAMP_SCAN_SVC_DONE, STAMP_SCAN_EXIT };
+enum { STAMP_SEL_ENTRY, STAMP_SEL_WAITED, STAMP_SEL_KEYS, STAMP_SEL_RANKED, STAMP_SEL_CHAINS, STAMP_SEL_EXIT };
+#ifdef VIDMEM_STEP_STAMPS
+static __device__ unsigned long long *g_stamps;
+__device__ __forceinline__ void step_stamp(int slot)
+{
+    if (!g_stamps) return;
+    unsigned long long t;
+    asm volatile("mov.u64 %0, %%globaltimer;" : "=l"(t));
+    g_stamps[2 * slot] = t;
+    g_stamps[2 * slot + 1] = (unsigned long long)clock64();
+}
+#define VM_STAMP_IF(cond, slot) do { if (cond) ::vm::step_stamp(slot); } while (0)
+#define VM_STAMP_VARS(...) __VA_ARGS__
+#define VM_STAMPS_BINDER(name) \
+    int name(unsigned long long *p) { VM_CUDA_CHECK(cudaMemcpyToSymbol(g_stamps, &p, sizeof(p))); return VM_OK; }
+int stamps_bind_store(unsigned long long *p);
+int stamps_bind_scan(unsigned long long *p);
+int stamps_bind_select(unsigned long long *p);
+#else
+#define VM_STAMP_IF(cond, slot) ((void)0)
+#define VM_STAMP_VARS(...)
+#endif
+
 template <typename... KArgs, typename... Args>
 static inline cudaError_t launch_pdl(void (*kernel)(KArgs...), dim3 grid, dim3 block, size_t smem, cudaStream_t st, bool pdl,
                                      Args &&...args)
@@ -84,6 +110,11 @@
 __host__ __device__ __forceinline__ float key_score(uint64_t k) { return f32_from_ordered((uint32_t)(k >> 32)); }
 
 static constexpr int SEED_TAB_WORDS = 256 * 64;
+static constexpr int SEED_BOUNDS = SEED_TAB_WORDS;
+static constexpr int SEED_PUB_CTR = SEED_TAB_WORDS + 64;
+static constexpr int SEED_TILE_CTR = SEED_TAB_WORDS + 65;
+static constexpr int SEED_SPILL_CNT = SEED_TAB_WORDS + 128;
+static constexpr int SEED_WORDS = SEED_TAB_WORDS + 192;
 #ifdef __CUDACC__
 __device__ __forceinline__ float seed_select(const uint32_t *seed_tab, int G, int nq_pad, int q, int k, int lane)
 {
diff --git a/real-time-brain-inspired-video-memory_b200/csrc/scan_tc.cu b/real-time-brain-inspired-video-memory_b200/csrc/scan_tc.cu
--- a/real-time-brain-inspired-video-memory_b200/csrc/scan_tc.cu
+++ b/real-time-brain-inspired-video-memory_b200/csrc/scan_tc.cu
@@ -10,6 +10,7 @@
 static constexpr int TC_THREADS = 192;
 static constexpr int TC_TMEM_COLS = 512;
 static constexpr int TC_MAX_STAGES = 8;
+static constexpr int TC_TRING = 8;
 
 struct CollectArgs {
     const float *thr;
@@ -44,7 +45,7 @@
     L.split = (split && dtype == VM_BF16) ? 1 : 0;
     uint32_t o = 0;
     L.off_b = o; o += (uint32_t)L.KB * L.nq_pad * 128 * (L.split ? 2 : 1);
-    const uint32_t epi = (uint32_t)L.nq_pad * (4 + 4 + 4 + 16) + 64 + 8 * (2 * TC_MAX_STAGES + 1 + 2 * TC_ACC) + 16;
+    const uint32_t epi = (uint32_t)L.nq_pad * (4 + 4 + 4 + 16) + 64 + 8 * (2 * TC_MAX_STAGES + 1 + 2 * TC_ACC + 2 * TC_TRING) + 16;
     int64_t room = 227 * 1024 - 2048 - (int64_t)o - epi;
     L.stages = (int)(room / TC_STAGE_BYTES);
     if (L.stages > TC_MAX_STAGES) L.stages = TC_MAX_STAGES;
@@ -55,7 +56,7 @@
     L.off_cmax = o; o += (uint32_t)L.nq_pad * 4;
     L.off_wmax = o; o += (uint32_t)L.nq_pad * 16;
     L.off_flags = o; o += 64;
-    L.off_bars = o; o += 8 * (2 * TC_MAX_STAGES + 1 + 2 * TC_ACC);
+    L.off_bars = o; o += 8 * (2 * TC_MAX_STAGES + 1 + 2 * TC_ACC + 2 * TC_TRING);
     L.off_tmem = o; o += 16;
     L.total = o + 1024;
 #ifdef VIDMEM_AB_SMEMPAD
@@ -98,6 +99,8 @@
                uint32_t *__restrict__ seed_tab, int *__restrict__ seed_ctr, CollectArgs col, BandArgs ub, int svc_sleep)
 {
     const bool collect = !DUMP && col.thr != nullptr;
+    VM_STAMP_VARS(const int stamp0 = STAMP_SCAN + STAMP_PER * (int)blockIdx.x; const bool stamps = !collect && blockIdx.x < 256;)
+    VM_STAMP_IF(stamps && threadIdx.x == 0, stamp0 + STAMP_SCAN_ENTRY);
 #ifndef VIDMEM_AB_NOPDL
     pdl_launch_dependents();
 #endif
@@ -118,6 +121,8 @@
     uint64_t *bars = (uint64_t *)(base + L.off_bars);
     uint64_t *full = bars, *empty = bars + TC_MAX_STAGES, *qfull = bars + 2 * TC_MAX_STAGES;
     uint64_t *tfull = qfull + 1, *tempty = tfull + TC_ACC;
+    uint64_t *idfull = tempty + TC_ACC, *idempty = idfull + TC_TRING;
+    volatile int *s_tile = (volatile int *)(base + L.off_flags) + 8;
     uint32_t *tmem_slot = (uint32_t *)(base + L.off_tmem);
 
     const int warp = __shfl_sync(0xffffffffu, threadIdx.x >> 5, 0);
@@ -131,12 +136,14 @@
         for (int s = 0; s < stages; ++s) { mbar_init(&full[s], 1); mbar_init(&empty[s], 1); }
         mbar_init(qfull, 1);
         for (int a = 0; a < TC_ACC; ++a) { mbar_init(&tfull[a], 1); mbar_init(&tempty[a], 4); }
+        if (!DUMP) for (int r = 0; r < TC_TRING; ++r) { mbar_init(&idfull[r], 1); mbar_init(&idempty[r], 5); }
         fence_barrier_init();
     }
     if (warp == 1) tmem_alloc(tmem_slot, TC_TMEM_COLS);
 #ifndef VIDMEM_AB_NOPDL
     if (!collect) pdl_wait();
 #endif
+    VM_STAMP_IF(stamps && threadIdx.x == 0, stamp0 + STAMP_SCAN_WAITED);
     if (warp >= 2 && warp < 6) {
         const int e = threadIdx.x - 64;
         if (e < nq_pad) {
@@ -150,7 +157,16 @@
     __syncthreads();
     tc_fence_after();
     const uint32_t tmem_base = *tmem_slot;
-    uint32_t *gbound = seed_tab ? seed_tab + SEED_TAB_WORDS : nullptr;
+    uint32_t *gbound = seed_tab ? seed_tab + SEED_BOUNDS : nullptr;
+    int *tile_ctr = (!DUMP && !collect && seed_tab) ? reinterpret_cast<int *>(seed_tab + SEED_TILE_CTR) : nullptr;
+    auto next_tile = [&](int i) -> int {
+        const int slot = i & (TC_TRING - 1);
+        mbar_wait(&idfull[slot], (uint32_t)(i / TC_TRING) & 1u);
+        const int t = s_tile[slot];
+        __syncwarp();
+        if (lane == 0) mbar_arrive(&idempty[slot]);
+        return t;
+    };
 
     if (warp == 0) {
         if (elect_one()) {
@@ -163,7 +179,19 @@
         __syncwarp();
         int stage = 0;
         uint32_t phase = 0;
-        for (int tile = blockIdx.x; tile < num_tiles; tile += gridDim.x) {
+        for (int i = 0, tile = blockIdx.x;; ++i) {
+            int claimed = 0;
+            if (tile_ctr && tile < num_tiles && lane == 0) claimed = atomicAdd(tile_ctr, 1);
+            if constexpr (!DUMP) {
+                const int slot = i & (TC_TRING - 1);
+                mbar_wait(&idempty[slot], ((uint32_t)(i / TC_TRING) & 1u) ^ 1u);
+                if (lane == 0) {
+                    s_tile[slot] = tile < num_tiles ? tile : -1;
+                    mbar_arrive(&idfull[slot]);
+                }
+                __syncwarp();
+            }
+            if (tile >= num_tiles) break;
             for (int kb = 0; kb < KB; ++kb) {
                 mbar_wait(&empty[stage], phase ^ 1);
                 if (elect_one()) {
@@ -173,16 +201,18 @@
                 __syncwarp();
                 if (++stage == stages) { stage = 0; phase ^= 1; }
             }
+            tile = tile_ctr ? (int)gridDim.x + __shfl_sync(0xffffffffu, claimed, 0) : tile + (int)gridDim.x;
         }
     } else if (warp == 1) {
         const uint32_t idesc = make_idesc(TF32 ? 2u : 1u, TC_BLOCK_M, (uint32_t)nq_pad);
         mbar_wait(qfull, 0);
         tc_fence_after();
+        VM_STAMP_IF(stamps && lane == 0, stamp0 + STAMP_SCAN_QFULL);
         int stage = 0, acc = 0;
         uint32_t phase = 0, acc_phase = 0;
         const uint64_t da0 = make_smem_desc_sw128(smem_u32(sA)), db0 = make_smem_desc_sw128(smem_u32(sB));
         const uint32_t kb_step = (uint32_t)(nq_pad * 128) >> 4, lo_step = (uint32_t)(KB * nq_pad * 128) >> 4;
-        for (int tile = blockIdx.x; tile < num_tiles; tile += gridDim.x) {
+        for (int i = 0; DUMP ? (int)blockIdx.x + i * (int)gridDim.x < num_tiles : next_tile(i) >= 0; ++i) {
             mbar_wait(&tempty[acc], acc_phase ^ 1);
             tc_fence_after();
             const uint32_t d_tmem = tmem_base + (uint32_t)(acc * nq_pad);
@@ -199,6 +229,7 @@
                     }
                     umma_commit(&empty[stage]);
                     if (kb == KB - 1) umma_commit(&tfull[acc]);
+                    VM_STAMP_IF(stamps && kb == 0 && i == 0, stamp0 + STAMP_SCAN_FIRST_MMA);
                 }
                 __syncwarp();
                 if (++stage == stages) { stage = 0; phase ^= 1; }
@@ -270,7 +301,7 @@
             }
             named_bar_sync(1, 128);
             const int G = (int)gridDim.x;
-            int *pub_ctr = reinterpret_cast<int *>(gbound + 64);
+            int *pub_ctr = reinterpret_cast<int *>(seed_tab + SEED_PUB_CTR);
             if (warp == 2) {
                 for (int q = blockIdx.x; q < nq; q += G) {
                     const float sd = seed_select(seed_tab, G, nq_pad, q, ub.ksel, lane);
@@ -296,11 +327,13 @@
         }
         if (!collect && e == 0) s_done[1] = 1;
         uint64_t *my_slab = collect ? nullptr : ub.slab + (size_t)blockIdx.x * nq * SCAN_SLAB;
-        int64_t row = (int64_t)blockIdx.x * TC_BLOCK_M + row_in_tile;
+        int tile = next_tile(0);
+        int64_t row = (int64_t)tile * TC_BLOCK_M + row_in_tile;
         float inv = row < n ? __ldg(inv_norms + row) : -1.0f;
-        for (int tile = blockIdx.x; tile < num_tiles; tile += gridDim.x) {
-            const int64_t row_next = row + (int64_t)gridDim.x * TC_BLOCK_M;
-            const float inv_next = (tile + (int)gridDim.x < num_tiles && row_next < n) ? __ldg(inv_norms + row_next) : -1.0f;
+        for (int i = 1; tile >= 0; ++i) {
+            const int tile_next = next_tile(i);
+            const int64_t row_next = (int64_t)tile_next * TC_BLOCK_M + row_in_tile;
+            const float inv_next = (tile_next >= 0 && row_next < n) ? __ldg(inv_norms + row_next) : -1.0f;
             const bool valid = inv >= 0.0f;
             mbar_wait(&tfull[acc], acc_phase);
             tc_fence_after();
@@ -370,6 +403,7 @@
             __syncwarp();
             if (lane == 0) mbar_arrive(&tempty[acc]);
             if (++acc == TC_ACC) { acc = 0; acc_phase ^= 1; }
+            tile = tile_next;
             row = row_next;
             inv = inv_next;
         }
@@ -383,6 +417,7 @@
         }
         __syncwarp();
         if (lane == 0) atomicAdd((int *)s_done, 1);
+        VM_STAMP_IF(stamps && e == 0, stamp0 + STAMP_SCAN_EPI_DONE);
     } else {
 #ifdef VIDMEM_AB_NOSVC
         if (false) {
@@ -405,12 +440,14 @@
                     }
                 }
                 __syncwarp();
+                if (__any_sync(0xffffffffu, s_done[0] >= 4)) break;
                 if (G >= ub.ksel)
                     for (int q = blockIdx.x; q < nq; q += G) {
                         const float sd = seed_select(seed_tab, G, nq_pad, q, ub.ksel, lane);
                         if (lane == 0 && sd > -INFINITY) atomicMax(gbound + q, f32_ordered(sd));
                     }
                 __syncwarp();
+                if (__any_sync(0xffffffffu, s_done[0] >= 4)) break;
 #ifndef VIDMEM_AB_KTH_LEVELS
 #define VIDMEM_AB_KTH_LEVELS 2
 #endif
@@ -457,8 +494,9 @@
                         }
                     }
                 }
-                __nanosleep(svc_sleep);
-            }
+                for (int t = 0; t < svc_sleep && s_done[0] < 4; t += 100) __nanosleep(100);
+            }
+            VM_STAMP_IF(stamps && lane == 0, stamp0 + STAMP_SCAN_SVC_DONE);
         }
     }
 
@@ -467,8 +505,13 @@
     if (warp == 1) {
         tc_fence_after();
         tmem_dealloc(tmem_base, TC_TMEM_COLS);
+        VM_STAMP_IF(stamps && lane == 0, stamp0 + STAMP_SCAN_EXIT);
     }
 }
+
+#ifdef VIDMEM_STEP_STAMPS
+VM_STAMPS_BINDER(stamps_bind_scan)
+#endif
 
 bool scan_tc_supported(int dtype, int dim, int nq, int kp, int split)
 {
diff --git a/real-time-brain-inspired-video-memory_b200/csrc/select.cu b/real-time-brain-inspired-video-memory_b200/csrc/select.cu
--- a/real-time-brain-inspired-video-memory_b200/csrc/select.cu
+++ b/real-time-brain-inspired-video-memory_b200/csrc/select.cu
@@ -481,44 +481,62 @@
 };
 
 template <int THREADS>
-__device__ int load_slab_keys(const SelectSrc &src, int q, int nq, uint64_t *skeys, int *s_cnts, int *s_total, float *s_bf, bool *incomplete)
+__device__ int load_slab_keys(const SelectSrc &src, int q, int nq, uint64_t *skeys, int *s_total, float *s_bf, bool *incomplete)
 {
     const int tid = threadIdx.x, lane = tid & 31, warp = tid >> 5;
-    if (warp == 0) {
+    constexpr int LW = THREADS / 32 - 1, PER_WARP = (256 + LW - 1) / LW;
+    static_assert(PER_WARP <= 32, "a warp's slab counts must fit one lane each");
+    static_assert(LW * PER_WARP >= 256, "the loading warps cover every slab of a grid of up to 256 CTAs");
+    const int w = warp - 1;
+    const int my_c = w + lane * LW;
+    const int my_cnt = (warp > 0 && lane < PER_WARP && my_c < src.ctas) ? min(__ldcg(src.scnt + (size_t)my_c * nq + q), SCAN_SLAB) : 0;
+    const int spilled = __ldcg(src.ucnt + q);
+    uint64_t kk[PER_WARP];
+    if (warp > 0) {
+#pragma unroll
+        for (int j = 0; j < PER_WARP; ++j) {
+            const int cnt = __shfl_sync(0xffffffffu, my_cnt, j);
+            kk[j] = lane < cnt ? __ldcg(src.slab + ((size_t)(w + j * LW) * nq + q) * SCAN_SLAB + lane) : 0ull;
+        }
+    } else {
         float Lb = -INFINITY;
         if (src.seed_tab != nullptr) {
             if (src.ctas >= src.ksel) Lb = seed_select(src.seed_tab, src.ctas, src.nq_pad, q, src.ksel, lane);
-            const uint32_t o = __ldcg(src.seed_tab + SEED_TAB_WORDS + q);
+            const uint32_t o = __ldcg(src.seed_tab + SEED_BOUNDS + q);
             if (o != 0u) Lb = fmaxf(Lb, f32_from_ordered(o));
         }
         if (lane == 0) { *s_bf = band_floor(Lb, src.band); *s_total = 0; }
     }
-    for (int c = tid; c < src.ctas; c += THREADS) s_cnts[c] = min(src.scnt[(size_t)c * nq + q], SCAN_SLAB);
     __syncthreads();
     const float bf = *s_bf;
-    constexpr int WARPS = THREADS / 32, PER = SCAN_SLAB / 32, BATCH = 4;
-    for (int c0 = warp; c0 < src.ctas; c0 += WARPS * BATCH) {
-        uint64_t kk[BATCH][PER];
+    auto keep = [&](uint64_t k) {
+        if (k != 0 && key_score(k) >= bf) {
+            const int p = atomicAdd(s_total, 1);
+            if (p < src.key_cap) skeys[p] = k;
+        }
+    };
+    if (warp > 0) {
 #pragma unroll
-        for (int b = 0; b < BATCH; ++b) {
-            const int c = c0 + b * WARPS;
-            const int cnt = c < src.ctas ? s_cnts[c] : 0;
+        for (int j = 0; j < PER_WARP; ++j) keep(kk[j]);
+        constexpr int RB = 6, REST = SCAN_SLAB / 32 - 1;
+        for (int j0 = 0; j0 < PER_WARP; j0 += RB) {
+            if (!__any_sync(0xffffffffu, lane >= j0 && lane < j0 + RB && my_cnt > 32)) continue;
+            uint64_t kr[RB][REST];
 #pragma unroll
-            for (int t = 0; t < PER; ++t)
-                kk[b][t] = (lane + 32 * t < cnt) ? __ldcg(src.slab + ((size_t)c * nq + q) * SCAN_SLAB + lane + 32 * t) : 0ull;
-        }
+            for (int b = 0; b < RB; ++b) {
+                const int cnt = __shfl_sync(0xffffffffu, my_cnt, (j0 + b) & 31);
 #pragma unroll
-        for (int b = 0; b < BATCH; ++b)
+                for (int t = 0; t < REST; ++t) {
+                    const int e = lane + 32 * (t + 1);
+                    kr[b][t] = (j0 + b < PER_WARP && e < cnt) ? __ldcg(src.slab + ((size_t)(w + (j0 + b) * LW) * nq + q) * SCAN_SLAB + e) : 0ull;
+                }
+            }
 #pragma unroll
-            for (int t = 0; t < PER; ++t) {
-                const uint64_t k = kk[b][t];
-                if (k != 0 && key_score(k) >= bf) {
-                    const int p = atomicAdd(s_total, 1);
-                    if (p < src.key_cap) skeys[p] = k;
-                }
-            }
-    }
-    const int spilled = src.ucnt[q];
+            for (int b = 0; b < RB; ++b)
+#pragma unroll
+                for (int t = 0; t < REST; ++t) keep(kr[b][t]);
+        }
+    }
     const int ns = min(spilled, src.ucap);
     for (int e = tid; e < ns; e += THREADS) {
         const uint64_t k = __ldcg(src.ubuf + (size_t)q * src.ucap + e);
@@ -538,13 +556,12 @@
 {
     extern __shared__ __align__(16) unsigned char st_smem[];
     uint64_t *skeys = reinterpret_cast<uint64_t *>(st_smem);
-    __shared__ int s_cnts[256];
     __shared__ int s_total, s_bin, s_need, s_m;
     __shared__ int hist[256];
     __shared__ float s_bf;
     const int q = blockIdx.x, tid = threadIdx.x;
     bool inc = false;
-    const int total = load_slab_keys<SR_THREADS>(src, q, nq, skeys, s_cnts, &s_total, &s_bf, &inc);
+    const int total = load_slab_keys<SR_THREADS>(src, q, nq, skeys, &s_total, &s_bf, &inc);
     for (int e = tid; e < kp; e += SR_THREADS) merged[(int64_t)q * kp + e] = 0;
     if (tid == 0) { incomplete[q] = inc ? 1 : 0; s_m = 0; }
     __syncthreads();
@@ -587,24 +604,26 @@
     __shared__ uint64_t surv[MERGE_SURV];
     __shared__ int hist[256];
     __shared__ int s_bin, s_need, s_m, s_nz, s_cnt, s_band, s_viol, s_out, s_total;
-    __shared__ int s_cnts[256];
     __shared__ uint32_t s_L;
     __shared__ float s_thr, s_bf;
     __shared__ double s_dot[64], s_rr[64], s_qq, s_score[64];
     const int q = blockIdx.x, tid = threadIdx.x, lane = tid & 31, warp = tid >> 5;
+    VM_STAMP_VARS(const int stamp0 = STAMP_SEL + STAMP_PER * q;)
+    VM_STAMP_IF(tid == 0, stamp0 + STAMP_SEL_ENTRY);
 
     pdl_launch_dependents();
     if (tid == 0) { s_m = 0; s_nz = 0; s_cnt = 0; s_band = 0; s_viol = 0; s_thr = -INFINITY; }
     if (tid < 64) s_top[tid] = 0;
     pdl_wait();
     __syncthreads();
+    VM_STAMP_IF(tid == 0, stamp0 + STAMP_SEL_WAITED);
 
     const bool union_mode = src.slab != nullptr;
     int total, lists = src.lists, list_len = src.list_len;
     bool overflow = false;
     int nz = 0;
     if (union_mode) {
-        total = load_slab_keys<SR_THREADS>(src, q, nq, skeys, s_cnts, &s_total, &s_bf, &overflow);
+        total = load_slab_keys<SR_THREADS>(src, q, nq, skeys, &s_total, &s_bf, &overflow);
         lists = 0;
         if (tid == 0) nz = total;
     } else {
@@ -620,6 +639,7 @@
     for (int i = tid; i < dim; i += SR_THREADS) sq[i] = load_as_double(queries, q_dtype, (int64_t)q * dim + i);
     if (nz) atomicAdd(&s_nz, nz);
     __syncthreads();
+    VM_STAMP_IF(tid == 0, stamp0 + STAMP_SEL_KEYS);
     const int nonzero = s_nz;
     bool done = false;
     if (total <= MERGE_SURV) {
@@ -700,7 +720,9 @@
     const bool cand_valid = j < kp && mykey != 0;
     if (j < 64) s_rid[j] = cand_valid ? key_row(mykey) : NO_ROW;
     __syncthreads();
+    VM_STAMP_IF(tid == 0, stamp0 + STAMP_SEL_RANKED);
     stage_and_chain<NEUMAIER, T, SR_THREADS>(rows, ld, dim, kp, s_rid, srow, pitch, sq, s_dot, s_rr, &s_qq);
+    VM_STAMP_IF(tid == 0, stamp0 + STAMP_SEL_CHAINS);
 
     double sc = 0.0;
     const uint32_t row = cand_valid ? key_row(mykey) : 0;
@@ -720,6 +742,7 @@
             f.out_count[q] = c;
             flags[q] = 0;
             if (collect_thr) collect_thr[q] = INFINITY;
+            VM_STAMP_IF(true, stamp0 + STAMP_SEL_EXIT);
         }
         return;
     }
@@ -779,6 +802,7 @@
             f.out_idx[(int64_t)q * f.k + t] = -1;
             f.out_score[(int64_t)q * f.k + t] = 0.0;
         }
+        VM_STAMP_IF(tid == 0, stamp0 + STAMP_SEL_EXIT);
         return;
     }
     if (tid == 0 && cum) { atomicAdd(cum, 1ull); if (s_viol) atomicAdd(cum + 4, 1ull); }
@@ -806,6 +830,7 @@
             flags[q] = 0;
             if (collect_thr) collect_thr[q] = INFINITY;
             if (cum) atomicAdd(cum + 1, 1ull);
+            VM_STAMP_IF(true, stamp0 + STAMP_SEL_EXIT);
         }
         return;
     }
@@ -824,6 +849,7 @@
         f.out_idx[(int64_t)q * f.k + t] = -1;
         f.out_score[(int64_t)q * f.k + t] = 0.0;
     }
+    VM_STAMP_IF(tid == 0, stamp0 + STAMP_SEL_EXIT);
 }
 
 static constexpr int CR_THREADS = 512;
@@ -959,9 +985,15 @@
                                                                int32_t *__restrict__ xlist_cnt, unsigned long long *__restrict__ cum,
                                                                int *__restrict__ done_ctr, FinalizeArgs f, uint8_t *__restrict__ taken)
 {
+    VM_STAMP_VARS(const bool stamper = done_ctr != nullptr && blockIdx.x == 0 && threadIdx.x == 0;)
+    VM_STAMP_IF(stamper, STAMP_FIX);
     pdl_launch_dependents();
     pdl_wait();
-    if (flags && flags[nq] == 0) return;
+    VM_STAMP_IF(stamper, STAMP_FIX + 1);
+    if (flags && flags[nq] == 0) {
+        VM_STAMP_IF(stamper, STAMP_FIX + 2);
+        return;
+    }
     if (flags && cum && blockIdx.x == 0 && threadIdx.x == 0) atomicAdd(cum + 3, (unsigned long long)flags[nq]);
     extern __shared__ __align__(16) unsigned char xs_smem[];
     double *sq = reinterpret_cast<double *>(xs_smem);
@@ -1267,6 +1299,9 @@
     out[i] = zero ? 0.0 : __ddiv_rn(dot.result<NEUMAIER>(), den);
 }
 
+#ifdef VIDMEM_STEP_STAMPS
+VM_STAMPS_BINDER(stamps_bind_select)
+#endif
 int k_merge_candidates(const uint64_t *cand, int lists, int nq, int kp, uint64_t *merged, cudaStream_t st)
 {
     size_t smem = (size_t)lists * kp * sizeof(uint64_t) + (size_t)lists * sizeof(uint32_t) + 16;
diff --git a/real-time-brain-inspired-video-memory_b200/csrc/store.cu b/real-time-brain-inspired-video-memory_b200/csrc/store.cu
--- a/real-time-brain-inspired-video-memory_b200/csrc/store.cu
+++ b/real-time-brain-inspired-video-memory_b200/csrc/store.cu
@@ -72,8 +72,11 @@
                                          int32_t *__restrict__ zero_me, uint32_t *__restrict__ zero_tab, int zero_tab_n,
                                          int tf32_round, int split)
 {
+    VM_STAMP_VARS(const bool stamper = blockIdx.x == 0 && threadIdx.x == 0;)
+    VM_STAMP_IF(stamper, STAMP_NORM);
     pdl_launch_dependents();
     pdl_wait();
+    VM_STAMP_IF(stamper, STAMP_NORM + 1);
     if (zero_me && blockIdx.x == 0 && threadIdx.x < 2) zero_me[threadIdx.x] = 0;
     for (int i = blockIdx.x * blockDim.x + threadIdx.x; i < zero_tab_n; i += gridDim.x * blockDim.x) zero_tab[i] = 0u;
     int lane = threadIdx.x & 31;
@@ -99,6 +102,7 @@
             if (split) out_bf16[((int64_t)nq_pad + w) * ld + c] = __float2bfloat16_rn(v - __bfloat162float(hi));
         }
     }
+    VM_STAMP_IF(stamper, STAMP_NORM + 2);
 }
 
 template <typename T>
@@ -137,6 +141,9 @@
     }
 }
 
+#ifdef VIDMEM_STEP_STAMPS
+VM_STAMPS_BINDER(stamps_bind_store)
+#endif
 int k_convert_rows(const void *src, int src_dtype, void *dst, int dst_dtype, int64_t n, int dim, int ld, cudaStream_t st)
 {
     if (n <= 0) return VM_OK;
```

Result: faster. 269,600, median of 6 (+2.4%).
